# cvjena/mvlm

Hardware: AMD Instinct MI355X
Metric: views/sec (render+CNN+fuse) per mesh, 256x256x96 views (higher is better)
Workload: dtype f32; 1 GPU; configs[2] BU_3DFE-RGB+depth.json: 96 views @ 256x256 of one 99458-triangle textured synthetic face OBJ, 84 landmarks, 4 input channels (RGB+depth), seeded random weights; views_total=96, views_per_gpu=96, landmarks=84, in_channels=4, triangles=99458, selection_method=simple, parallelism=1 GPU, no collective

## Files before the change

### include/mvlm_hip.h

```cpp
#ifndef MVLM_HIP_H
#define MVLM_HIP_H

#include <stddef.h>
#include <stdint.h>

#ifdef __cplusplus
extern "C" {
#endif

typedef struct mvlm_ctx mvlm_ctx;
typedef struct mvlm_mesh mvlm_mesh;
typedef struct mvlm_texture mvlm_texture;

#define MVLM_IMAGE_SIZE 256
#define MVLM_CONV_DESC_INTS 12

enum { MVLM_MODE_QUANTILE = 0, MVLM_MODE_ABSOLUTE = 1 };
enum { MVLM_MAXIMA_SIMPLE = 0, MVLM_MAXIMA_MOMENT = 1 };

int mvlm_ctx_create(int device, mvlm_ctx** out);
void mvlm_ctx_destroy(mvlm_ctx* ctx);
const char* mvlm_last_error(mvlm_ctx* ctx);
int mvlm_set_stream(mvlm_ctx* ctx, void* hip_stream);
int mvlm_synchronize(mvlm_ctx* ctx);
const char* mvlm_build_arch(void);

typedef struct mvlm_obj mvlm_obj;
enum { MVLM_OBJ_ERR_ARGS = 1, MVLM_OBJ_ERR_FILE = 2, MVLM_OBJ_ERR_EMPTY = 3, MVLM_OBJ_ERR_INDEX = 4,
       MVLM_OBJ_ERR_SYNTAX = 5 };
int mvlm_obj_read(const char* path, mvlm_obj** out, char* err, int err_len);
int mvlm_obj_info(const mvlm_obj* obj, int64_t* n_verts, int64_t* n_tris, int* has_uvs);
int mvlm_obj_copy(const mvlm_obj* obj, float* verts, float* uvs, int32_t* tris);
int mvlm_obj_has_colors(const mvlm_obj* obj, int* has);
int mvlm_obj_copy_colors(const mvlm_obj* obj, uint8_t* rgb);
int mvlm_obj_has_normals(const mvlm_obj* obj, int* has);
int mvlm_obj_copy_normals(const mvlm_obj* obj, float* normals);
void mvlm_obj_free(mvlm_obj* obj);
int mvlm_mesh_read(const char* path, mvlm_obj** out, char* err, int err_len);

int mvlm_mesh_upload(mvlm_ctx* ctx, const float* verts_host, const float* uvs_host, int n_verts,
                     const int32_t* tris_host, int n_tris, const uint8_t* tex_host, int tex_h, int tex_w,
                     mvlm_mesh** out);
int mvlm_mesh_upload_colors(mvlm_ctx* ctx, mvlm_mesh* mesh, const uint8_t* rgb_host, int n_verts);
int mvlm_mesh_set_point_radius(mvlm_ctx* ctx, mvlm_mesh* mesh, double r_model_units);
int mvlm_mesh_point_radius(const mvlm_mesh* mesh, double* r_model_units);
int mvlm_points_auto_radius(const float* verts_host, int n, double* r_model_units);
int mvlm_points_set_counting(mvlm_ctx* ctx, int enabled);
int mvlm_points_get_stats(mvlm_ctx* ctx, unsigned long long* covered, unsigned long long* issued);
int mvlm_points_stage_ms(mvlm_ctx* ctx, float* ms2);
int mvlm_mesh_upload_normals(mvlm_ctx* ctx, mvlm_mesh* mesh, const float* normals_host, int n_verts);
int mvlm_mesh_estimate_normals(mvlm_ctx* ctx, mvlm_mesh* mesh, int32_t* neighbors_dev);
int mvlm_mesh_copy_normals(mvlm_ctx* ctx, const mvlm_mesh* mesh, float* normals_host);
int mvlm_normals_stage_ms(mvlm_ctx* ctx, float* ms3);
int mvlm_normals_get_stats(mvlm_ctx* ctx, unsigned long long* stats3);
int mvlm_mesh_triangulate_points(mvlm_ctx* ctx, const mvlm_mesh* cloud, const int32_t* neighbors_dev, int32_t* tris_dev, long long cap,
                                 int32_t* n_tris_dev);
int mvlm_cloud_mesh_stage_ms(mvlm_ctx* ctx, float* ms3);
void mvlm_mesh_free(mvlm_ctx* ctx, mvlm_mesh* mesh);

int mvlm_jpeg_info(const uint8_t* jpeg_host, size_t n_bytes, int* width, int* height, int* components, char* why, int why_len);
int mvlm_mesh_upload_jpeg(mvlm_ctx* ctx, const float* verts_host, const float* uvs_host, int n_verts,
                          const int32_t* tris_host, int n_tris, const uint8_t* jpeg_host, size_t jpeg_bytes,
                          mvlm_mesh** out);
int mvlm_texture_from_jpeg(mvlm_ctx* ctx, const uint8_t* jpeg_host, size_t jpeg_bytes, mvlm_texture** out);
int mvlm_texture_size(const mvlm_texture* tex, int* height, int* width);
void mvlm_texture_free(mvlm_ctx* ctx, mvlm_texture* tex);
int mvlm_mesh_upload_texture(mvlm_ctx* ctx, const float* verts_host, const float* uvs_host, int n_verts,
                             const int32_t* tris_host, int n_tris, mvlm_texture* tex, int* consumed, mvlm_mesh** out);
int mvlm_jpeg_decode(mvlm_ctx* ctx, const uint8_t* jpeg_host, size_t jpeg_bytes, uint8_t* rgb_dev, int* rounds_out);

int mvlm_render(mvlm_ctx* ctx, const mvlm_mesh* mesh, const double* rot_host, int n_views, float* out_dev);
int mvlm_render_rotations_dev(mvlm_ctx* ctx, const double** rot_dev);
int mvlm_set_render_shading(mvlm_ctx* ctx, int shading);
int mvlm_set_render_subpixel_bits(mvlm_ctx* ctx, int bits);
int mvlm_set_render_multisamples(mvlm_ctx* ctx, int samples);
int mvlm_render_set_profiling(mvlm_ctx* ctx, int enabled);
int mvlm_render_get_profile(mvlm_ctx* ctx, int32_t* n_views, int32_t* n_verts, int32_t* n_tris, float* ms, int cap);
int mvlm_render_check(mvlm_ctx* ctx);

int mvlm_render_landmark_view(mvlm_ctx* ctx, const mvlm_mesh* mesh, const double* rot_host, int n_views, int size,
                              const float* frame_host ,
                              const double* landmarks_host , int n_lm,
                              float radius, const uint8_t* lm_rgb_host ,
                              uint8_t* out_dev , int32_t* lm_pixels_dev );
int mvlm_landmark_view_stage_ms(mvlm_ctx* ctx, float* ms7);
int mvlm_render_landmark_view_colored(mvlm_ctx* ctx, const mvlm_mesh* mesh, const double* rot_host, int n_views, int size,
                                      const float* frame_host, const double* landmarks_host, int n_lm, float radius,
                                      const uint8_t* lm_rgb_host, uint8_t* out_dev, int32_t* lm_pixels_dev,
                                      const uint8_t* vert_rgba_dev );

int mvlm_render_ray_view(mvlm_ctx* ctx, const mvlm_mesh* mesh, const double* rot_host, int n_views, int size,
                         const float* frame_host, const double* landmarks_host, int n_lm, float radius, const uint8_t* lm_rgb_host,
                         const double* starts_dev, const double* ends_dev, int n_rays ,
                         float ray_radius, const uint8_t* ray_rgb_host ,
                         uint8_t* out_dev, int32_t* lm_pixels_dev, int32_t* ray_pixels_dev );
int mvlm_ray_view_stage_ms(mvlm_ctx* ctx, float* ms8);

int mvlm_view_sheet_layout(int n_views, int cols_in, int scale, int gap, int* cols, int* rows, int* width, int* height, char* why,
                           int why_len);
int mvlm_render_view_sheet(mvlm_ctx* ctx, const float* images_dev, int n_views, const float* maxima_dev, int n_lm,
                           const double* rot_host, const double* landmarks_host, const uint8_t* lm_rgb_host, const uint8_t* used_host,
                           int background, int cols_in, int scale, int gap, double marker_radius, uint8_t* out_dev);

int mvlm_heat_plane_peaks(mvlm_ctx* ctx, const float* heat_dev, int n_planes, float* peaks_dev);
int mvlm_render_heat_sheet(mvlm_ctx* ctx, const float* images_dev, const float* heat_dev, int n_views, int n_lm,
                           const uint8_t* sel_host , const uint8_t* lm_rgb_host ,
                           int background, int cols_in, int scale, int gap, double floor, double opacity, uint8_t* out_dev);
int mvlm_heat_sheet_stage_ms(mvlm_ctx* ctx, float* ms3);

int mvlm_surface_heat(mvlm_ctx* ctx, const mvlm_mesh* mesh, const double* rot_dev, const float* images_dev, const float* heat_dev,
                      int n_views, int n_lm, const uint8_t* sel_host, const uint8_t* lm_rgb_host, double floor, double opacity,
                      int depth_tol, uint8_t* vert_rgba_dev, float* score_dev ,
                      int32_t* n_vis_dev , int32_t* peak_vertex_dev ,
                      float* peak_score_dev );
int mvlm_surface_heat_stage_ms(mvlm_ctx* ctx, float* ms3);
int mvlm_surface_heat_release(mvlm_ctx* ctx);
int mvlm_scratch_bytes(mvlm_ctx* ctx, const char* prefix, size_t* bytes);

int mvlm_landmark_geodesics(mvlm_ctx* ctx, const mvlm_mesh* mesh, const double* pts_dev, int n, int init_rings, int max_sweeps,
                            long long max_scratch_bytes, const int32_t* pairs_host, int n_pairs, double* snapped_dev,
                            int32_t* tri_dev, double* D_dev, double* E_dev, int32_t* sweeps_dev, double* field_dev);
int mvlm_geodesic_stage_ms(mvlm_ctx* ctx, float* ms4);
int mvlm_geodesic_release(mvlm_ctx* ctx);

int mvlm_png_bound(int height, int width, size_t* bytes);
int mvlm_png_encode(mvlm_ctx* ctx, const uint8_t* rgba_dev, int n_images, int height, int width, int filter_mode,
                    uint8_t* png_host, size_t stride_bytes, size_t* png_bytes_out );
int mvlm_png_stage_ms(mvlm_ctx* ctx, float* ms4);

int mvlm_cnn_load(mvlm_ctx* ctx, const float* blob_host, size_t n_floats, const int32_t* desc_host, int n_slots,
                  int n_landmarks, int in_channels);
size_t mvlm_cnn_workspace_bytes(mvlm_ctx* ctx, int batch);
int mvlm_cnn_maxima(mvlm_ctx* ctx, const float* images_dev, int n_views, const int32_t* chan_sel_host,
                    float* maxima_dev, void* workspace_dev, size_t workspace_bytes, int batch);
int mvlm_cnn_set_selection(mvlm_ctx* ctx, int method);
int mvlm_cnn_heatmaps(mvlm_ctx* ctx, const float* images_dev, int n_views, const int32_t* chan_sel_host,
                      float* heat_dev, void* workspace_dev, size_t workspace_bytes, int batch);
int mvlm_cnn_set_execution(mvlm_ctx* ctx, int graph_mode, int concurrency);
int mvlm_cnn_set_pairing(mvlm_ctx* ctx, int mode);
int mvlm_cnn_set_winograd(mvlm_ctx* ctx, int mode);
int mvlm_pack_winograd_weights(const float* w9_host, int cin_pad, int cout_pad, float* w12_host);
int mvlm_cnn_set_winograd4(mvlm_ctx* ctx, int mode);
int mvlm_pack_winograd4_weights(const float* w9_host, int cin_pad, int cout_pad, float* w18_host);
int mvlm_cnn_set_winograd4_wide(mvlm_ctx* ctx, int on);
int mvlm_conv_wino4_wide_serves(int ksize, int cin_pad, int cout_pad, int size);
int mvlm_conv_wino4_wide_launches(mvlm_ctx* ctx, int64_t* count, int reset);
int mvlm_cnn_set_winograd4_padded(mvlm_ctx* ctx, int mode);
int mvlm_conv_wino4_padded_launches(mvlm_ctx* ctx, int64_t* count, int reset);
int mvlm_conv_wino4_padded_stride(int cout_pad);
int mvlm_pack_winograd4_weights_padded(const float* w9_host, const float* bias_host, int cin_pad, int cout_pad, float* w18_pad_host,
                                       float* bias_pad_host);
int mvlm_cnn_execution_stats(mvlm_ctx* ctx, int64_t* eager_runs, int64_t* graph_captures, int64_t* graph_replays,
                             int64_t* graph_failures);
size_t mvlm_pack_fast_weights(const float* w, int cout, int cin, int cout_pad, int cin_pad, uint16_t* out);
int mvlm_cnn_load_fast(mvlm_ctx* ctx, const uint16_t* blob_host, size_t n_u16, const int64_t* slot_offsets, int n_slots);
int mvlm_cnn_set_precision(mvlm_ctx* ctx, int fast);
int mvlm_conv2d_fast(mvlm_ctx* ctx, const float* x_dev, int batch, int cin, int h, int w, const float* w_host, int cout,
                     const float* bias_host, const float* pre_scale_host, const float* pre_shift_host,
                     const float* post_scale_host, const float* post_shift_host, const float* r_dev, float* y_dev);
size_t mvlm_pack_fast_weights16(const float* w, int cout, int cin, int cout_pad, int cin_pad, uint16_t* out, float* unscale);
int mvlm_cnn_load_fast16(mvlm_ctx* ctx, const uint16_t* blob_host, size_t n_u16, const int64_t* slot_offsets,
                         const float* slot_unscale, int n_slots);
int mvlm_cnn_fast16_overflowed(mvlm_ctx* ctx, int* overflowed);
int mvlm_conv2d_fast16(mvlm_ctx* ctx, const float* x_dev, int batch, int cin, int h, int w, const float* w_host, int cout,
                       const float* bias_host, const float* pre_scale_host, const float* pre_shift_host,
                       const float* post_scale_host, const float* post_shift_host, const float* r_dev, float* y_dev);
int mvlm_cnn_set_profiling(mvlm_ctx* ctx, int enabled);
int mvlm_cnn_get_profile(mvlm_ctx* ctx, int32_t* slot, int32_t* variant, double* flops, float* ms, int cap);
const char* mvlm_conv_variant_name(int variant);
int mvlm_cnn_get_profile_shapes(mvlm_ctx* ctx, int32_t* shapes6, int cap);
int mvlm_conv_variant_serves(int variant, int ksize, int cin_pad, int cout_pad, int size, int kind);
int mvlm_conv_set_override(mvlm_ctx* ctx, int ksize, int cin_pad, int cout_pad, int size, int kind, int variant);

int mvlm_heatmap_maxima(mvlm_ctx* ctx, const float* heat_dev, int n_views, int n_landmarks, int size, int method,
                        float* out_dev);

int mvlm_conv2d(mvlm_ctx* ctx, const float* x_dev, int batch, int cin, int h, int w, const float* w_host, int cout,
                int ksize, const float* bias_host, const float* pre_scale_host, const float* pre_shift_host,
                const float* post_scale_host, const float* post_shift_host, const float* r_dev, int upsample_in,
                float* y_dev);

int mvlm_conv2d_pair(mvlm_ctx* ctx, int batch, int cin, int cout, const float* x0_dev, int size0, const float* w0_host,
                     const float* r0_dev, float* raw0_dev, float* y0_dev, const float* x1_dev, int size1,
                     const float* w1_host, const float* r1_dev, float* raw1_dev, float* y1_dev,
                     const float* pre_scale_host, const float* pre_shift_host, int variant);
int mvlm_conv_force_variant(mvlm_ctx* ctx, int variant);
int mvlm_conv_bench(mvlm_ctx* ctx, int batch, int cin, int cout, int ksize, int size, int flags, int variant, int iters,
                    float* ms_per_launch, int* variant_used);
int mvlm_conv_pair_bench(mvlm_ctx* ctx, int batch, int cin, int cout, int size, int flags, int variant, int iters,
                         float* ms_per_launch);

int mvlm_estimate_lines(mvlm_ctx* ctx, const float* maxima_dev, const double* rot_dev, int n_views, int n_landmarks,
                        int image_size, double* starts_dev, double* ends_dev);
int mvlm_consensus_mask(mvlm_ctx* ctx, const float* maxima_dev, int n_views, int n_landmarks, int mode, double q,
                        double thr, uint8_t* mask_dev, int32_t* count_dev);
int mvlm_consensus_solve(mvlm_ctx* ctx, const double* starts_dev, const double* ends_dev, const uint8_t* mask_dev,
                         const int32_t* count_dev, const int32_t* draws_dev, int n_views, int n_landmarks,
                         double* out_dev, double* err_dev);

#define MVLM_REPORT_STATS 9
#define MVLM_VIEW_KEPT 1
#define MVLM_VIEW_DRAWN 2
#define MVLM_VIEW_INLIER 4
#define MVLM_VIEW_USED 8
int mvlm_consensus_report(mvlm_ctx* ctx, const double* starts_dev, const double* ends_dev, const uint8_t* mask_dev,
                          const int32_t* draws_dev, int n_views, int n_landmarks, double* out_dev, double* err_dev,
                          double* stats_dev, int32_t* counts_dev, double* dist2_dev, uint8_t* flags_dev);

int mvlm_project_to_surface(mvlm_ctx* ctx, const mvlm_mesh* mesh, const double* pts_dev, int n_points,
                            double* out_dev);

int mvlm_surface_attach(mvlm_ctx* ctx, const mvlm_mesh* mesh, const double* pts_dev, int n_points, double* snapped_dev,
                        int32_t* tri_dev, double* bary_dev, double* uv_dev);

int mvlm_clip_rays_to_mesh(mvlm_ctx* ctx, const mvlm_mesh* mesh, const double* starts_dev, const double* ends_dev,
                           int n_rays, double* new_ends_dev, uint8_t* hit_dev);

int mvlm_allgather_maxima(mvlm_ctx* ctx, void* nccl_comm, int rank, int world, const float* maxima_local_dev, int n_total,
                          int n_landmarks, float* maxima_all_dev);
int mvlm_gather_pack(mvlm_ctx* ctx, const float* maxima_local_dev, int n_local, int n_max, int n_landmarks, float* slot_dev);
int mvlm_gather_unpack(mvlm_ctx* ctx, const float* slots_dev, int world, int n_total, int n_landmarks, float* maxima_all_dev);

#ifdef __cplusplus
}
#endif
#endif
```

### mvlm_amd/_lib.py

```python
from __future__ import annotations

import ctypes as C
import os
import subprocess
import threading
from pathlib import Path

_HERE = Path(__file__).resolve().parent
LIB_PATH = Path(os.environ["MVLM_HIP_LIB"]) if os.environ.get("MVLM_HIP_LIB") else _HERE / "lib" / "libmvlm_hip.so"
CSRC = _HERE / "csrc"

c_float_p = C.POINTER(C.c_float)
c_double_p = C.POINTER(C.c_double)
c_int32_p = C.POINTER(C.c_int32)
c_uint8_p = C.POINTER(C.c_uint8)

SIGNATURES = {
    "mvlm_ctx_create": (C.c_int, [C.c_int, C.POINTER(C.c_void_p)]),
    "mvlm_ctx_destroy": (None, [C.c_void_p]),
    "mvlm_last_error": (C.c_char_p, [C.c_void_p]),
    "mvlm_set_stream": (C.c_int, [C.c_void_p, C.c_void_p]),
    "mvlm_synchronize": (C.c_int, [C.c_void_p]),
    "mvlm_build_arch": (C.c_char_p, []),
    "mvlm_obj_read": (C.c_int, [C.c_char_p, C.POINTER(C.c_void_p), C.c_char_p, C.c_int]),
    "mvlm_mesh_read": (C.c_int, [C.c_char_p, C.POINTER(C.c_void_p), C.c_char_p, C.c_int]),
    "mvlm_obj_info": (C.c_int, [C.c_void_p, C.POINTER(C.c_int64), C.POINTER(C.c_int64), C.POINTER(C.c_int)]),
    "mvlm_obj_copy": (C.c_int, [C.c_void_p, c_float_p, c_float_p, c_int32_p]),
    "mvlm_obj_has_colors": (C.c_int, [C.c_void_p, C.POINTER(C.c_int)]),
    "mvlm_obj_copy_colors": (C.c_int, [C.c_void_p, c_uint8_p]),
    "mvlm_obj_has_normals": (C.c_int, [C.c_void_p, C.POINTER(C.c_int)]),
    "mvlm_obj_copy_normals": (C.c_int, [C.c_void_p, c_float_p]),
    "mvlm_obj_free": (None, [C.c_void_p]),
    "mvlm_mesh_upload": (C.c_int, [C.c_void_p, c_float_p, c_float_p, C.c_int, c_int32_p, C.c_int, c_uint8_p,
                                   C.c_int, C.c_int, C.POINTER(C.c_void_p)]),
    "mvlm_mesh_upload_colors": (C.c_int, [C.c_void_p, C.c_void_p, c_uint8_p, C.c_int]),
    "mvlm_mesh_set_point_radius": (C.c_int, [C.c_void_p, C.c_void_p, C.c_double]),
    "mvlm_mesh_point_radius": (C.c_int, [C.c_void_p, c_double_p]),
    "mvlm_points_auto_radius": (C.c_int, [c_float_p, C.c_int, c_double_p]),
    "mvlm_points_set_counting": (C.c_int, [C.c_void_p, C.c_int]),
    "mvlm_points_stage_ms": (C.c_int, [C.c_void_p, c_float_p]),
    "mvlm_points_get_stats": (C.c_int, [C.c_void_p, C.POINTER(C.c_uint64), C.POINTER(C.c_uint64)]),
    "mvlm_mesh_upload_normals": (C.c_int, [C.c_void_p, C.c_void_p, c_float_p, C.c_int]),
    "mvlm_mesh_estimate_normals": (C.c_int, [C.c_void_p, C.c_void_p, C.c_void_p]),
    "mvlm_mesh_copy_normals": (C.c_int, [C.c_void_p, C.c_void_p, c_float_p]),
    "mvlm_normals_stage_ms": (C.c_int, [C.c_void_p, c_float_p]),
    "mvlm_normals_get_stats": (C.c_int, [C.c_void_p, C.POINTER(C.c_uint64)]),
    "mvlm_mesh_triangulate_points": (C.c_int, [C.c_void_p, C.c_void_p, C.c_void_p, C.c_void_p, C.c_longlong, C.c_void_p]),
    "mvlm_cloud_mesh_stage_ms": (C.c_int, [C.c_void_p, c_float_p]),
    "mvlm_mesh_free": (None, [C.c_void_p, C.c_void_p]),
    "mvlm_jpeg_info": (C.c_int, [c_uint8_p, C.c_size_t, C.POINTER(C.c_int), C.POINTER(C.c_int), C.POINTER(C.c_int), C.c_char_p, C.c_int]),
    "mvlm_mesh_upload_jpeg": (C.c_int, [C.c_void_p, c_float_p, c_float_p, C.c_int, c_int32_p, C.c_int, c_uint8_p, C.c_size_t,
                                        C.POINTER(C.c_void_p)]),
    "mvlm_texture_from_jpeg": (C.c_int, [C.c_void_p, c_uint8_p, C.c_size_t, C.POINTER(C.c_void_p)]),
    "mvlm_texture_size": (C.c_int, [C.c_void_p, C.POINTER(C.c_int), C.POINTER(C.c_int)]),
    "mvlm_texture_free": (None, [C.c_void_p, C.c_void_p]),
    "mvlm_mesh_upload_texture": (C.c_int, [C.c_void_p, c_float_p, c_float_p, C.c_int, c_int32_p, C.c_int, C.c_void_p,
                                           C.POINTER(C.c_int), C.POINTER(C.c_void_p)]),
    "mvlm_jpeg_decode": (C.c_int, [C.c_void_p, c_uint8_p, C.c_size_t, C.c_void_p, C.POINTER(C.c_int)]),
    "mvlm_render": (C.c_int, [C.c_void_p, C.c_void_p, c_double_p, C.c_int, C.c_void_p]),
    "mvlm_render_check": (C.c_int, [C.c_void_p]),
    "mvlm_render_landmark_view": (C.c_int, [C.c_void_p, C.c_void_p, c_double_p, C.c_int, C.c_int, c_float_p, c_double_p, C.c_int,
                                            C.c_float, c_uint8_p, C.c_void_p, C.c_void_p]),
    "mvlm_landmark_view_stage_ms": (C.c_int, [C.c_void_p, c_float_p]),
    "mvlm_render_ray_view": (C.c_int, [C.c_void_p, C.c_void_p, c_double_p, C.c_int, C.c_int, c_float_p, c_double_p, C.c_int,
                                       C.c_float, c_uint8_p, C.c_void_p, C.c_void_p, C.c_int, C.c_float, c_uint8_p,
                                       C.c_void_p, C.c_void_p, C.c_void_p]),
    "mvlm_ray_view_stage_ms": (C.c_int, [C.c_void_p, c_float_p]),
    "mvlm_view_sheet_layout": (C.c_int, [C.c_int, C.c_int, C.c_int, C.c_int, C.POINTER(C.c_int), C.POINTER(C.c_int), C.POINTER(C.c_int),
                                         C.POINTER(C.c_int), C.c_char_p, C.c_int]),
    "mvlm_render_view_sheet": (C.c_int, [C.c_void_p, C.c_void_p, C.c_int, C.c_void_p, C.c_int, c_double_p, c_double_p, c_uint8_p,
                                         c_uint8_p, C.c_int, C.c_int, C.c_int, C.c_int, C.c_double, C.c_void_p]),
    "mvlm_heat_plane_peaks": (C.c_int, [C.c_void_p, C.c_void_p, C.c_int, C.c_void_p]),
    "mvlm_render_heat_sheet": (C.c_int, [C.c_void_p, C.c_void_p, C.c_void_p, C.c_int, C.c_int, c_uint8_p, c_uint8_p, C.c_int, C.c_int,
                                         C.c_int, C.c_int, C.c_double, C.c_double, C.c_void_p]),
    "mvlm_heat_sheet_stage_ms": (C.c_int, [C.c_void_p, c_float_p]),
    "mvlm_surface_heat": (C.c_int, [C.c_void_p, C.c_void_p, C.c_void_p, C.c_void_p, C.c_void_p, C.c_int, C.c_int, c_uint8_p, c_uint8_p,
                                    C.c_double, C.c_double, C.c_int, C.c_void_p, C.c_void_p, C.c_void_p, C.c_void_p, C.c_void_p]),
    "mvlm_surface_heat_stage_ms": (C.c_int, [C.c_void_p, c_float_p]),
    "mvlm_surface_heat_release": (C.c_int, [C.c_void_p]),
    "mvlm_render_landmark_view_colored": (C.c_int, [C.c_void_p, C.c_void_p, c_double_p, C.c_int, C.c_int, c_float_p, c_double_p, C.c_int,
                                                    C.c_float, c_uint8_p, C.c_void_p, C.c_void_p, C.c_void_p]),
    "mvlm_scratch_bytes": (C.c_int, [C.c_void_p, C.c_char_p, C.POINTER(C.c_size_t)]),
    "mvlm_landmark_geodesics": (C.c_int, [C.c_void_p, C.c_void_p, C.c_void_p, C.c_int, C.c_int, C.c_int, C.c_longlong, c_int32_p, C.c_int,
                                          C.c_void_p, C.c_void_p, C.c_void_p, C.c_void_p, C.c_void_p, C.c_void_p]),
    "mvlm_geodesic_stage_ms": (C.c_int, [C.c_void_p, c_float_p]),
    "mvlm_geodesic_release": (C.c_int, [C.c_void_p]),
    "mvlm_png_bound": (C.c_int, [C.c_int, C.c_int, C.POINTER(C.c_size_t)]),
    "mvlm_png_encode": (C.c_int, [C.c_void_p, C.c_void_p, C.c_int, C.c_int, C.c_int, C.c_int, C.c_void_p, C.c_size_t,
                                  C.POINTER(C.c_size_t)]),
    "mvlm_png_stage_ms": (C.c_int, [C.c_void_p, c_float_p]),
    "mvlm_render_set_profiling": (C.c_int, [C.c_void_p, C.c_int]),
    "mvlm_render_get_profile": (C.c_int, [C.c_void_p, c_int32_p, c_int32_p, c_int32_p, c_float_p, C.c_int]),
    "mvlm_render_rotations_dev": (C.c_int, [C.c_void_p, C.POINTER(C.c_void_p)]),
    "mvlm_gather_pack": (C.c_int, [C.c_void_p, C.c_void_p, C.c_int, C.c_int, C.c_int, C.c_void_p]),
    "mvlm_gather_unpack": (C.c_int, [C.c_void_p, C.c_void_p, C.c_int, C.c_int, C.c_int, C.c_void_p]),
    "mvlm_allgather_maxima": (C.c_int, [C.c_void_p, C.c_void_p, C.c_int, C.c_int, C.c_void_p, C.c_int, C.c_int, C.c_void_p]),
    "mvlm_set_render_shading": (C.c_int, [C.c_void_p, C.c_int]),
    "mvlm_set_render_subpixel_bits": (C.c_int, [C.c_void_p, C.c_int]),
    "mvlm_set_render_multisamples": (C.c_int, [C.c_void_p, C.c_int]),
    "mvlm_cnn_load": (C.c_int, [C.c_void_p, c_float_p, C.c_size_t, c_int32_p, C.c_int, C.c_int, C.c_int]),
    "mvlm_cnn_workspace_bytes": (C.c_size_t, [C.c_void_p, C.c_int]),
    "mvlm_cnn_maxima": (C.c_int, [C.c_void_p, C.c_void_p, C.c_int, c_int32_p, C.c_void_p, C.c_void_p, C.c_size_t,
                                  C.c_int]),
    "mvlm_cnn_heatmaps": (C.c_int, [C.c_void_p, C.c_void_p, C.c_int, c_int32_p, C.c_void_p, C.c_void_p, C.c_size_t,
                                    C.c_int]),
    "mvlm_cnn_set_execution": (C.c_int, [C.c_void_p, C.c_int, C.c_int]),
    "mvlm_cnn_set_selection": (C.c_int, [C.c_void_p, C.c_int]),
    "mvlm_cnn_set_pairing": (C.c_int, [C.c_void_p, C.c_int]),
    "mvlm_cnn_set_winograd": (C.c_int, [C.c_void_p, C.c_int]),
    "mvlm_pack_winograd_weights": (C.c_int, [c_float_p, C.c_int, C.c_int, c_float_p]),
    "mvlm_cnn_set_winograd4": (C.c_int, [C.c_void_p, C.c_int]),
    "mvlm_pack_winograd4_weights": (C.c_int, [c_float_p, C.c_int, C.c_int, c_float_p]),
    "mvlm_cnn_set_winograd4_wide": (C.c_int, [C.c_void_p, C.c_int]),
    "mvlm_conv_wino4_wide_serves": (C.c_int, [C.c_int, C.c_int, C.c_int, C.c_int]),
    "mvlm_conv_wino4_wide_launches": (C.c_int, [C.c_void_p, C.POINTER(C.c_int64), C.c_int]),
    "mvlm_cnn_set_winograd4_padded": (C.c_int, [C.c_void_p, C.c_int]),
    "mvlm_conv_wino4_padded_launches": (C.c_int, [C.c_void_p, C.POINTER(C.c_int64), C.c_int]),
    "mvlm_conv_wino4_padded_stride": (C.c_int, [C.c_int]),
    "mvlm_pack_winograd4_weights_padded": (C.c_int, [c_float_p, c_float_p, C.c_int, C.c_int, c_float_p, c_float_p]),
    "mvlm_cnn_execution_stats": (C.c_int, [C.c_void_p, C.POINTER(C.c_int64), C.POINTER(C.c_int64), C.POINTER(C.c_int64),
                                          C.POINTER(C.c_int64)]),
    "mvlm_pack_fast_weights": (C.c_size_t, [c_float_p, C.c_int, C.c_int, C.c_int, C.c_int, C.POINTER(C.c_uint16)]),
    "mvlm_cnn_load_fast": (C.c_int, [C.c_void_p, C.POINTER(C.c_uint16), C.c_size_t, C.POINTER(C.c_int64), C.c_int]),
    "mvlm_cnn_set_precision": (C.c_int, [C.c_void_p, C.c_int]),
    "mvlm_pack_fast_weights16": (C.c_size_t, [c_float_p, C.c_int, C.c_int, C.c_int, C.c_int, C.POINTER(C.c_uint16), c_float_p]),
    "mvlm_cnn_load_fast16": (C.c_int, [C.c_void_p, C.POINTER(C.c_uint16), C.c_size_t, C.POINTER(C.c_int64), c_float_p, C.c_int]),
    "mvlm_cnn_fast16_overflowed": (C.c_int, [C.c_void_p, C.POINTER(C.c_int)]),
    "mvlm_conv2d_fast16": (C.c_int, [C.c_void_p, C.c_void_p, C.c_int, C.c_int, C.c_int, C.c_int, c_float_p, C.c_int, c_float_p,
                                     c_float_p, c_float_p, c_float_p, c_float_p, C.c_void_p, C.c_void_p]),
    "mvlm_conv2d_fast": (C.c_int, [C.c_void_p, C.c_void_p, C.c_int, C.c_int, C.c_int, C.c_int, c_float_p, C.c_int, c_float_p,
                                   c_float_p, c_float_p, c_float_p, c_float_p, C.c_void_p, C.c_void_p]),
    "mvlm_cnn_set_profiling": (C.c_int, [C.c_void_p, C.c_int]),
    "mvlm_cnn_get_profile": (C.c_int, [C.c_void_p, c_int32_p, c_int32_p, c_double_p, c_float_p, C.c_int]),
    "mvlm_conv_variant_name": (C.c_char_p, [C.c_int]),
    "mvlm_cnn_get_profile_shapes": (C.c_int, [C.c_void_p, c_int32_p, C.c_int]),
    "mvlm_conv_variant_serves": (C.c_int, [C.c_int, C.c_int, C.c_int, C.c_int, C.c_int, C.c_int]),
    "mvlm_conv_set_override": (C.c_int, [C.c_void_p, C.c_int, C.c_int, C.c_int, C.c_int, C.c_int, C.c_int]),
    "mvlm_heatmap_maxima": (C.c_int, [C.c_void_p, C.c_void_p, C.c_int, C.c_int, C.c_int, C.c_int, C.c_void_p]),
    "mvlm_conv2d": (C.c_int, [C.c_void_p, C.c_void_p, C.c_int, C.c_int, C.c_int, C.c_int, c_float_p, C.c_int, C.c_int,
                              c_float_p, c_float_p, c_float_p, c_float_p, c_float_p, C.c_void_p, C.c_int, C.c_void_p]),
    "mvlm_conv2d_pair": (C.c_int, [C.c_void_p, C.c_int, C.c_int, C.c_int, C.c_void_p, C.c_int, c_float_p, C.c_void_p, C.c_void_p,
                                   C.c_void_p, C.c_void_p, C.c_int, c_float_p, C.c_void_p, C.c_void_p, C.c_void_p, c_float_p, c_float_p,
                                   C.c_int]),
    "mvlm_conv_force_variant": (C.c_int, [C.c_void_p, C.c_int]),
    "mvlm_conv_bench": (C.c_int, [C.c_void_p, C.c_int, C.c_int, C.c_int, C.c_int, C.c_int, C.c_int, C.c_int, C.c_int,
                                  c_float_p, C.POINTER(C.c_int)]),
    "mvlm_conv_pair_bench": (C.c_int, [C.c_void_p, C.c_int, C.c_int, C.c_int, C.c_int, C.c_int, C.c_int, C.c_int, c_float_p]),
    "mvlm_estimate_lines": (C.c_int, [C.c_void_p, C.c_void_p, C.c_void_p, C.c_int, C.c_int, C.c_int, C.c_void_p,
                                      C.c_void_p]),
    "mvlm_consensus_mask": (C.c_int, [C.c_void_p, C.c_void_p, C.c_int, C.c_int, C.c_int, C.c_double, C.c_double,
                                      C.c_void_p, C.c_void_p]),
    "mvlm_consensus_solve": (C.c_int, [C.c_void_p, C.c_void_p, C.c_void_p, C.c_void_p, C.c_void_p, C.c_void_p, C.c_int,
                                       C.c_int, C.c_void_p, C.c_void_p]),
    "mvlm_project_to_surface": (C.c_int, [C.c_void_p, C.c_void_p, C.c_void_p, C.c_int, C.c_void_p]),
    "mvlm_consensus_report": (C.c_int, [C.c_void_p, C.c_void_p, C.c_void_p, C.c_void_p, C.c_void_p, C.c_int, C.c_int,
                                        C.c_void_p, C.c_void_p, C.c_void_p, C.c_void_p, C.c_void_p, C.c_void_p]),
    "mvlm_surface_attach": (C.c_int, [C.c_void_p, C.c_void_p, C.c_void_p, C.c_int, C.c_void_p, C.c_void_p, C.c_void_p,
                                      C.c_void_p]),
    "mvlm_clip_rays_to_mesh": (C.c_int, [C.c_void_p, C.c_void_p, C.c_void_p, C.c_void_p, C.c_int, C.c_void_p,
                                         C.c_void_p]),
}

_lib = None


class MvlmHipError(RuntimeError):
    pass


def build(force: bool = False) -> Path:
    if force and LIB_PATH.exists():
        LIB_PATH.unlink()
    jobs = str(min(8, os.cpu_count() or 1))
    r = subprocess.run(["make", "-C", str(CSRC), "-j", jobs], capture_output=True, text=True)
    if r.returncode != 0 or not LIB_PATH.exists():
        raise MvlmHipError(f"building libmvlm_hip.so failed:\n{r.stdout[-4000:]}\n{r.stderr[-4000:]}")
    return LIB_PATH


def load():
    global _lib
    if _lib is not None:
        return _lib
    if not LIB_PATH.exists():
        raise MvlmHipError(
            f"{LIB_PATH} not found - the MI355X HIP library is required (no CPU fallback). "
            "Build it with `python -c 'import __graft_entry__ as g; g.build()'` or `make -C mvlm_amd/csrc`.")
    import torch

    lib = C.CDLL(str(LIB_PATH))
    for name, (res, args) in SIGNATURES.items():
        fn = getattr(lib, name)
        fn.restype = res
        fn.argtypes = args
    _lib = lib
    return lib


def as_ptr(arr, ctype):
    return arr.ctypes.data_as(C.POINTER(ctype))


class Context:

    def __init__(self, device: int = 0):
        self.lib = load()
        self.handle = C.c_void_p()
        rc = self.lib.mvlm_ctx_create(int(device), C.byref(self.handle))
        if rc != 0:
            reasons = {2: "no such GPU device", 3: "hipSetDevice failed", 4: "hipGetDeviceProperties failed",
                       5: "device is not a gfx950 (MI355X)"}
            raise MvlmHipError(f"mvlm_ctx_create(device={device}) failed: {reasons.get(rc, rc)}")
        self.device = int(device)

    def check(self, rc: int, exc=MvlmHipError):
        if rc != 0:
            msg = self.lib.mvlm_last_error(self.handle)
            raise exc(msg.decode() if msg else f"mvlm call failed ({rc})")

    def set_stream(self, stream_ptr: int):
        self.check(self.lib.mvlm_set_stream(self.handle, C.c_void_p(stream_ptr)))
        self._bound_stream = stream_ptr

    def bind_current_stream(self, torch, dev):
        held = getattr(self, "_held_stream", None)
        if held is not None and held[0] == threading.get_ident() and getattr(self, "_bound_stream", None) == held[1]:
            return
        self.set_stream(torch.cuda.current_stream(dev).cuda_stream)

    def hold_stream(self, torch, dev):
        return _HeldStream(self, torch, dev)

    def synchronize(self):
        self.check(self.lib.mvlm_synchronize(self.handle))

    def close(self):
        if getattr(self, "handle", None) and self.handle.value:
            self.lib.mvlm_ctx_destroy(self.handle)
            self.handle = C.c_void_p()

    def __del__(self):
        try:
            self.close()
        except Exception:
            pass


class _HeldStream:
    def __init__(self, ctx, torch, dev):
        self.ctx, self.torch, self.dev, self.mine = ctx, torch, dev, False

    def __enter__(self):
        if getattr(self.ctx, "_held_stream", None) is None:
            ptr = self.torch.cuda.current_stream(self.dev).cuda_stream
            self.ctx.set_stream(ptr)
            self.ctx._held_stream = (threading.get_ident(), ptr)
            self.mine = True
        return self

    def __exit__(self, *exc):
        if self.mine:
            self.ctx._held_stream = None
        return False


_contexts: dict[int, Context] = {}


def get_context(device: int = 0) -> Context:
    ctx = _contexts.get(device)
    if ctx is None:
        ctx = _contexts[device] = Context(device)
# ... 2 lines not shown
```

### mvlm_amd/csrc/api.hip

```cpp
#include <atomic>
#include <cstring>

#include <memory>

#include <cmath>

#include "common.h"
#include "raster_points_math.h"
#include "raster_view_math.h"

void* mvlm_ctx::get_scratch(const char* name, size_t bytes) {
    auto& e = scratch[name];
    if (e.second >= bytes && e.first) return e.first;
    if (e.first) {
        hipStreamSynchronize(stream);
        hipFree(e.first);
        e = {nullptr, 0};
    }
    void* p = nullptr;
    const size_t want = bytes + bytes / 4 + 256;
    if (hipMalloc(&p, want) != hipSuccess) return nullptr;
    e = {p, want};
    return p;
}

extern "C" const char* mvlm_build_arch(void) { return "gfx950"; }

extern "C" int mvlm_ctx_create(int device, mvlm_ctx** out) {
    if (!out) return 1;
    *out = nullptr;
    int n = 0;
    if (hipGetDeviceCount(&n) != hipSuccess || device < 0 || device >= n) return 2;
    if (hipSetDevice(device) != hipSuccess) return 3;
    hipDeviceProp_t prop;
    if (hipGetDeviceProperties(&prop, device) != hipSuccess) return 4;
    auto* ctx = new mvlm_ctx();
    ctx->device = device;
    if (std::string(prop.gcnArchName).rfind("gfx950", 0) != 0) {
        fprintf(stderr, "mvlm_hip: device %d is %s, this library is built for gfx950 (MI355X) only\n", device,
                prop.gcnArchName);
        delete ctx;
        return 5;
    }
    *out = ctx;
    return 0;
}

extern "C" void mvlm_ctx_destroy(mvlm_ctx* ctx) {
    if (!ctx) return;
    hipSetDevice(ctx->device);
    hipStreamSynchronize(ctx->stream);
    for (auto& kv : ctx->scratch)
        if (kv.second.first) hipFree(kv.second.first);
    if (ctx->cnn.blob) hipFree(ctx->cnn.blob);
    if (ctx->cnn.fast_blob) hipFree(ctx->cnn.fast_blob);
    if (ctx->cnn.fast16_blob) hipFree(ctx->cnn.fast16_blob);
    for (auto& ww : ctx->cnn.wino)
        if (ww.blob) hipFree(ww.blob);
    if (ctx->cnn.wino4_pad_blob) hipFree(ctx->cnn.wino4_pad_blob);
    if (ctx->cnn.fast16_flag) hipFree(ctx->cnn.fast16_flag);
    if (ctx->switch_event) hipEventDestroy(ctx->switch_event);
    for (int i = 0; i < 2; ++i) {
        if (ctx->kparts_ws[i]) hipFree(ctx->kparts_ws[i]);
        if (ctx->kparts_cnt[i]) hipFree(ctx->kparts_cnt[i]);
    }
    for (auto& e : ctx->mesh_pool) {
        hipFree(e.p);
        if (e.freed) hipEventDestroy(e.freed);
    }
    for (hipEvent_t e : ctx->event_free) hipEventDestroy(e);
    for (int i = 0; i < 2; ++i) {
        if (ctx->upload_stage[i]) hipHostFree(ctx->upload_stage[i]);
        if (ctx->upload_stage_done[i]) hipEventDestroy(ctx->upload_stage_done[i]);
    }
    if (ctx->upload_stream) hipStreamDestroy(ctx->upload_stream);
    if (ctx->jpeg_scratch) hipFree(ctx->jpeg_scratch);
    if (ctx->jpeg_flags_host) hipHostFree(ctx->jpeg_flags_host);
    if (ctx->render_overflow_host) hipHostFree(ctx->render_overflow_host);
    for (auto e : ctx->cnn.event_pool)
        if (e) hipEventDestroy(e);
    for (auto e : ctx->render_events)
        if (e) hipEventDestroy(e);
    for (auto e : ctx->cnn.sync_events)
        if (e) hipEventDestroy(e);
    ctx->cnn.drop_graphs();
    if (ctx->cnn.side_stream) hipStreamDestroy(ctx->cnn.side_stream);
    if (ctx->cnn.capture_stream) hipStreamDestroy(ctx->cnn.capture_stream);
    delete ctx;
}

extern "C" const char* mvlm_last_error(mvlm_ctx* ctx) {
    if (!ctx) return "null context";
    if (mvlm_thread_error_ctx() != ctx) {
        std::lock_guard<std::mutex> lock(ctx->err_mu);
        mvlm_thread_error() = ctx->err;
        mvlm_thread_error_ctx() = ctx;
    }
    return mvlm_thread_error().c_str();
}

extern "C" int mvlm_set_stream(mvlm_ctx* ctx, void* hip_stream) {
    MVLM_ENTER(ctx);
    hipStream_t next = static_cast<hipStream_t>(hip_stream);
    if (next != ctx->stream) {
        if (!ctx->switch_event) MVLM_CHECK_HIP(ctx, hipEventCreateWithFlags(&ctx->switch_event, hipEventDisableTiming));
        if (!ctx->track_order) {
            MVLM_CHECK_HIP(ctx, hipEventRecord(ctx->switch_event, ctx->stream));
            ctx->order_recorded = true;
            ctx->track_order = true;
        }
        if (ctx->order_recorded) MVLM_CHECK_HIP(ctx, hipStreamWaitEvent(next, ctx->switch_event, 0));
    }
    ctx->stream = next;
    return 0;
}

extern "C" int mvlm_synchronize(mvlm_ctx* ctx) {
    MVLM_ENTER(ctx);
    MVLM_CHECK_HIP(ctx, hipStreamSynchronize(ctx->stream));
    return 0;
}

static bool take_upload_buffer(mvlm_ctx* ctx, size_t bytes, size_t room, void** p, size_t* cap, hipEvent_t* waited) {
    int pick = -1;
    for (int k = 0; k < int(ctx->mesh_pool.size()); ++k) {
        const size_t c = ctx->mesh_pool[size_t(k)].cap;
        if (c >= room && c <= 4 * bytes + (1u << 20)) {
            pick = k;
            break;
        }
    }
    if (pick >= 0) {
        const auto e = ctx->mesh_pool[size_t(pick)];
        ctx->mesh_pool.erase(ctx->mesh_pool.begin() + pick);
        ctx->mesh_pool_bytes -= e.cap;
        *p = e.p;
        *cap = e.cap;
        *waited = e.freed;
        return !(e.freed && hipStreamWaitEvent(ctx->upload_stream, e.freed, 0) != hipSuccess);
    }
    *cap = (room + 65535) / 65536 * 65536;
    if (hipMalloc(p, *cap) != hipSuccess) {
        *p = nullptr;
        *cap = 0;
        return false;
    }
    return true;
}

struct mvlm_texture {
    uint8_t* dev = nullptr;
    size_t cap = 0;
    int h = 0, w = 0;
    hipEvent_t waited = nullptr;
};

static int mesh_upload_impl(mvlm_ctx* ctx, const float* verts_host, const float* uvs_host, int n_verts, const int32_t* tris_host,
                            int n_tris, const uint8_t* tex_host, int tex_h, int tex_w, MvlmJpegPlan* jpeg,
                            const uint8_t* jpeg_bytes, size_t jpeg_n, mvlm_mesh** out, mvlm_texture* pre = nullptr) {
    MVLM_REQUIRE(ctx, out, "mesh_upload: null output");
    *out = nullptr;
    MVLM_REQUIRE(ctx, verts_host && n_verts > 0 && n_tris >= 0 && (tris_host || n_tris == 0), "mesh_upload: mesh does not contain any points");
    MVLM_REQUIRE(ctx, n_tris > 0 || !(jpeg || pre), "mesh_upload: a point cloud (n_tris == 0) takes no texture");
    if (n_tris == 0) {
        uvs_host = nullptr;
        tex_host = nullptr;
    }
    MVLM_REQUIRE(ctx, !(tex_host || jpeg || pre) || (tex_h > 0 && tex_w > 0), "mesh_upload: bad texture size");
    for (long i = 0; i < 3l * n_tris; ++i)
        MVLM_REQUIRE(ctx, tris_host[i] >= 0 && tris_host[i] < n_verts, "mesh_upload: triangle index out of range");
    const bool with_tex = (tex_host || jpeg || pre) && uvs_host;
    if (!with_tex) jpeg = nullptr;
    if (!with_tex) pre = nullptr;
    const void* src[4] = {verts_host, uvs_host, tris_host, with_tex && !jpeg && !pre ? tex_host : nullptr};
    const size_t bytes[4] = {size_t(n_verts) * 12, uvs_host ? size_t(n_verts) * 8 : 0, size_t(n_tris) * 12,
                             with_tex ? size_t(tex_h) * tex_w * 3 : 0};
    const size_t room[4] = {bytes[0], bytes[1], bytes[2], bytes[3] ? bytes[3] + 4 : 0};
    size_t off[5], total = 0;
    for (int i = 0; i < 4; ++i) {
        off[i] = total;
        total += ((src[i] ? bytes[i] : 0) + 255) / 256 * 256;
    }
    off[4] = total;
    if (jpeg) total += mvlm_jpeg_stage_bytes(*jpeg, jpeg_n);

    std::lock_guard<std::mutex> upload_lock(ctx->upload_mu);
    MVLM_CHECK_HIP(ctx, hipSetDevice(ctx->device));
    if (!ctx->upload_stream) MVLM_CHECK_HIP(ctx, hipStreamCreateWithFlags(&ctx->upload_stream, hipStreamNonBlocking));
    const int slot = ctx->upload_stage_next;
    ctx->upload_stage_next ^= 1;
    if (ctx->upload_stage_done[slot]) MVLM_CHECK_HIP(ctx, hipEventSynchronize(ctx->upload_stage_done[slot]));
    if (ctx->upload_stage_cap[slot] < total) {
        if (ctx->upload_stage[slot]) (void)hipHostFree(ctx->upload_stage[slot]);
        ctx->upload_stage[slot] = nullptr;
        ctx->upload_stage_cap[slot] = 0;
        const size_t cap = (total + (size_t(4) << 20)) / (size_t(4) << 20) * (size_t(4) << 20);
        MVLM_CHECK_HIP(ctx, hipHostMalloc(&ctx->upload_stage[slot], cap, hipHostMallocDefault));
        ctx->upload_stage_cap[slot] = cap;
    }
    auto* stage = static_cast<unsigned char*>(ctx->upload_stage[slot]);
    for (int i = 0; i < 4; ++i)
        if (src[i] && bytes[i]) std::memcpy(stage + off[i], src[i], bytes[i]);
    std::string jpeg_why;
    if (jpeg && mvlm_jpeg_fill_stage(*jpeg, jpeg_bytes, jpeg_n, stage + off[4], jpeg_why) != 0) {
        ctx->fail("jpeg: " + jpeg_why);
        return 2;
    }

    auto* m = new mvlm_mesh();
    static std::atomic<unsigned long long> next_uid{1};
    m->uid = next_uid.fetch_add(1);
    m->n_verts = n_verts;
// ... 537 lines not shown
```

### mvlm_amd/csrc/cnn_graph.hip

```cpp
#include <cstdlib>
#include <cstring>

#include "common.h"

namespace {

constexpr long CONCURRENT_MAX_PIXELS_32 = 32l * 32 * 32;

struct Tensor {
    float* p = nullptr;
    int C = 0, S = 0;
    size_t off = 0, elems = 0;
};

struct Block {
    size_t off, size;
    bool free;
    int arena;
    bool deferred;
};

bool parity_slots_usable(const ConvSlotDesc& r) { return r.present != 0 && (r.cout_pad == 96 || r.cout_pad == 80 || r.cout_pad == 84); }

struct Exec {
// ... 1 lines not shown
    CnnState& st;
    int B;
    char* ws;
    size_t ws_bytes;
    bool dry;
    size_t cursor = 0, high = 0;
    std::vector<Block> blocks;
    int rc = 0;
    int arena = 0;
    bool forked = false;
    const bool no_pool_fusion = [] { const char* e = getenv("MVLM_POOL_KERNEL_ONLY"); return e && e[0] == '1'; }();
    const bool scatter_only = [] { const char* e = getenv("MVLM_SCATTER_ONLY"); return e && e[0] == '1'; }();
    const int consumer_add_max_batch = [] { const char* e = getenv("MVLM_CONSUMER_ADD_MAX_BATCH"); return e ? atoi(e) : 16; }();

    Exec(mvlm_ctx* c, int batch, void* w, size_t wb, bool d) : ctx(c), st(c->cnn), B(batch), ws((char*)w), ws_bytes(wb), dry(d) {}

    Tensor alloc_raw(size_t bytes, int C, int S) {
        bytes = (bytes + 255) / 256 * 256;
        Tensor t;
        t.C = C;
        t.S = S;
        t.elems = bytes / 4;
        for (auto& b : blocks)
            if (b.free && b.size == bytes && b.arena == arena) {
                b.free = false;
                t.off = b.off;
                t.p = dry ? nullptr : reinterpret_cast<float*>(ws + b.off);
                return t;
            }
        blocks.push_back({cursor, bytes, false, arena, false});
        t.off = cursor;
        cursor += bytes;
        if (cursor > high) high = cursor;
        if (!dry && cursor > ws_bytes) {
            rc = ctx->fail("cnn: workspace too small (mvlm_cnn_workspace_bytes)");
            t.p = nullptr;
            return t;
        }
        t.p = dry ? nullptr : reinterpret_cast<float*>(ws + t.off);
        return t;
    }
    Tensor alloc(int C, int S) { return alloc_raw(size_t(B) * C * S * S * 4, C, S); }
    void release(const Tensor& t) {
        for (auto& b : blocks)
            if (b.off == t.off && !b.free && !b.deferred) {
                if (forked && b.arena == 0)
                    b.deferred = true;
                else
                    b.free = true;
                return;
            }
    }

    hipEvent_t next_event() {
        if (st.sync_cursor >= st.sync_events.size()) st.sync_events.resize(st.sync_cursor + 1, nullptr);
        hipEvent_t& e = st.sync_events[st.sync_cursor++];
        if (!e && hipEventCreateWithFlags(&e, hipEventDisableTiming) != hipSuccess) {
            rc = ctx->fail("cnn: hipEventCreate failed");
            return nullptr;
        }
        return e;
    }
    void fork() {
        forked = true;
        if (dry || rc) return;
        if (!st.side_stream) {
            int lo_prio = 0, hi_prio = 0;
            (void)hipDeviceGetStreamPriorityRange(&lo_prio, &hi_prio);
            if (hipStreamCreateWithPriority(&st.side_stream, hipStreamNonBlocking, hi_prio) != hipSuccess) {
                rc = ctx->fail("cnn: hipStreamCreate failed");
                return;
            }
        }
        hipEvent_t e = next_event();
        if (rc) return;
        if (hipEventRecord(e, ctx->stream) != hipSuccess || hipStreamWaitEvent(st.side_stream, e, 0) != hipSuccess)
            rc = ctx->fail("cnn: fork of the side stream failed");
    }
    void side() {
        arena = 1;
        if (!dry) ctx->launch_stream = st.side_stream;
    }
    void main() {
        arena = 0;
        ctx->launch_stream = nullptr;
    }
    void join() {
        main();
        forked = false;
        for (auto& b : blocks)
            if (b.deferred) {
                b.deferred = false;
                b.free = true;
            }
        if (dry || rc) return;
        hipEvent_t e = next_event();
        if (rc) return;
        if (hipEventRecord(e, st.side_stream) != hipSuccess || hipStreamWaitEvent(ctx->stream, e, 0) != hipSuccess)
            rc = ctx->fail("cnn: join of the side stream failed");
    }

    const ConvSlotDesc& d(int slot) const { return st.desc[size_t(slot)]; }
    const float* blob(int off) const { return off < 0 ? nullptr : st.blob + off; }

    void fill_shape(int slot, ConvArgs& a, int S) const {
        const ConvSlotDesc& r = d(slot);
        a.cin = r.cin;
        a.cout = r.cout;
        a.ksize = r.ksize;
        a.cin_pad = r.cin_pad;
        a.cout_pad = r.cout_pad;
        a.B = B;
        a.H = a.W = S;
    }
    int fill(int slot, const Tensor& x, ConvArgs& a, int S) {
        if (rc) return rc;
        const ConvSlotDesc& r = d(slot);
        if (!r.present) return rc = ctx->fail("cnn: conv slot not present in the packed weights");
        a.in = x.p;
        a.in_ctot = x.C;
        a.in_coff = 0;
        fill_shape(slot, a, S);
        a.w = blob(r.w_off);
        for (int f = 0; f < MVLM_WINO_FORMS_N; ++f) {
            const CnnState::WinoWeights& ww = st.wino[f];
            a.*mvlm_wino_form(f).weights = (size_t(slot) < ww.off.size() && ww.off[size_t(slot)] >= 0) ? ww.blob + ww.off[size_t(slot)] : nullptr;
        }
        a.wino4_pad = size_t(slot) < st.wino4_pad_id.size() ? st.wino4_pad_id[size_t(slot)] : 0;
        a.bias = blob(r.bias_off);
        a.pre_scale = blob(r.pre_scale_off);
        a.pre_shift = blob(r.pre_shift_off);
        a.post_scale = blob(r.post_scale_off);
        a.post_shift = blob(r.post_shift_off);
        if (x.C != a.cin) return rc = ctx->fail("cnn: channel mismatch between graph and packed weights");
        return 0;
    }
    bool runs_fast(int slot, const ConvArgs& a) const {
        const std::vector<long long>& off = st.fast == 2 ? st.fast16_off : st.fast_off;
        return st.fast && size_t(slot) < off.size() && off[size_t(slot)] >= 0 && mvlm_conv_fast_ok(a, st.fast == 2 ? 2 : 3);
    }
    int prof_begin(hipEvent_t& e0, hipEvent_t& e1) {
        if (!st.profiling) return 0;
        if (st.event_cursor + 2 > st.event_pool.size()) st.event_pool.resize(st.event_cursor + 2, nullptr);
        for (int k = 0; k < 2; ++k) {
            hipEvent_t& e = st.event_pool[st.event_cursor + k];
            if (!e && hipEventCreate(&e) != hipSuccess) return rc = ctx->fail("cnn: hipEventCreate failed");
        }
        e0 = st.event_pool[st.event_cursor];
        e1 = st.event_pool[st.event_cursor + 1];
        st.event_cursor += 2;
        hipEventRecord(e0, ctx->cur_stream());
        return 0;
    }
    static double conv_flops(const ConvArgs& a, int variant = -1) {
        const double taps = mvlm_conv_variant_is_wino(variant) ? mvlm_wino_form(MVLM_WINO_F23).macs
                            : mvlm_conv_variant_is_wino4(variant) ? mvlm_wino_form(MVLM_WINO_F43).macs : double(a.ksize * a.ksize);
        return 2.0 * a.cin * a.cout * taps * double(a.H) * a.W * a.B * a.n_par;
    }

    int conv(int slot, const Tensor& x, ConvArgs a, int S) {
        if (fill(slot, x, a, S)) return rc;
        if (dry) return 0;
        int variant = -1;
        hipEvent_t e0 = nullptr, e1 = nullptr;
        if (prof_begin(e0, e1)) return rc;
        if (runs_fast(slot, a)) {
            if (st.fast == 2) {
                variant = MVLM_CONV_VARIANT_FAST16;
                if (mvlm_launch_conv_fast(ctx, a, st.fast16_blob + st.fast16_off[size_t(slot)], 2, st.fast16_unscale[size_t(slot)])) return rc = 1;
            } else {
                variant = MVLM_CONV_VARIANT_FAST;
                if (mvlm_launch_conv_fast(ctx, a, st.fast_blob + st.fast_off[size_t(slot)])) return rc = 1;
            }
        } else if (mvlm_launch_conv(ctx, a, &variant)) {
            return rc = 1;
        }
        if (st.profiling) {
            hipEventRecord(e1, ctx->cur_stream());
            ConvProfileRec rec{slot, variant, conv_flops(a, variant), e0, e1};
            const ConvKey key = mvlm_conv_key(a);
            const short shape[6] = {key.ksize, key.cin_pad, key.cout_pad, key.size, key.kind, key.batch};
            for (int i = 0; i < 6; ++i) rec.shape[i] = shape[i];
            st.prof.push_back(rec);
        }
        return 0;
    }

    int pair_variant(int slot0, const Tensor& x0, ConvArgs a0, int S0, int slot1, const Tensor& x1, ConvArgs a1, int S1) {
        if (st.pairing == 0 || fill(slot0, x0, a0, S0) || fill(slot1, x1, a1, S1)) return -1;
        if (runs_fast(slot0, a0) || runs_fast(slot1, a1)) return -1;
        if (mvlm_conv_wino_variant(ctx, a0) >= 0 || mvlm_conv_wino_variant(ctx, a1) >= 0) return -1;
        return mvlm_conv_pair_variant(a0, a1, st.pairing);
    }

    int conv_pair(int pv, int slot0, const Tensor& x0, ConvArgs a0, int S0, int slot1, const Tensor& x1, ConvArgs a1, int S1) {
        if (pv < 0) {
            conv(slot0, x0, a0, S0);
            return conv(slot1, x1, a1, S1);
        }
        if (fill(slot0, x0, a0, S0) || fill(slot1, x1, a1, S1)) return rc;
        if (dry) return 0;
        hipEvent_t e0 = nullptr, e1 = nullptr;
        if (prof_begin(e0, e1)) return rc;
        if (mvlm_launch_conv_pair(ctx, a0, a1, pv)) return rc = 1;
        if (st.profiling) {
            hipEventRecord(e1, ctx->cur_stream());
            st.prof.push_back({slot0, pv, conv_flops(a0) + conv_flops(a1), e0, e1});
        }
        return 0;
    }

    struct RbPlan {
        int base = 0, S = 0, cout = 0;
        bool resample = false;
        Tensor x, y, t1, t2;
        Tensor* pooled = nullptr;
        ConvArgs ar, a[3];
        bool want_pool = false, keep_full = true;
    };
    RbPlan plan_rb(int rb_index, const Tensor& x, Tensor* hi, Tensor* pooled = nullptr, bool keep_full = true) {
        RbPlan P;
        P.base = 1 + 4 * rb_index;
        P.S = x.S;
        P.x = x;
        P.cout = d(P.base + 1).cout * 2;
        const int cout = P.cout, h = cout / 2, q = cout / 4;
        P.resample = d(P.base).present != 0;
        if (!hi) P.y = alloc(cout, P.S);
        if (P.resample && hi) {
            rc = ctx->fail("cnn: resampling block cannot scatter");
            return P;
        }
        P.t1 = alloc(h, P.S);
        P.t2 = alloc(q, P.S);
        if (P.resample) {
            P.ar.out = P.y.p;
            P.ar.out_ctot = cout;
        }
        const Tensor& res = P.resample ? P.y : P.x;
        const int coffs[3] = {0, h, h + q};
        for (int j = 0; j < 3; ++j) {
            ConvArgs& a = P.a[j];
            a.res1 = res.p;
            a.res1_ctot = res.C;
            a.res1_coff = coffs[j];
            if (hi) {
                a.out = hi->p;
                a.out_ctot = hi->C;
                a.out_coff = coffs[j];
                a.up_out = 1;
                a.skip = hi->p;
                a.skip_ctot = hi->C;
                a.skip_coff = coffs[j];
            } else {
                a.out = P.y.p;
                a.out_ctot = cout;
                a.out_coff = coffs[j];
            }
        }
        P.a[0].out_raw = P.t1.p;
        P.a[0].raw_ctot = h;
        P.a[1].out_raw = P.t2.p;
        P.a[1].raw_ctot = q;
        P.want_pool = pooled && !hi;
        if (P.want_pool)
            for (ConvArgs& a : P.a) a.pool_hint = 1;
        P.keep_full = keep_full;
        P.pooled = pooled;
        if (P.want_pool) *pooled = alloc(cout, P.S / 2);
        return P;
    }
    const Tensor& rb_input(const RbPlan& P, int j) const { return j == 0 ? P.x : (j == 1 ? P.t1 : P.t2); }
    void set_pool(RbPlan& P, bool can_fuse) {
        if (!P.want_pool || !can_fuse) return;
        for (ConvArgs& a : P.a) {
            a.pool_out = P.pooled->p;
            a.pool_ctot = P.cout;
            a.pool_coff = a.out_coff;
            if (!P.keep_full) a.out = nullptr;
        }
    }
    void finish_rb(RbPlan& P) {
        release(P.t1);
        release(P.t2);
        if (P.want_pool && !P.a[0].pool_out && !dry && !rc) pool_kernel(P.y.p, P.cout, P.S, P.pooled->p);
    }
    void pool_kernel(const float* in, int channels, int S, float* out) {
        hipEvent_t e0 = nullptr, e1 = nullptr;
        if (prof_begin(e0, e1)) return;
        if (mvlm_launch_maxpool2(ctx, in, B * channels, S, S, out)) {
            rc = 1;
            return;
        }
        if (st.profiling) {
            hipEventRecord(e1, ctx->cur_stream());
            ConvProfileRec rec{-1, -1, 0.0, e0, e1};
            rec.shape[2] = short(channels);
            rec.shape[3] = short(S);
            rec.shape[5] = short(B > 32767 ? 32767 : B);
            st.prof.push_back(rec);
        }
    }

    Tensor rb(int rb_index, const Tensor& x, Tensor* hi, Tensor* pooled = nullptr, bool keep_full = true) {
        RbPlan P = plan_rb(rb_index, x, hi, pooled, keep_full);
        if (rc) return P.y;
        if (P.resample) conv(P.base, x, P.ar, P.S);
        bool fuse = P.want_pool;
        for (int j = 0; j < 3 && fuse; ++j) fuse = pool_fusable(P.base + 1 + j, rb_input(P, j), P.a[j], P.S);
        set_pool(P, fuse);
        for (int j = 0; j < 3; ++j) conv(P.base + 1 + j, rb_input(P, j), P.a[j], P.S);
        finish_rb(P);
        return P.y;
    }

    void rb_pair(int rbA, const Tensor& xA, Tensor& yA, int rbB, const Tensor& xB, Tensor& yB, Tensor* pooledB) {
        RbPlan PA = plan_rb(rbA, xA, nullptr), PB = plan_rb(rbB, xB, nullptr, pooledB);
        yA = PA.y;
        yB = PB.y;
        if (rc) return;
        if (PA.resample) conv(PA.base, xA, PA.ar, PA.S);
        if (PB.resample) conv(PB.base, xB, PB.ar, PB.S);
        int pv[3];
        bool fuse = PB.want_pool;
        for (int j = 0; j < 3; ++j) {
            pv[j] = pair_variant(PA.base + 1 + j, rb_input(PA, j), PA.a[j], PA.S, PB.base + 1 + j, rb_input(PB, j), PB.a[j], PB.S);
            if (fuse) fuse = pv[j] >= 0 ? (!no_pool_fusion && mvlm_conv_variant_can_pool(pv[j])) : pool_fusable(PB.base + 1 + j, rb_input(PB, j), PB.a[j], PB.S);
        }
        set_pool(PB, fuse);
        for (int j = 0; j < 3; ++j)
            conv_pair(pv[j], PA.base + 1 + j, rb_input(PA, j), PA.a[j], PA.S, PB.base + 1 + j, rb_input(PB, j), PB.a[j], PB.S);
        finish_rb(PA);
// ... 271 lines not shown
int run_batch(mvlm_ctx* ctx, const float* img, int nb, const int* sel4, float* maxima, int view0, int n_total,
              float* heat, void* ws, size_t ws_bytes) {
    CnnState& st = ctx->cnn;
    auto eager = [&]() {
        st.sync_cursor = 0;
        Exec ex(ctx, nb, ws, ws_bytes, false);
        const int rc = ex.forward(img, sel4, maxima, view0, n_total, heat);
        ctx->launch_stream = nullptr;
        ++st.eager_runs;
        return rc;
    };
    if (!st.graph_mode || st.profiling) return eager();
    const void* out = heat ? static_cast<const void*>(heat) : static_cast<const void*>(maxima);
    CnnGraphEntry* ent = nullptr;
    for (auto& g : st.graphs)
        if (g.images == img && g.out == out && g.ws == ws && g.ws_bytes == ws_bytes && g.nb == nb && g.view0 == view0 &&
            g.n_total == n_total && g.heat == (heat ? 1 : 0) && g.sel4[0] == sel4[0] && g.sel4[1] == sel4[1] &&
            g.sel4[2] == sel4[2] && g.sel4[3] == sel4[3]) {
            ent = &g;
            break;
        }
    if (!ent) {
        constexpr size_t MAX_GRAPHS = 16;
        if (st.graphs.size() >= MAX_GRAPHS) {
            if (st.graphs.front().exec) hipGraphExecDestroy(st.graphs.front().exec);
            st.graphs.erase(st.graphs.begin());
        }
        CnnGraphEntry g;
        g.images = img;
        g.out = out;
        g.ws = ws;
        g.ws_bytes = ws_bytes;
        g.nb = nb;
        g.view0 = view0;
        g.n_total = n_total;
        g.heat = heat ? 1 : 0;
        for (int k = 0; k < 4; ++k) g.sel4[k] = sel4[k];
        st.graphs.push_back(g);
        ent = &st.graphs.back();
    }
    ++ent->uses;
    if (ent->exec) {
        MVLM_CHECK_HIP(ctx, hipGraphLaunch(ent->exec, ctx->stream));
        ++st.graph_replays;
        return 0;
    }
    if (ent->uses < 2) return eager();
    auto note = [&](const char* what, hipError_t e) {
        if (st.graph_failures++ == 0)
            fprintf(stderr, "mvlm_hip: %s failed (%s); this pass runs launch by launch\n", what, hipGetErrorString(e));
        (void)hipGetLastError();
    };
    if (!st.capture_stream) {
        const hipError_t e = hipStreamCreateWithFlags(&st.capture_stream, hipStreamNonBlocking);
        if (e != hipSuccess) {
            st.capture_stream = nullptr;
            note("hipStreamCreate (capture stream)", e);
            return eager();
        }
    }
    st.sync_cursor = 0;
    hipStream_t user_stream = ctx->stream;
    hipError_t e_begin = hipStreamBeginCapture(st.capture_stream, hipStreamCaptureModeThreadLocal);
    if (e_begin != hipSuccess) {
        note("hipStreamBeginCapture", e_begin);
        return eager();
    }
    int rc;
    ctx->stream = st.capture_stream;
    {
        Exec ex(ctx, nb, ws, ws_bytes, false);
        rc = ex.forward(img, sel4, maxima, view0, n_total, heat);
        ctx->launch_stream = nullptr;
    }
    ctx->stream = user_stream;
    hipGraph_t graph = nullptr;
    const hipError_t e_end = hipStreamEndCapture(st.capture_stream, &graph);
    if (rc) {
        if (graph) hipGraphDestroy(graph);
        return rc;
    }
    if (e_end != hipSuccess || !graph) {
        note("hipStreamEndCapture", e_end);
        if (graph) hipGraphDestroy(graph);
        ent->uses = -1000000;
        return eager();
    }
    hipGraphExec_t exec = nullptr;
    const hipError_t e_inst = hipGraphInstantiate(&exec, graph, nullptr, nullptr, 0);
    hipGraphDestroy(graph);
    if (e_inst != hipSuccess || !exec) {
        note("hipGraphInstantiate", e_inst);
        ent->uses = -1000000;
        return eager();
    }
    ent->exec = exec;
    ++st.graph_captures;
    MVLM_CHECK_HIP(ctx, hipGraphLaunch(ent->exec, ctx->stream));
    ++st.graph_replays;
    return 0;
}

int run_cnn(mvlm_ctx* ctx, const float* images, int n_views, const int32_t* chan_sel, float* maxima, float* heat,
            void* ws, size_t ws_bytes, int batch) {
    CnnState& st = ctx->cnn;
    MVLM_REQUIRE(ctx, st.loaded, "cnn: mvlm_cnn_load has not been called");
    MVLM_REQUIRE(ctx, images && n_views > 0 && batch > 0 && ws, "cnn: bad arguments");
    MVLM_REQUIRE(ctx, maxima || heat, "cnn: no output requested");
    int sel4[4] = {0, 0, 0, 0};
    for (int k = 0; k < st.in_channels; ++k) {
        MVLM_REQUIRE(ctx, chan_sel[k] >= 0 && chan_sel[k] < 4, "cnn: channel selector out of range");
        sel4[k] = chan_sel[k];
    }
    st.prof.clear();
    st.event_cursor = 0;
    if (st.fast == 2) MVLM_CHECK_HIP(ctx, hipMemsetAsync(st.fast16_flag, 0, sizeof(unsigned), ctx->stream));
    const size_t img_elems = size_t(MVLM_IMAGE_SIZE) * MVLM_IMAGE_SIZE;
    for (int v0 = 0; v0 < n_views; v0 += batch) {
        const int nb = (n_views - v0) < batch ? (n_views - v0) : batch;
        float* h = heat ? heat + size_t(v0) * st.n_landmarks * img_elems : nullptr;
        const float* img = images + size_t(v0) * img_elems * 4;
        if (run_batch(ctx, img, nb, sel4, maxima, v0, n_views, h, ws, ws_bytes)) return 1;
    }
    return 0;
}

}

extern "C" int mvlm_cnn_load(mvlm_ctx* ctx, const float* blob_host, size_t n_floats, const int32_t* desc_host,
                             int n_slots, int n_landmarks, int in_channels) {
    MVLM_ENTER(ctx);
    MVLM_REQUIRE(ctx, blob_host && desc_host && n_floats > 0, "cnn_load: null weights");
    MVLM_REQUIRE(ctx, n_slots == MVLM_N_SLOTS, "cnn_load: descriptor table must have 183 conv slots");
    MVLM_REQUIRE(ctx, n_landmarks > 0 && in_channels >= 1 && in_channels <= 4, "cnn_load: bad landmark / channel count");
    CnnState& st = ctx->cnn;
    MVLM_CHECK_HIP(ctx, hipSetDevice(ctx->device));
    if (st.blob) {
        MVLM_CHECK_HIP(ctx, hipFree(st.blob));
        st.blob = nullptr;
    }
    st.loaded = false;
    st.fast = 0;
    st.fast_off.clear();
    if (st.fast_blob) {
        (void)hipFree(st.fast_blob);
        st.fast_blob = nullptr;
    }
    st.fast16_off.clear();
    st.fast16_unscale.clear();
    if (st.fast16_blob) {
        (void)hipFree(st.fast16_blob);
        st.fast16_blob = nullptr;
    }
    float** const form_blobs[MVLM_WINO_FORMS_N + 1] = {&st.wino[MVLM_WINO_F23].blob, &st.wino[MVLM_WINO_F43].blob, &st.wino4_pad_blob};
    for (float** b : form_blobs)
        if (*b) {
            (void)hipFree(*b);
            *b = nullptr;
        }
    for (CnnState::WinoWeights& ww : st.wino) ww.off.clear();
    st.wino4_pad_id.clear();
    ctx->conv_wino4_pads.resize(1);
    st.drop_graphs();
    st.desc.resize(size_t(n_slots));
    memcpy(st.desc.data(), desc_host, size_t(n_slots) * sizeof(ConvSlotDesc));
    for (const ConvSlotDesc& r : st.desc) {
        if (!r.present) continue;
        MVLM_REQUIRE(ctx, r.cin > 0 && r.cout > 0 && r.ksize >= 1 && r.ksize <= 3, "cnn_load: bad conv shape");
        MVLM_REQUIRE(ctx, r.cin_pad % 4 == 0 && r.cin_pad >= r.cin &&
                              (r.cout_pad % 16 == 0 || (r.cout_pad == 84 && r.cout == 84 && (r.ksize == 3 || r.ksize == 2))) && r.cout_pad >= r.cout,
                     "cnn_load: bad padding");
        const size_t wsz = size_t(r.ksize) * r.ksize * r.cin_pad * r.cout_pad;
        MVLM_REQUIRE(ctx, r.w_off >= 0 && size_t(r.w_off) + wsz <= n_floats, "cnn_load: weight offset out of range");
        const int offs[5] = {r.bias_off, r.pre_scale_off, r.pre_shift_off, r.post_scale_off, r.post_shift_off};
        const int lens[5] = {r.cout_pad, r.cin_pad, r.cin_pad, r.cout_pad, r.cout_pad};
        for (int k = 0; k < 5; ++k)
            MVLM_REQUIRE(ctx, offs[k] < 0 || size_t(offs[k]) + lens[k] <= n_floats, "cnn_load: vector offset out of range");
    }
    MVLM_REQUIRE(ctx, st.desc[0].cin == in_channels, "cnn_load: conv1 input channels != in_channels");
    MVLM_REQUIRE(ctx, st.desc[MVLM_SLOT_CONV11].cout == n_landmarks, "cnn_load: conv11 output channels != n_landmarks");
    MVLM_CHECK_HIP(ctx, hipMalloc(&st.blob, n_floats * sizeof(float)));
    MVLM_CHECK_HIP(ctx, hipMemcpy(st.blob, blob_host, n_floats * sizeof(float), hipMemcpyHostToDevice));
    std::vector<float> host[MVLM_WINO_FORMS_N + 1];
    std::vector<ConvPackTargets> to(st.desc.size());
    size_t total[MVLM_WINO_FORMS_N + 1] = {0, 0, 0};
    for (int s = 0; s < n_slots; ++s) {
        const ConvSlotDesc& r = st.desc[size_t(s)];
        if (!r.present) continue;
        const ConvPackSizes sizes = mvlm_conv_pack_sizes(r.ksize, r.cin_pad, r.cout_pad);
        for (int f = 0; f < MVLM_WINO_FORMS_N; ++f)
            if (mvlm_wino_form(f).serves_slot(r.ksize, r.cin_pad, r.cout_pad)) {
                to[size_t(s)].wino[f] = &host[f];
                total[f] += sizes.wino[f];
            }
        if (mvlm_conv_wino4_pad_serves_slot(r.ksize, r.cin_pad, r.cout_pad)) {
            to[size_t(s)].wino4_pad = &host[MVLM_WINO_FORMS_N];
            total[MVLM_WINO_FORMS_N] += sizes.wino4_pad + sizes.wino4_pad_bias;
        }
    }
    for (int k = 0; k <= MVLM_WINO_FORMS_N; ++k) host[k].reserve(total[k]);
    for (CnnState::WinoWeights& ww : st.wino) ww.off.assign(size_t(n_slots), -1);
    st.wino4_pad_id.assign(size_t(n_slots), 0);
    std::vector<ConvPackOffsets> made(st.desc.size());
    for (int s = 0; s < n_slots; ++s) {
        const ConvSlotDesc& r = st.desc[size_t(s)];
        if (r.present) made[size_t(s)] = mvlm_conv_pack_forms(to[size_t(s)], blob_host + r.w_off, r.bias_off >= 0 ? blob_host + r.bias_off : nullptr, r.cin_pad, r.cout_pad);
    }
    for (int k = 0; k <= MVLM_WINO_FORMS_N; ++k)
        if (!host[k].empty()) {
            MVLM_CHECK_HIP(ctx, hipMalloc(form_blobs[k], host[k].size() * sizeof(float)));
            MVLM_CHECK_HIP(ctx, hipMemcpy(*form_blobs[k], host[k].data(), host[k].size() * sizeof(float), hipMemcpyHostToDevice));
        }
    for (int s = 0; s < n_slots; ++s) {
        const ConvPackOffsets& m = made[size_t(s)];
        for (int f = 0; f < MVLM_WINO_FORMS_N; ++f) st.wino[f].off[size_t(s)] = m.wino[f];
        if (m.wino4_pad < 0) continue;
        ctx->conv_wino4_pads.push_back({st.wino4_pad_blob + m.wino4_pad, m.wino4_pad_bias < 0 ? nullptr : st.wino4_pad_blob + m.wino4_pad_bias});
        st.wino4_pad_id[size_t(s)] = int(ctx->conv_wino4_pads.size());
    }
    st.n_landmarks = n_landmarks;
    st.in_channels = in_channels;
    st.loaded = true;
    return 0;
}

extern "C" size_t mvlm_cnn_workspace_bytes(mvlm_ctx* ctx, int batch) {
    std::lock_guard<std::mutex> lk(ctx->mu);
    if (!ctx->cnn.loaded || batch <= 0) return 0;
    Exec ex(ctx, batch, nullptr, 0, true);
    const int sel4[4] = {0, 0, 0, 0};
    ex.forward(nullptr, sel4, reinterpret_cast<float*>(8), 0, batch, nullptr);
    return ex.high + 256;
}

extern "C" int mvlm_cnn_maxima(mvlm_ctx* ctx, const float* images_dev, int n_views, const int32_t* chan_sel_host,
                               float* maxima_dev, void* workspace_dev, size_t workspace_bytes, int batch) {
    MVLM_ENTER(ctx);
    MVLM_REQUIRE(ctx, maxima_dev && chan_sel_host, "cnn_maxima: null output / selector");
    return run_cnn(ctx, images_dev, n_views, chan_sel_host, maxima_dev, nullptr, workspace_dev, workspace_bytes, batch);
}

extern "C" int mvlm_cnn_heatmaps(mvlm_ctx* ctx, const float* images_dev, int n_views, const int32_t* chan_sel_host,
                                 float* heat_dev, void* workspace_dev, size_t workspace_bytes, int batch) {
    MVLM_ENTER(ctx);
    MVLM_REQUIRE(ctx, heat_dev && chan_sel_host, "cnn_heatmaps: null output / selector");
    return run_cnn(ctx, images_dev, n_views, chan_sel_host, nullptr, heat_dev, workspace_dev, workspace_bytes, batch);
}

extern "C" int mvlm_cnn_set_execution(mvlm_ctx* ctx, int graph_mode, int concurrency) {
    MVLM_ENTER(ctx);
    MVLM_REQUIRE(ctx, (graph_mode == 0 || graph_mode == 1) && (concurrency == 0 || concurrency == 1),
                 "cnn_set_execution: flags must be 0 or 1");
    CnnState& st = ctx->cnn;
    if (concurrency != st.concurrency) st.drop_graphs();
    st.graph_mode = graph_mode;
    st.concurrency = concurrency;
    return 0;
}

extern "C" int mvlm_cnn_set_selection(mvlm_ctx* ctx, int method) {
    MVLM_ENTER(ctx);
    MVLM_REQUIRE(ctx, method == MVLM_MAXIMA_SIMPLE || method == MVLM_MAXIMA_MOMENT, "cnn_set_selection: 0 simple, 1 moment");
    CnnState& st = ctx->cnn;
    MVLM_REQUIRE(ctx, st.loaded, "cnn_set_selection: mvlm_cnn_load comes first");
    if (method == MVLM_MAXIMA_MOMENT) {
        const ConvSlotDesc& r = st.desc[MVLM_SLOT_PARITY0];
        MVLM_REQUIRE(ctx, parity_slots_usable(r) && r.ksize == 2,
                     "cnn_set_selection: the fused moment selection needs conv11's parity slots in the packed weights");
    }
    if (method != st.selection) st.drop_graphs();
    st.selection = method;
    return 0;
}

extern "C" int mvlm_cnn_set_pairing(mvlm_ctx* ctx, int mode) {
    MVLM_ENTER(ctx);
    MVLM_REQUIRE(ctx, mode >= 0 && mode <= 2, "cnn_set_pairing: 0 never, 1 the measured table (default), 2 wherever one kernel variant serves both");
    CnnState& st = ctx->cnn;
    if (mode != st.pairing) st.drop_graphs();
    st.pairing = mode;
    return 0;
}

static int set_winograd_mode(mvlm_ctx* ctx, int mvlm_ctx::*which, int mode, const char* usage) {
    MVLM_ENTER(ctx);
    MVLM_REQUIRE(ctx, mode >= 0 && mode <= 2, usage);
    if (mode != ctx->*which) ctx->cnn.drop_graphs();
    ctx->*which = mode;
    return 0;
}

extern "C" int mvlm_cnn_set_winograd(mvlm_ctx* ctx, int mode) {
    return set_winograd_mode(ctx, &mvlm_ctx::conv_winograd, mode, "cnn_set_winograd: 0 never, 1 the measured table (default), 2 every layer a Winograd variant can serve");
}

extern "C" int mvlm_cnn_set_winograd4(mvlm_ctx* ctx, int mode) {
    return set_winograd_mode(ctx, &mvlm_ctx::conv_winograd4, mode, "cnn_set_winograd4: 0 never, 1 the measured table (default), 2 every layer the F(4,3) Winograd tile can serve");
}

extern "C" int mvlm_cnn_set_winograd4_wide(mvlm_ctx* ctx, int on) {
    MVLM_ENTER(ctx);
    MVLM_REQUIRE(ctx, on == 0 || on == 1, "cnn_set_winograd4_wide: 0 the 32 x 16 shape on every launch, 1 the wide shape where the output channels come in 64s (default)");
    if (on != ctx->conv_winograd4_wide) ctx->cnn.drop_graphs();
    ctx->conv_winograd4_wide = on;
    return 0;
}

extern "C" int mvlm_cnn_set_winograd4_padded(mvlm_ctx* ctx, int mode) {
    return set_winograd_mode(ctx, &mvlm_ctx::conv_winograd4_padded, mode,
                             "cnn_set_winograd4_padded: 0 never, 1 the measured table (default), 2 every eligible launch of the 80- and 84-row tiles");
}

extern "C" int mvlm_conv_wino4_padded_launches(mvlm_ctx* ctx, int64_t* count, int reset) {
    std::lock_guard<std::mutex> lk(ctx->mu);
    if (count) *count = ctx->conv_wino4_padded_launches;
    if (reset) ctx->conv_wino4_padded_launches = 0;
    return 0;
}

extern "C" int mvlm_conv_wino4_wide_launches(mvlm_ctx* ctx, int64_t* count, int reset) {
    std::lock_guard<std::mutex> lk(ctx->mu);
    if (count) *count = ctx->conv_wino4_wide_launches;
    if (reset) ctx->conv_wino4_wide_launches = 0;
    return 0;
}

extern "C" int mvlm_cnn_execution_stats(mvlm_ctx* ctx, int64_t* eager_runs, int64_t* graph_captures,
                                        int64_t* graph_replays, int64_t* graph_failures) {
    std::lock_guard<std::mutex> lk(ctx->mu);
    const CnnState& st = ctx->cnn;
    if (eager_runs) *eager_runs = st.eager_runs;
    if (graph_captures) *graph_captures = st.graph_captures;
    if (graph_replays) *graph_replays = st.graph_replays;
    if (graph_failures) *graph_failures = st.graph_failures;
    return 0;
}

static int load_fast_weights(mvlm_ctx* ctx, const std::string& who, int splits, const uint16_t* blob_host, size_t n_u16, const int64_t* slot_offsets,
                             const float* slot_unscale, int n_slots) {
    CnnState& st = ctx->cnn;
    const bool f16 = splits == 2;
    MVLM_REQUIRE(ctx, st.loaded, who + ": mvlm_cnn_load comes first");
    MVLM_REQUIRE(ctx, blob_host && slot_offsets && (slot_unscale || !f16) && n_u16 > 0 && size_t(n_slots) == st.desc.size(), who + ": bad arguments");
    for (int s = 0; s < n_slots; ++s) {
        if (slot_offsets[s] < 0) continue;
        const ConvSlotDesc& r = st.desc[size_t(s)];
        MVLM_REQUIRE(ctx, r.present && r.ksize == 3 && mvlm_fast_channels_ok(r.cin, r.cout), who + ": slot is not a fast-eligible 3x3 layer");
        const size_t need = size_t(mvlm_fast_cin_pad(r.cin) / 16) * 9 * 2 * splits * size_t(mvlm_fast_cout_pad(r.cout)) * 8;
        MVLM_REQUIRE(ctx, slot_offsets[s] % 8 == 0 && size_t(slot_offsets[s]) + need <= n_u16, who + ": offset out of range");
        MVLM_REQUIRE(ctx, !f16 || (slot_unscale[s] > 0.f && slot_unscale[s] < 3.0e38f), who + ": bad inverse scale");
    }
    st.drop_graphs();
    if (st.fast == (f16 ? 2 : 1)) st.fast = 0;
    unsigned short*& blob = f16 ? st.fast16_blob : st.fast_blob;
    if (blob) {
        MVLM_CHECK_HIP(ctx, hipFree(blob));
        blob = nullptr;
    }
    if (f16 && !st.fast16_flag) {
        MVLM_CHECK_HIP(ctx, hipMalloc(&st.fast16_flag, sizeof(unsigned)));
        MVLM_CHECK_HIP(ctx, hipMemset(st.fast16_flag, 0, sizeof(unsigned)));
    }
    MVLM_CHECK_HIP(ctx, hipMalloc(&blob, n_u16 * sizeof(uint16_t)));
    MVLM_CHECK_HIP(ctx, hipMemcpy(blob, blob_host, n_u16 * sizeof(uint16_t), hipMemcpyHostToDevice));
    (f16 ? st.fast16_off : st.fast_off).assign(slot_offsets, slot_offsets + n_slots);
    if (f16) st.fast16_unscale.assign(slot_unscale, slot_unscale + n_slots);
    return 0;
}

extern "C" int mvlm_cnn_load_fast(mvlm_ctx* ctx, const uint16_t* blob_host, size_t n_u16, const int64_t* slot_offsets, int n_slots) {
    MVLM_ENTER(ctx);
    return load_fast_weights(ctx, "cnn_load_fast", 3, blob_host, n_u16, slot_offsets, nullptr, n_slots);
}

extern "C" int mvlm_cnn_load_fast16(mvlm_ctx* ctx, const uint16_t* blob_host, size_t n_u16, const int64_t* slot_offsets,
                                    const float* slot_unscale, int n_slots) {
    MVLM_ENTER(ctx);
    return load_fast_weights(ctx, "cnn_load_fast16", 2, blob_host, n_u16, slot_offsets, slot_unscale, n_slots);
}

extern "C" int mvlm_cnn_fast16_overflowed(mvlm_ctx* ctx, int* overflowed) {
    MVLM_ENTER(ctx);
    MVLM_REQUIRE(ctx, overflowed, "cnn_fast16_overflowed: null output");
    *overflowed = 0;
    if (!ctx->cnn.fast16_flag) return 0;
    unsigned v = 0;
    MVLM_CHECK_HIP(ctx, hipMemcpyAsync(&v, ctx->cnn.fast16_flag, sizeof(unsigned), hipMemcpyDeviceToHost, ctx->stream));
    MVLM_CHECK_HIP(ctx, hipStreamSynchronize(ctx->stream));
    *overflowed = v != 0u;
    return 0;
}

extern "C" int mvlm_cnn_set_precision(mvlm_ctx* ctx, int fast) {
    MVLM_ENTER(ctx);
    CnnState& st = ctx->cnn;
    MVLM_REQUIRE(ctx, fast >= 0 && fast <= 2, "cnn_set_precision: 0 (exact fp32), 1 (bf16x3 split) or 2 (f16x2 split on the eligible layers)");
    MVLM_REQUIRE(ctx, fast != 1 || st.fast_blob, "cnn_set_precision: mvlm_cnn_load_fast has not been called");
    MVLM_REQUIRE(ctx, fast != 2 || st.fast16_blob, "cnn_set_precision: mvlm_cnn_load_fast16 has not been called");
    if (fast != st.fast) st.drop_graphs();
    st.fast = fast;
    return 0;
}

extern "C" int mvlm_cnn_set_profiling(mvlm_ctx* ctx, int enabled) {
    MVLM_ENTER(ctx);
    ctx->cnn.profiling = enabled != 0;
    return 0;
}

extern "C" int mvlm_cnn_get_profile(mvlm_ctx* ctx, int32_t* slot, int32_t* variant, double* flops, float* ms, int cap) {
    std::lock_guard<std::mutex> lk(ctx->mu);
    if (hipSetDevice(ctx->device) != hipSuccess) return -1;
    CnnState& st = ctx->cnn;
    if (hipStreamSynchronize(ctx->stream) != hipSuccess) return -1;
    int n = 0;
    for (const auto& r : st.prof) {
        if (n >= cap) break;
        float t = 0.f;
        if (hipEventElapsedTime(&t, r.e0, r.e1) != hipSuccess) return -1;
        slot[n] = r.slot;
        variant[n] = r.variant;
        flops[n] = r.flops;
        ms[n] = t;
        ++n;
    }
    return n;
}

extern "C" int mvlm_cnn_get_profile_shapes(mvlm_ctx* ctx, int32_t* shapes6, int cap) {
    std::lock_guard<std::mutex> lk(ctx->mu);
    int n = 0;
    for (const auto& r : ctx->cnn.prof) {
        if (n >= cap) break;
        for (int k = 0; k < 6; ++k) shapes6[n * 6 + k] = r.shape[k];
        ++n;
    }
    return n;
}

extern "C" const char* mvlm_conv_variant_name(int variant) { return mvlm_conv_variant_name_impl(variant); }
```

### mvlm_amd/csrc/common.h

```cpp
#pragma once
#include <hip/hip_runtime.h>

#include <cstdint>
#include <cstdio>
#include <cstdlib>
#include <map>
#include <mutex>
#include <string>
#include <vector>

#include "../../include/mvlm_hip.h"
#include "conv_pack.h"
#include "jpeg_plan.h"

#define MVLM_CHECK_HIP(ctx, expr)                                                            \
    do {                                                                                     \
        hipError_t _e = (expr);                                                              \
        if (_e != hipSuccess) {                                                              \
            (ctx)->fail(std::string(#expr) + ": " + hipGetErrorString(_e));                  \
            return 1;                                                                        \
        }                                                                                    \
    } while (0)

#define MVLM_ENTER(ctx)                               \
    std::lock_guard<std::mutex> _mvlm_lock((ctx)->mu); \
    MvlmOrderGuard _mvlm_order{(ctx)};                 \
    MVLM_CHECK_HIP(ctx, hipSetDevice((ctx)->device))

#define MVLM_REQUIRE(ctx, cond, msg)                                                         \
    do {                                                                                     \
        if (!(cond)) {                                                                       \
            (ctx)->fail(std::string(msg) + " [" #cond "]");                                  \
            return 1;                                                                        \
        }                                                                                    \
    } while (0)

__host__ __device__ inline int argmax_key(float v) {
    v = v + 0.0f;
    int b;
    __builtin_memcpy(&b, &v, 4);
    if (v != v) return 0x7fffffff;
    return b >= 0 ? b : (b ^ 0x7fffffff);
}
__host__ __device__ inline float argmax_value(int key) {
    int b = key == 0x7fffffff ? 0x7fc00000 : (key >= 0 ? key : (key ^ 0x7fffffff));
    float v;
    __builtin_memcpy(&v, &b, 4);
    return v;
}
__host__ __device__ inline bool argmax_better(float ov, int oi, float bv, int bi) {
    const int ok = argmax_key(ov), bk = argmax_key(bv);
    return ok > bk || (ok == bk && oi < bi);
}

struct ConvArgs {
    const float* in = nullptr;
    int in_ctot = 0, in_coff = 0;
    int cin = 0, cin_pad = 0;
    int up_in = 0;
    const float* pre_scale = nullptr;
    const float* pre_shift = nullptr;
    int B = 0, H = 0, W = 0;
    const float* w = nullptr;
    int cout = 0, cout_pad = 0, ksize = 3;
    int wino4_pad = 0;
    const float* bias = nullptr;
    const float* post_scale = nullptr;
    const float* post_shift = nullptr;
    const float* res1 = nullptr;
    int res1_ctot = 0, res1_coff = 0;
    const float* res2 = nullptr;
    int res2_ctot = 0, res2_coff = 0;
    float* out_raw = nullptr;
    int raw_ctot = 0, raw_coff = 0;
    float* out = nullptr;
    int out_ctot = 0, out_coff = 0;
    int up_out = 0;
    int sub_y = 0, sub_x = 0;
    int n_par = 1;
    const float* w_par[4] = {nullptr, nullptr, nullptr, nullptr};
    int amax_par_stride = 0;
    const float* skip = nullptr;
    int skip_ctot = 0, skip_coff = 0;
    const float* in2 = nullptr;
    int in2_ctot = 0;
    int kparts = 1;
    float* kws = nullptr;
    unsigned* kcnt = nullptr;
    float* amax_val = nullptr;
    int* amax_idx = nullptr;
    int amax_parts = 0;
    int amax_part0 = 0;
    float* pool_out = nullptr;
    int pool_ctot = 0, pool_coff = 0;
    float fast_unscale = 1.f;
    int pool_hint = 0;
    unsigned* fast_ovf = nullptr;
    const float* w_wino4 = nullptr;
    unsigned long long* timing = nullptr;
    const float* w_wino = nullptr;
};
static_assert(sizeof(ConvArgs) == 360 && offsetof(ConvArgs, wino4_pad) == 84 && offsetof(ConvArgs, bias) == 88 && offsetof(ConvArgs, fast_ovf) == 328 &&
                  offsetof(ConvArgs, timing) == 344,
              "ConvArgs is passed to the kernels by value: moving a field changes the device code of every convolution kernel");

struct ConvWino4Pad {
    const float* w = nullptr;
    const float* bias = nullptr;
};

struct ConvProfileRec {
    int slot, variant;
    double flops;
    hipEvent_t e0, e1;
    short shape[6] = {0, 0, 0, 0, 0, 0};
};

struct ConvOverride {
    short ksize, cin_pad, cout_pad, size, kind;
    int variant;
};
struct ConvKey {
    short ksize, cin_pad, cout_pad, size, kind, batch;
};

struct CnnGraphEntry {
    const void* images = nullptr;
    const void* out = nullptr;
    const void* ws = nullptr;
    size_t ws_bytes = 0;
    int nb = 0, view0 = 0, n_total = 0, heat = 0;
    int sel4[4] = {0, 0, 0, 0};
    int uses = 0;
    hipGraphExec_t exec = nullptr;
};

struct WinoForm {
    bool (*serves_slot)(int ksize, int cin_pad, int cout_pad);
    const float* ConvArgs::*weights;
    double macs;
    const char* pack_fn;
};
const WinoForm& mvlm_wino_form(int form);

struct ConvSlotDesc {
    int32_t present, cin, cout, ksize, cin_pad, cout_pad, w_off, bias_off, pre_scale_off, pre_shift_off, post_scale_off, post_shift_off;
};
static_assert(sizeof(ConvSlotDesc) == MVLM_CONV_DESC_INTS * sizeof(int32_t), "a row is the 12 ints of include/mvlm_hip.h");
enum {
    MVLM_SLOT_CONV5 = 1 + 4 * 43,
    MVLM_SLOT_CONV6,
    MVLM_SLOT_CONV7,
    MVLM_SLOT_CONV9,
    MVLM_SLOT_CONV10,
    MVLM_SLOT_CONV11,
    MVLM_SLOT_PARITY0,
    MVLM_N_SLOTS = MVLM_SLOT_PARITY0 + 4,
};
static_assert(MVLM_N_SLOTS == 183, "the descriptor table has 183 conv slots");

struct CnnState {
    bool loaded = false;
    int n_landmarks = 0, in_channels = 0;
    float* blob = nullptr;
    std::vector<ConvSlotDesc> desc;
    bool profiling = false;
    std::vector<ConvProfileRec> prof;
    std::vector<hipEvent_t> event_pool;
    size_t event_cursor = 0;
    hipStream_t side_stream = nullptr;
    hipStream_t capture_stream = nullptr;
    std::vector<hipEvent_t> sync_events;
    size_t sync_cursor = 0;
    int graph_mode = 1;
    int concurrency = 0;
    int selection = 0;
    int pairing = 1;
    unsigned short* fast_blob = nullptr;
    std::vector<long long> fast_off;
    int fast = 0;
    unsigned short* fast16_blob = nullptr;
    std::vector<long long> fast16_off;
    std::vector<float> fast16_unscale;
    unsigned* fast16_flag = nullptr;
    struct WinoWeights {
        float* blob = nullptr;
        std::vector<long long> off;
    } wino[MVLM_WINO_FORMS_N];
    float* wino4_pad_blob = nullptr;
    std::vector<int> wino4_pad_id;
    std::vector<CnnGraphEntry> graphs;
    long graph_replays = 0, graph_captures = 0, eager_runs = 0, graph_failures = 0;
    void drop_graphs() {
        for (CnnGraphEntry& g : graphs)
            if (g.exec) hipGraphExecDestroy(g.exec);
        graphs.clear();
    }
};

struct mvlm_mesh {
    float* verts = nullptr;
    float* uvs = nullptr;
    int32_t* tris = nullptr;
    uint8_t* tex = nullptr;
    uint8_t* colors = nullptr;
    float* normals = nullptr;
    float* normals_buf = nullptr;
    int n_verts = 0, n_tris = 0, tex_h = 0, tex_w = 0;
    double point_radius = 0.0;
    int32_t point_R = 0;
    float point_c = 0.f;
    unsigned long long uid = 0;
    size_t cap[6] = {0, 0, 0, 0, 0, 0};
    hipEvent_t ready = nullptr;
    hipEvent_t waited[6] = {nullptr, nullptr, nullptr, nullptr, nullptr, nullptr};
};

struct RenderProfileRec {
    int n_views, n_verts, n_tris;
    hipEvent_t e0, e1;
};

inline std::string& mvlm_thread_error() {
    thread_local std::string s;
    return s;
}
inline const void*& mvlm_thread_error_ctx() {
    thread_local const void* c = nullptr;
    return c;
}

struct mvlm_ctx;

struct StageClock {
    StageClock() = default;
    StageClock(const StageClock&) = delete;
    StageClock& operator=(const StageClock&) = delete;
    ~StageClock() {
        for (hipEvent_t e : events) hipEventDestroy(e);
    }
    void invalidate() { recorded = 0; }
    int arm(mvlm_ctx* ctx, int n);
    int record(mvlm_ctx* ctx, int k, hipStream_t stream);
    hipEvent_t event(int k) const { return armed ? events[k] : nullptr; }
    void mark(int n) { recorded = armed ? n : 0; }
    int read(mvlm_ctx* ctx, int m, float* ms, const char* none);

private:
    std::vector<hipEvent_t> events;
    int recorded = 0;
    bool armed = false;
};

struct mvlm_ctx {
    int device = 0;
    hipStream_t stream = nullptr;
    hipStream_t launch_stream = nullptr;
    hipStream_t cur_stream() const { return launch_stream ? launch_stream : stream; }
    unsigned long long snap_mesh_uid = 0;
    const void* snap_soup = nullptr;
    const void* snap_vert_tri = nullptr;
    hipEvent_t switch_event = nullptr;
    bool track_order = false;
    bool order_recorded = false;
    std::mutex mu;
    std::string err;
    CnnState cnn;
    std::map<std::string, std::pair<void*, size_t>> scratch;
    float* kparts_ws[2] = {nullptr, nullptr};
    unsigned* kparts_cnt[2] = {nullptr, nullptr};
    int conv_force_variant = -1;
    int conv_winograd = [] { const char* e = getenv("MVLM_WINOGRAD"); return (e && e[0] >= '0' && e[0] <= '2' && !e[1]) ? e[0] - '0' : 1; }();
    int conv_winograd4 = [] { const char* e = getenv("MVLM_WINOGRAD4"); return (e && e[0] >= '0' && e[0] <= '2' && !e[1]) ? e[0] - '0' : 1; }();
    int conv_winograd4_wide = [] { const char* e = getenv("MVLM_WINOGRAD4_WIDE"); return (e && e[0] >= '0' && e[0] <= '1' && !e[1]) ? e[0] - '0' : 1; }();
    long long conv_wino4_wide_launches = 0;
    int conv_winograd4_padded = [] { const char* e = getenv("MVLM_WINOGRAD4_PADDED"); return (e && e[0] >= '0' && e[0] <= '2' && !e[1]) ? e[0] - '0' : 1; }();
    long long conv_wino4_padded_launches = 0;
    std::vector<ConvWino4Pad> conv_wino4_pads = std::vector<ConvWino4Pad>(1);
    std::vector<ConvOverride> conv_overrides;
    unsigned long long conv_attr_mask = 0;
    struct KeyPlaneState {
        const void* ptr = nullptr;
        size_t cap = 0;
    };
    KeyPlaneState raster_keys_clean;
    KeyPlaneState raster_keys4_clean;
    int render_subpixel_bits = 8;
    int render_multisamples = 0;
    int render_shading = 0;
    int* render_overflow_host = nullptr;
    bool points_counting = false;
    bool render_profiling = false;
    std::vector<RenderProfileRec> render_prof;
    std::vector<hipEvent_t> render_events;
    size_t render_event_cursor = 0;
    StageClock points_clock;
    StageClock normals_clock;
    StageClock cloudmesh_clock;
    StageClock view_clock;
    StageClock png_clock;
    StageClock heat_clock;
    StageClock backproject_clock;
    StageClock geodesic_clock;
    int geodesic_groups = 0;
    struct PoolEntry {
        void* p;
        size_t cap;
        hipEvent_t freed;
    };
    std::vector<PoolEntry> mesh_pool;
    size_t mesh_pool_bytes = 0;
    std::mutex upload_mu;
    hipStream_t upload_stream = nullptr;
    void* upload_stage[2] = {nullptr, nullptr};
    size_t upload_stage_cap[2] = {0, 0};
    hipEvent_t upload_stage_done[2] = {nullptr, nullptr};
    int upload_stage_next = 0;
    void* jpeg_scratch = nullptr;
    size_t jpeg_scratch_cap = 0;
    int32_t* jpeg_flags_host = nullptr;
    std::vector<hipEvent_t> event_free;
    hipEvent_t take_event() {
        if (!event_free.empty()) {
            hipEvent_t e = event_free.back();
            event_free.pop_back();
            return e;
        }
        hipEvent_t e = nullptr;
        if (hipEventCreateWithFlags(&e, hipEventDisableTiming) != hipSuccess) return nullptr;
        return e;
    }
    std::mutex err_mu;
    int fail(const std::string& m);
    void* get_scratch(const char* name, size_t bytes);
};

inline int mvlm_ctx::fail(const std::string& m) {
    {
        std::lock_guard<std::mutex> lock(err_mu);
        err = m;
    }
    mvlm_thread_error() = m;
    mvlm_thread_error_ctx() = this;
    return 1;
}

inline int StageClock::arm(mvlm_ctx* ctx, int n) {
    armed = false;
    if (!ctx->render_profiling) return 0;
    while (int(events.size()) < n) {
        hipEvent_t e = nullptr;
        MVLM_CHECK_HIP(ctx, hipEventCreate(&e));
        events.push_back(e);
    }
    armed = true;
    return 0;
}
inline int StageClock::record(mvlm_ctx* ctx, int k, hipStream_t stream) {
    if (armed) MVLM_CHECK_HIP(ctx, hipEventRecord(events[k], stream));
    return 0;
}
inline int StageClock::read(mvlm_ctx* ctx, int m, float* ms, const char* none) {
    if (recorded != m + 1) return ctx->fail(none);
    MVLM_CHECK_HIP(ctx, hipStreamSynchronize(ctx->stream));
    for (int k = 0; k < m; ++k) MVLM_CHECK_HIP(ctx, hipEventElapsedTime(&ms[k], events[k], events[k + 1]));
    return 0;
}

struct MvlmOrderGuard {
    mvlm_ctx* ctx;
    ~MvlmOrderGuard() {
        if (!ctx->track_order || !ctx->switch_event) return;
        if (hipEventRecord(ctx->switch_event, ctx->stream) == hipSuccess)
            ctx->order_recorded = true;
        else
            (void)hipGetLastError();
    }
};

inline int mvlm_mesh_wait_ready(mvlm_ctx* ctx, const mvlm_mesh* m, hipStream_t stream) {
    if (m->ready && hipStreamWaitEvent(stream, m->ready, 0) != hipSuccess) return ctx->fail("mesh: hipStreamWaitEvent failed");
    return 0;
}

int mvlm_jpeg_run(mvlm_ctx* ctx, MvlmJpegPlan& plan, const uint8_t* stage_pinned, uint8_t* rgb_dev, hipStream_t stream,
                  std::string& why, int* rounds_out);

int mvlm_view_sheet_draw(mvlm_ctx* ctx, const float* images_dev, int n_views, const float* maxima_dev, int n_lm, const double* rot_host,
                         const double* landmarks_host, const uint8_t* lm_rgb_host, const uint8_t* used_host, int background, int cols_in,
                         int scale, int gap, double marker_radius, uint8_t* out_dev);

void mvlm_heat_launch_peaks(mvlm_ctx* ctx, const float* heat_dev, int n_planes, float* peaks_dev);

constexpr long MVLM_KPARTS_MAX_TILES = 2048;
constexpr long MVLM_KPARTS_MAX_PARTS = 4096;
int mvlm_conv_kparts_workspace(mvlm_ctx* ctx, float** ws, unsigned** cnt);
int mvlm_launch_conv(mvlm_ctx* ctx, const ConvArgs& a, int* variant_out);
bool mvlm_conv_in2_ok(const mvlm_ctx* ctx, const ConvArgs& a);
bool mvlm_conv_can_pool(const mvlm_ctx* ctx, const ConvArgs& a);
int mvlm_conv_kind(const ConvArgs& a);
ConvKey mvlm_conv_key(const ConvArgs& a);
bool mvlm_conv_variant_can_pool(int variant);
bool mvlm_conv_variant_is_wino(int variant);
bool mvlm_conv_variant_is_wino4(int variant);
int mvlm_conv_wino_variant(const mvlm_ctx* ctx, const ConvArgs& a);
bool mvlm_conv_wino_serves_slot(int ksize, int cin_pad, int cout_pad);
bool mvlm_conv_wino4_serves_slot(int ksize, int cin_pad, int cout_pad);
constexpr int MVLM_CONV_PAIR_FLAG = 0x1000;
int mvlm_conv_pair_variant(const ConvArgs& a0, const ConvArgs& a1, int mode);
int mvlm_launch_conv_pair(mvlm_ctx* ctx, const ConvArgs& a0, const ConvArgs& a1, int pair_variant);
int mvlm_conv_amax_parts(int H, int W);
const char* mvlm_conv_variant_name_impl(int v);

inline int mvlm_fast_cin_pad(int cin) { return (cin + 15) / 16 * 16; }
inline int mvlm_fast_cout_pad(int cout) { return cout <= 32 ? 32 : (cout + 63) / 64 * 64; }
inline bool mvlm_fast_channels_ok(int cin, int cout) {
    return cin >= 16 && cin <= 256 && cout > 0 && cout * 8 >= mvlm_fast_cout_pad(cout) * 5;
}
bool mvlm_conv_fast_ok(const ConvArgs& a, int splits);
int mvlm_launch_conv_fast(mvlm_ctx* ctx, const ConvArgs& a, const unsigned short* wq_dev, int splits = 3, float unscale = 1.f);
constexpr int MVLM_CONV_VARIANT_WINO4 = 2048;
constexpr int MVLM_CONV_WINO4_ATTR_BIT = 41, MVLM_CONV_WINO4_WIDE_ATTR_BIT = 42, MVLM_CONV_FAST_ATTR_BIT0 = 54;
inline bool mvlm_conv_wino4_wide_shape_ok(int cout_pad, int H) { return cout_pad > 0 && cout_pad % 64 == 0 && H % 16 == 0; }
inline bool mvlm_conv_wino4_pad_serves_slot(int ksize, int cin_pad, int cout_pad) {
    return cout_pad > 0 && cout_pad % 32 != 0 && mvlm_conv_wino4_serves_slot(ksize, cin_pad, mvlm_conv_wino4_padded_cout(cout_pad));
}
constexpr int MVLM_CONV_VARIANT_FAST = 62;
constexpr int MVLM_CONV_VARIANT_FAST16 = 61;

int mvlm_launch_landmark_view(mvlm_ctx* ctx, const mvlm_mesh* mesh, const double* rot_host, int n_views, int size,
                              const float* frames_host, const double* landmarks_host, int n_lm, float radius,
                              const uint8_t* lm_rgb_host, uint8_t* out_dev, int32_t* lm_pixels_dev,
                              const uint8_t* vert_rgba_dev = nullptr);

int mvlm_launch_ray_view(mvlm_ctx* ctx, const mvlm_mesh* mesh, const double* rot_host, int n_views, int size,
                         const float* frames_host, const double* landmarks_host, int n_lm, float radius, const uint8_t* lm_rgb_host,
                         const double* starts_dev, const double* ends_dev, int n_rays, float ray_radius, const uint8_t* ray_rgb_host,
                         uint8_t* out_dev, int32_t* lm_pixels_dev, int32_t* ray_pixels_dev);

int mvlm_project_partials(mvlm_ctx* ctx, const mvlm_mesh* mesh, const double* pts_dev, int n_points, int* n_chunks_out,
                          const double** part_d_out, const int** part_t_out);

int mvlm_launch_surface_attach(mvlm_ctx* ctx, const mvlm_mesh* mesh, const double* pts_dev, int n_points, double* snapped_dev,
                               int32_t* tri_dev, double* bary_dev, double* uv_dev);

int mvlm_points_nearest(mvlm_ctx* ctx, const mvlm_mesh* mesh, const double* pts_dev, int n_points, double* out_dev);
extern "C" int mvlm_points_auto_radius(const float* verts, int n, double* r_out);

float* mvlm_mesh_normals_buffer(mvlm_ctx* ctx, mvlm_mesh* mesh);

int mvlm_launch_pack_input(mvlm_ctx* ctx, const float* images, int n, const int* sel4, int c, float* out);
int mvlm_launch_maxpool2(mvlm_ctx* ctx, const float* in, int planes, int H, int W, float* out);
int mvlm_launch_amax_final(mvlm_ctx* ctx, const float* val, const int* idx, int n_img, int view0, int n_views_total,
                           int nl, int parts, int size, float* maxima, int* best_idx = nullptr);
int mvlm_launch_fp16_poison(mvlm_ctx* ctx, const unsigned* flag, float* maxima, int n_img, int view0, int n_views_total, int nl,
                            float* heat);
int mvlm_launch_moment_refine(mvlm_ctx* ctx, const float* x10, int n_img, int nl, int cin_pad, int cout_pad, const float* const w_par[4],
                              const float* bias, const int* best_idx, int view0, int n_views_total, float* maxima);
```

### mvlm_amd/csrc/conv_hooks.hip

```cpp
#include <algorithm>

#include "common.h"
#include "conv_pack.h"

namespace {

struct LayerOffsets {
    long w = 0, bias = -1, pre_scale = -1, pre_shift = -1, post_scale = -1, post_shift = -1;
    ConvPackOffsets forms;
};

struct LayerDims {
    int batch, cin, cin_pad, cout, cout_pad, ksize, h, w;
};

ConvPackTargets forms_served(int ksize, int cin_pad, int cout_pad, std::vector<float>* blob) {
    ConvPackTargets to;
    for (int f = 0; f < MVLM_WINO_FORMS_N; ++f) to.wino[f] = mvlm_wino_form(f).serves_slot(ksize, cin_pad, cout_pad) ? blob : nullptr;
    to.wino4_pad = mvlm_conv_wino4_pad_serves_slot(ksize, cin_pad, cout_pad) ? blob : nullptr;
    return to;
}

ConvArgs layer_args(const float* base, const LayerOffsets& o, const LayerDims& d) {
    auto at = [&](long off) { return off < 0 ? nullptr : base + off; };
    ConvArgs a;
    a.in_ctot = a.cin = d.cin;
    a.cin_pad = d.cin_pad;
    a.B = d.batch;
    a.H = d.h;
    a.W = d.w;
    a.w = at(o.w);
    for (int f = 0; f < MVLM_WINO_FORMS_N; ++f) a.*mvlm_wino_form(f).weights = at(o.forms.wino[f]);
    a.wino4_pad = o.forms.wino4_pad < 0 ? 0 : 1;
    a.cout = a.out_ctot = d.cout;
    a.cout_pad = d.cout_pad;
    a.ksize = d.ksize;
    a.bias = at(o.bias);
    a.pre_scale = at(o.pre_scale);
    a.pre_shift = at(o.pre_shift);
    a.post_scale = at(o.post_scale);
    a.post_shift = at(o.post_shift);
    return a;
}

void set_tensors(ConvArgs& a, const float* in, const float* res, float* raw, float* out) {
    a.in = in;
    a.out = out;
    a.res1 = res;
    a.out_raw = raw;
    if (res) a.res1_ctot = a.cout;
    if (raw) a.raw_ctot = a.cout;
}

ConvWino4Pad wino4_pad_entry(const float* base, const ConvPackOffsets& o) {
    return {o.wino4_pad < 0 ? nullptr : base + o.wino4_pad, o.wino4_pad_bias < 0 ? nullptr : base + o.wino4_pad_bias};
}

template <class Launch>
int timed_launches(mvlm_ctx* ctx, const std::string& who, int iters, Launch launch, int* first, float* ms_per_launch) {
    int rc = launch(first);
    hipEvent_t e0 = nullptr, e1 = nullptr;
    if (!rc && (hipEventCreate(&e0) != hipSuccess || hipEventCreate(&e1) != hipSuccess)) rc = ctx->fail(who + ": hipEventCreate failed");
    if (!rc) {
        hipEventRecord(e0, ctx->stream);
        for (int i = 0; i < iters && !rc; ++i) rc = launch(nullptr);
        hipEventRecord(e1, ctx->stream);
        if (!rc && hipEventSynchronize(e1) != hipSuccess) rc = ctx->fail(who + ": kernel failed");
        float ms = 0.f;
        if (!rc) hipEventElapsedTime(&ms, e0, e1);
        *ms_per_launch = ms / iters;
    }
    if (e0) hipEventDestroy(e0);
    if (e1) hipEventDestroy(e1);
    return rc;
}

size_t round4(size_t n) { return (n + 3) / 4 * 4; }

}

extern "C" int mvlm_conv_force_variant(mvlm_ctx* ctx, int variant) {
    MVLM_ENTER(ctx);
    ctx->conv_force_variant = variant < 0 ? -1 : variant;
    return 0;
}

extern "C" int mvlm_conv2d(mvlm_ctx* ctx, const float* x_dev, int batch, int cin, int h, int w, const float* w_host,
                           int cout, int ksize, const float* bias_host, const float* pre_scale_host,
                           const float* pre_shift_host, const float* post_scale_host, const float* post_shift_host,
                           const float* r_dev, int upsample_in, float* y_dev) {
    MVLM_ENTER(ctx);
    MVLM_REQUIRE(ctx, x_dev && w_host && y_dev, "conv2d: null pointer");
    MVLM_REQUIRE(ctx, ksize == 1 || ksize == 3, "conv2d: kernel size must be 1 or 3");
    MVLM_REQUIRE(ctx, (pre_scale_host == nullptr) == (pre_shift_host == nullptr), "conv2d: pre scale/shift come in pairs");
    MVLM_REQUIRE(ctx, (post_scale_host == nullptr) == (post_shift_host == nullptr), "conv2d: post scale/shift come in pairs");
    const ConvPadding pad = mvlm_conv_hook_padding(
        MVLM_HOOK_CONV2D, {ksize, cin, cout, bias_host != nullptr, pre_scale_host != nullptr, post_scale_host != nullptr, r_dev != nullptr, upsample_in != 0, w, h});
    const int cin_pad = pad.cin_pad, cout_pad = pad.cout_pad;
    const ConvPackSizes sizes = mvlm_conv_pack_sizes(ksize, cin_pad, cout_pad);
    std::vector<float> blob;
    blob.reserve(round4(sizes.w) + round4(sizes.wino[0]) + round4(sizes.wino[1]) + round4(sizes.wino4_pad) + round4(sizes.wino4_pad_bias) +
                 2 * round4(size_t(cin_pad)) + 3 * round4(size_t(cout_pad)));
    auto push = [&](size_t n) {
        const size_t off = blob.size();
        blob.resize(off + round4(n), 0.f);
        return long(off);
    };
    auto vec = [&](const float* src, int n, int n_pad) -> long {
        if (!src) return -1;
        const long off = push(size_t(n_pad));
        std::copy(src, src + n, blob.begin() + off);
        return off;
    };
    LayerOffsets o;
    o.w = push(sizes.w);
    mvlm_conv_pack_transpose(w_host, cout, cin, ksize, cin_pad, cout_pad, blob.data() + o.w);
    o.bias = vec(bias_host, cout, cout_pad);
    o.pre_scale = vec(pre_scale_host, cin, cin_pad);
    o.pre_shift = vec(pre_shift_host, cin, cin_pad);
    o.post_scale = vec(post_scale_host, cout, cout_pad);
    o.post_shift = vec(post_shift_host, cout, cout_pad);
    o.forms = mvlm_conv_pack_forms(forms_served(ksize, cin_pad, cout_pad, &blob), blob.data() + o.w, o.bias < 0 ? nullptr : blob.data() + o.bias, cin_pad, cout_pad);
    auto* d = static_cast<float*>(ctx->get_scratch("conv2d.blob", blob.size() * 4));
    MVLM_REQUIRE(ctx, d, "conv2d: scratch allocation failed");
    MVLM_CHECK_HIP(ctx, hipMemcpy(d, blob.data(), blob.size() * 4, hipMemcpyHostToDevice));
    ConvArgs a = layer_args(d, o, {batch, cin, cin_pad, cout, cout_pad, ksize, h, w});
    set_tensors(a, x_dev, r_dev, nullptr, y_dev);
    a.up_in = upsample_in;
    ctx->conv_wino4_pads[0] = wino4_pad_entry(d, o.forms);
    if (mvlm_launch_conv(ctx, a, nullptr)) return 1;
    MVLM_CHECK_HIP(ctx, hipStreamSynchronize(ctx->stream));
    return 0;
}

extern "C" int mvlm_conv_bench(mvlm_ctx* ctx, int batch, int cin, int cout, int ksize, int size, int flags, int variant,
                               int iters, float* ms_per_launch, int* variant_used) {
    MVLM_ENTER(ctx);
    MVLM_REQUIRE(ctx, batch > 0 && cin > 0 && cout > 0 && size > 0 && iters > 0 && ms_per_launch, "conv_bench: bad arguments");
    MVLM_REQUIRE(ctx, ksize == 1 || ksize == 3, "conv_bench: kernel size must be 1 or 3");
    const ConvPadding pad = mvlm_conv_hook_padding(
        MVLM_HOOK_CONV_BENCH, {ksize, cin, cout, (flags & 4) != 0, (flags & 1) != 0, (flags & 8) != 0, (flags & 2) != 0, false, size, size});
    const int cin_pad = pad.cin_pad, cout_pad = pad.cout_pad;
    const size_t px = size_t(batch) * size * size;
    const size_t n_w = mvlm_conv_pack_arena_floats(ksize, cin_pad, cout_pad), n_vec = size_t(cin_pad) * 2 + size_t(cout_pad) * 3;
    const size_t n_x = px * cin, n_y = px * cout;
    const size_t total = n_w + n_vec + n_x + 3 * n_y + 64;
    auto* base = static_cast<float*>(ctx->get_scratch("conv_bench", total * sizeof(float)));
    MVLM_REQUIRE(ctx, base, "conv_bench: scratch allocation failed");
    MVLM_CHECK_HIP(ctx, hipMemsetAsync(base, 0, total * sizeof(float), ctx->stream));
    const long vec = long(n_w);
    float* x = base + vec + round4(n_vec);
    float* y = x + round4(n_x);
    float* raw = y + round4(n_y);
    float* res = raw + round4(n_y);
    std::vector<float> none;
    const ConvPackTargets which = forms_served(ksize, cin_pad, cout_pad, &none);
    LayerOffsets o;
    for (int f = 0; f < MVLM_WINO_FORMS_N; ++f) o.forms.wino[f] = which.wino[f] ? 0 : -1;
    if (which.wino4_pad) {
        o.forms.wino4_pad = 0;
        o.forms.wino4_pad_bias = vec + 2 * cin_pad;
    }
    if (flags & 1) {
        o.pre_scale = vec;
        o.pre_shift = vec + cin_pad;
    }
    if (flags & 4) o.bias = vec + 2 * cin_pad;
    if (flags & 8) {
        o.post_scale = vec + 2 * cin_pad + cout_pad;
        o.post_shift = vec + 2 * cin_pad + 2 * cout_pad;
    }
    ConvArgs a = layer_args(base, o, {batch, cin, cin_pad, cout, cout_pad, ksize, size, size});
    ctx->conv_wino4_pads[0] = wino4_pad_entry(base, o.forms);
    set_tensors(a, x, (flags & 2) ? res : nullptr, (flags & 2) ? raw : nullptr, y);
    const int saved = ctx->conv_force_variant;
    ctx->conv_force_variant = variant >= 0 ? variant : (variant == -2 ? -2 : -1);
    int used = -1;
    unsigned short* wq = nullptr;
    const int splits = variant == MVLM_CONV_VARIANT_FAST ? 3 : (variant == MVLM_CONV_VARIANT_FAST16 ? 2 : 0);
    if (splits) {
        a.cin_pad = (cin + 15) / 16 * 16;
        a.cout_pad = mvlm_fast_cout_pad(cout);
        const size_t n16 = size_t(a.cin_pad / 16) * 9 * 2 * splits * a.cout_pad * 8;
        wq = static_cast<unsigned short*>(ctx->get_scratch("conv_bench.wq", n16 * 2));
        if (!wq || !mvlm_conv_fast_ok(a, splits)) {
            ctx->conv_force_variant = saved;
            return ctx->fail("conv_bench: shape not eligible for the fast kernel");
        }
        (void)hipMemsetAsync(wq, 0, n16 * 2, ctx->stream);
    }
    auto launch = [&](int* v) { return wq ? mvlm_launch_conv_fast(ctx, a, wq, splits, 1.f) : mvlm_launch_conv(ctx, a, v); };
    const int rc = timed_launches(ctx, "conv_bench", iters, launch, &used, ms_per_launch);
    ctx->conv_force_variant = saved;
    if (variant_used) *variant_used = used;
    return rc;
}

extern "C" int mvlm_conv2d_pair(mvlm_ctx* ctx, int batch, int cin, int cout, const float* x0_dev, int size0, const float* w0_host,
                                const float* r0_dev, float* raw0_dev, float* y0_dev, const float* x1_dev, int size1,
                                const float* w1_host, const float* r1_dev, float* raw1_dev, float* y1_dev,
                                const float* pre_scale_host, const float* pre_shift_host, int variant) {
    MVLM_ENTER(ctx);
    MVLM_REQUIRE(ctx, x0_dev && x1_dev && w0_host && w1_host && y0_dev && y1_dev && variant >= 0, "conv2d_pair: bad arguments");
    MVLM_REQUIRE(ctx, (pre_scale_host == nullptr) == (pre_shift_host == nullptr), "conv2d_pair: pre scale/shift come in pairs");
    const ConvPadding pad = mvlm_conv_hook_padding(MVLM_HOOK_PAIR, {3, cin, cout});
    const int cin_pad = pad.cin_pad, cout_pad = pad.cout_pad;
    const size_t n_w = round4(mvlm_conv_pack_sizes(3, cin_pad, cout_pad).w);
    std::vector<float> blob(2 * n_w + 2 * size_t(cin_pad), 0.f);
    const float* ws[2] = {w0_host, w1_host};
    for (int i = 0; i < 2; ++i) mvlm_conv_pack_transpose(ws[i], cout, cin, 3, cin_pad, cout_pad, blob.data() + i * n_w);
    if (pre_scale_host) {
        std::copy(pre_scale_host, pre_scale_host + cin, blob.begin() + 2 * n_w);
        std::copy(pre_shift_host, pre_shift_host + cin, blob.begin() + 2 * n_w + cin_pad);
    }
    auto* d = static_cast<float*>(ctx->get_scratch("conv2d.blob", blob.size() * 4));
    MVLM_REQUIRE(ctx, d, "conv2d_pair: scratch allocation failed");
    MVLM_CHECK_HIP(ctx, hipMemcpy(d, blob.data(), blob.size() * 4, hipMemcpyHostToDevice));
    ConvArgs a[2];
    const float* xs[2] = {x0_dev, x1_dev};
    const float* rs[2] = {r0_dev, r1_dev};
    float* raws[2] = {raw0_dev, raw1_dev};
    float* ys[2] = {y0_dev, y1_dev};
    const int sizes[2] = {size0, size1};
    for (int i = 0; i < 2; ++i) {
        LayerOffsets o;
        o.w = long(i * n_w);
        if (pre_scale_host) {
            o.pre_scale = long(2 * n_w);
            o.pre_shift = long(2 * n_w) + cin_pad;
        }
        a[i] = layer_args(d, o, {batch, cin, cin_pad, cout, cout_pad, 3, sizes[i], sizes[i]});
        set_tensors(a[i], xs[i], rs[i], raws[i], ys[i]);
    }
    if (mvlm_launch_conv_pair(ctx, a[0], a[1], (variant & 0xfff) | MVLM_CONV_PAIR_FLAG)) return 1;
    MVLM_CHECK_HIP(ctx, hipStreamSynchronize(ctx->stream));
    return 0;
}

extern "C" int mvlm_conv_pair_bench(mvlm_ctx* ctx, int batch, int cin, int cout, int size, int flags, int variant, int iters,
                                    float* ms_per_launch) {
    MVLM_ENTER(ctx);
    MVLM_REQUIRE(ctx, batch > 0 && cin > 0 && cout > 0 && size >= 8 && size % 2 == 0 && iters > 0 && ms_per_launch, "conv_pair_bench: bad arguments");
    const ConvPadding pad = mvlm_conv_hook_padding(MVLM_HOOK_PAIR, {3, cin, cout});
    const int cin_pad = pad.cin_pad, cout_pad = pad.cout_pad;
    const size_t n_w = mvlm_conv_pack_sizes(3, cin_pad, cout_pad).w, n_vec = round4(size_t(cin_pad) * 2 + size_t(cout_pad) * 3);
    size_t px[2] = {size_t(batch) * size * size, size_t(batch) * (size / 2) * (size / 2)};
    size_t total = n_w + n_vec + 64;
    for (int i = 0; i < 2; ++i) total += round4(px[i] * cin) + 3 * round4(px[i] * cout);
    auto* base = static_cast<float*>(ctx->get_scratch("conv_bench", total * sizeof(float)));
    MVLM_REQUIRE(ctx, base, "conv_pair_bench: scratch allocation failed");
    MVLM_CHECK_HIP(ctx, hipMemsetAsync(base, 0, total * sizeof(float), ctx->stream));
    LayerOffsets o;
    if (flags & 1) {
        o.pre_scale = long(n_w);
        o.pre_shift = long(n_w) + cin_pad;
    }
    float* cur = base + n_w + n_vec;
    ConvArgs a[2];
    for (int i = 0; i < 2; ++i) {
        const int s = i ? size / 2 : size;
        a[i] = layer_args(base, o, {batch, cin, cin_pad, cout, cout_pad, 3, s, s});
        const size_t n_x = round4(px[i] * cin), n_y = round4(px[i] * cout);
        float* y = cur + n_x;
        set_tensors(a[i], cur, (flags & 2) ? y + 2 * n_y : nullptr, (flags & 2) ? y + n_y : nullptr, y);
        cur = y + 3 * n_y;
    }
    const int saved = ctx->conv_force_variant;
    ctx->conv_force_variant = -1;
    auto launch = [&](int*) -> int {
        if (variant < 0) return mvlm_launch_conv(ctx, a[0], nullptr) || mvlm_launch_conv(ctx, a[1], nullptr);
        return mvlm_launch_conv_pair(ctx, a[0], a[1], (variant & 0xfff) | MVLM_CONV_PAIR_FLAG);
    };
    const int rc = timed_launches(ctx, "conv_pair_bench", iters, launch, nullptr, ms_per_launch);
    ctx->conv_force_variant = saved;
    return rc;
}
```

### mvlm_amd/csrc/conv_mfma.hip

```cpp
#include <algorithm>
#include <array>
#include <cstdlib>
#include <map>
#include <mutex>
#include <string>
#include <tuple>
#include <vector>

#include "common.h"
#include "conv_cfg.h"
#include "conv_variants.h"
#include "conv_tuned.h"
#include "conv_tuned_net.h"
#include "conv_pair_tuned.h"
#include "conv_tuned_wino.h"
#include "conv_tuned_wino4.h"
#include "conv_wino4_wide_hold.h"
#include "conv_tuned_wino4_pad.h"

#define X(id, name, ...)                                         \
    int mvlm_conv_launch_##id(mvlm_ctx* ctx, const ConvArgs& a); \
    int mvlm_conv_pair_launch_##id(mvlm_ctx* ctx, const ConvArgs& a0, const ConvArgs& a1);
MVLM_CONV_VARIANTS(X)
#undef X
int mvlm_conv_launch_wino4_narrow(mvlm_ctx* ctx, const ConvArgs& a);
int mvlm_conv_launch_wino4_wide(mvlm_ctx* ctx, const ConvArgs& a);

const WinoForm& mvlm_wino_form(int form) {
    static const WinoForm forms[MVLM_WINO_FORMS_N] = {
        {mvlm_conv_wino_serves_slot, &ConvArgs::w_wino, 6.0, "mvlm_pack_winograd_weights"},
        {mvlm_conv_wino4_serves_slot, &ConvArgs::w_wino4, 4.5, "mvlm_pack_winograd4_weights"},
    };
    return forms[form];
}

namespace {

struct ConvVariantInfo {
    int id;
    const char* name;
    int KS, TW, TRI, NIMG, COUT_T, CK, PIX_T, NT, BN_MAXC;
    int form;
    bool SPLITK, TAIL16, PAIRABLE, CAN_POOL_ANY, HAS_IN2;
    int (*launch)(mvlm_ctx*, const ConvArgs&);
    int (*launch_pair)(mvlm_ctx*, const ConvArgs&, const ConvArgs&);
};
constexpr int MAX_VARIANT_ID = 64;

template <int ID, class V>
constexpr ConvVariantInfo variant_info(const char* name, int (*launch)(mvlm_ctx*, const ConvArgs&),
                                       int (*launch_pair)(mvlm_ctx*, const ConvArgs&, const ConvArgs&)) {
    static_assert(ID == MVLM_CONV_VARIANT_WINO4 || (ID >= 0 && ID < MVLM_CONV_FAST_ATTR_BIT0 && ID != MVLM_CONV_WINO4_ATTR_BIT && ID != MVLM_CONV_WINO4_WIDE_ATTR_BIT),
                  "base ids are below the fast kernels' attribute bits and leave the F(4,3) tile's two free");
    static_assert((ID == MVLM_CONV_VARIANT_WINO4) == V::WINO4, "the F(4,3) tile has the code of its own, and nothing else has");
    return {ID, name, V::KS, V::TW, V::TRI, V::NIMG, V::COUT_T, V::CK, V::PIX_T, V::NT, V::BN_MAXC,
            V::WINO ? MVLM_WINO_F23 : V::WINO4 ? MVLM_WINO_F43 : -1, V::SPLITK, V::TAIL16, V::PAIRABLE, V::CAN_POOL_ANY, V::HAS_IN2, launch, launch_pair};
}

constexpr ConvVariantInfo VARIANTS[] = {
#define X(id, name, ...) variant_info<id, __VA_ARGS__>(name, mvlm_conv_launch_##id, mvlm_conv_pair_launch_##id),
    MVLM_CONV_VARIANTS(X)
#undef X
    variant_info<MVLM_CONV_VARIANT_WINO4, MVLM_CONV_WINO4_CFG>(MVLM_CONV_WINO4_NAME, mvlm_conv_launch_wino4_narrow, nullptr),
};

const ConvVariantInfo* conv_variant(int id) {
    static const std::array<const ConvVariantInfo*, MAX_VARIANT_ID> by_id = [] {
        std::array<const ConvVariantInfo*, MAX_VARIANT_ID> t{};
        for (const ConvVariantInfo& v : VARIANTS)
            if (v.id < MAX_VARIANT_ID) t[size_t(v.id)] = &v;
        return t;
    }();
    if (id == MVLM_CONV_VARIANT_WINO4) return &VARIANTS[sizeof VARIANTS / sizeof VARIANTS[0] - 1];
    return id >= 0 && id < MAX_VARIANT_ID ? by_id[size_t(id)] : nullptr;
}

struct VariantCode {
    const ConvVariantInfo* row;
    int kparts;
};
VariantCode decode_variant(int v) {
    if (v == MVLM_CONV_VARIANT_WINO4) return {conv_variant(v), 1};
    if (v >= 0 && v < 1024) return {conv_variant(v & 255), 1 << (v >> 8)};
    return {nullptr, 0};
}
const ConvVariantInfo* variant_row(int v) { return conv_variant(v == MVLM_CONV_VARIANT_WINO4 ? v : v & 255); }

bool tile_fits(const ConvVariantInfo& t, int ksize, int cin_pad, int cout_pad, int H, int W) {
    return ksize == t.KS && W % t.TW == 0 && H % t.TRI == 0 && cout_pad % t.COUT_T == 0 && cin_pad % t.CK == 0 &&
           (!t.SPLITK || cin_pad % 32 == 0);
}

template <class E, class Lead, class LeadOf>
const E* tuned_entry(const E* table, int n, const Lead& lead, short batch, LeadOf lead_of) {
    const E* end = table + n;
    const E* it = std::lower_bound(table, end, std::make_pair(lead, batch),
                                   [&](const E& e, const std::pair<Lead, short>& key) { return std::make_pair(lead_of(e), e.batch) < key; });
    return it != end && lead_of(*it) == lead ? it : nullptr;
}

const ConvOverride* find_override(const mvlm_ctx* ctx, const ConvKey& k) {
    if (ctx)
        for (const ConvOverride& o : ctx->conv_overrides)
            if (o.ksize == k.ksize && o.cin_pad == k.cin_pad && o.cout_pad == k.cout_pad && o.size == k.size && o.kind == k.kind) return &o;
    return nullptr;
}

constexpr long SPLITK_MAX_PIXELS = 8192;

int pick_variant_rules(const ConvArgs& a) {
    if (a.ksize == 1) return (a.W >= 32 && a.cout_pad % 128 == 0) ? 4 : -1;
    if (a.ksize == 2) return (a.W >= 32 && a.H % 8 == 0) ? (a.cout_pad == 96 ? 11 : a.cout_pad == 80 ? 17 : a.cout_pad == 84 ? 29 : -1) : -1;
    if (a.cout_pad == 80) return (a.W >= 32 && a.H % 8 == 0) ? 16 : -1;
    if (a.cout_pad % 32 == 20)
        return (a.cout_pad == 84 && a.W >= 32 && a.H % 8 == 0 && !a.amax_val && !a.up_out) ? 26 : -1;
    const long px = long(a.B) * a.H * a.W;
    const bool sk = a.cin_pad % 32 == 0 && px <= SPLITK_MAX_PIXELS && !a.amax_val;
    if (a.W == 32 && sk) return 15;
    if (a.W >= 32) {
        if (a.cout_pad % 128 == 0) {
            const long blocks = px / 256 * (a.cout_pad / 128);
            return (blocks < 512 && !a.amax_val) ? 8 : 0;
        }
        if (a.cout_pad % 96 == 0) return 1;
        if (a.cout_pad % 64 == 0) {
            const long blocks = px / 256 * (a.cout_pad / 64);
            return blocks < 768 ? 9 : 10;
        }
        return (a.H % 16 == 0) ? 3 : -1;
    }
    if (a.W == 16) return sk ? 12 : (a.cin_pad % 16 == 0 ? 5 : -1);
    if (a.W == 8) return sk ? 13 : (a.cin_pad % 16 == 0 ? 6 : -1);
    if (a.W == 4) return sk ? 14 : (a.cin_pad % 16 == 0 ? 7 : -1);
    return -1;
}

int pick_variant(const mvlm_ctx* ctx, const ConvArgs& a, bool rules_only = false) {
    const int by_rule = pick_variant_rules(a);
    if (rules_only || a.amax_val || a.up_in || a.up_out == 2 || a.ksize == 2 || a.H != a.W) return by_rule;
    const ConvKey k = mvlm_conv_key(a);
    if (const ConvOverride* o = find_override(ctx, k)) return o->variant;
    const auto shape = std::make_tuple(k.ksize, k.cin_pad, k.cout_pad, k.size);
    if (const ConvTunedNet* e = tuned_entry(MVLM_CONV_TUNED_NET, MVLM_CONV_TUNED_NET_N, std::tuple_cat(shape, std::make_tuple(k.kind)), k.batch,
                                            [](const ConvTunedNet& e) { return std::make_tuple(e.ksize, e.cin_pad, e.cout_pad, e.size, e.kind); }))
        return e->variant;
    if (const ConvTuned* e = tuned_entry(MVLM_CONV_TUNED, MVLM_CONV_TUNED_N, shape, k.batch,
                                         [](const ConvTuned& e) { return std::make_tuple(e.ksize, e.cin_pad, e.cout_pad, e.size); }))
        return e->variant;
    return by_rule;
}

int wino_candidate(const ConvArgs& a, int form) {
    if (a.ksize != 3 || a.up_in || a.in2 || a.amax_val || a.up_out == 2 || a.n_par != 1 || a.H != a.W) return -1;
    for (const ConvVariantInfo& t : VARIANTS)
        if (t.form == form && tile_fits(t, a.ksize, a.cin_pad, a.cout_pad, a.H, a.W) && a.cin_pad <= t.BN_MAXC) return t.id;
    return -1;
}

bool form_serves_slot(int form, int ksize, int cin_pad, int cout_pad, bool bn_bound) {
    for (const ConvVariantInfo& t : VARIANTS)
        if (t.form == form && tile_fits(t, ksize, cin_pad, cout_pad, t.TRI, t.TW) && (!bn_bound || cin_pad <= t.BN_MAXC)) return true;
    return false;
}

template <class E>
const E* shape_kind_row(const E* table, int n, int cin_pad, int cout_pad, int size, int kind) {
    for (int i = 0; i < n; ++i)
        if (table[i].cin_pad == cin_pad && table[i].cout_pad == cout_pad && table[i].size == size && table[i].kind == kind) return &table[i];
    return nullptr;
}

template <class E>
int wino_table_variant(const E* table, int n, const ConvKey& k) {
    const E* e = shape_kind_row(table, n, k.cin_pad, k.cout_pad, k.size, k.kind);
    return e && k.batch >= e->min_batch ? e->variant : -1;
}

enum class F43Plan { none, narrow, wide, padded };

F43Plan f43_plan(const mvlm_ctx* ctx, const ConvArgs& a, const ConvVariantInfo& t, int kparts) {
    const int kind = mvlm_conv_kind(a);
    if (t.form == MVLM_WINO_F43) {
        const bool wide = ctx->conv_winograd4_wide && mvlm_conv_wino4_wide_shape_ok(a.cout_pad, a.H) &&
                          !shape_kind_row(MVLM_CONV_WINO4_WIDE_HOLD, MVLM_CONV_WINO4_WIDE_HOLD_N, a.cin_pad, a.cout_pad, a.H, kind);
        return wide ? F43Plan::wide : F43Plan::narrow;
    }
    if (t.form >= 0 || !t.TAIL16 || t.KS != 3) return F43Plan::none;
    if (a.wino4_pad <= 0 || size_t(a.wino4_pad) > ctx->conv_wino4_pads.size()) return F43Plan::none;
    const ConvWino4Pad& pad = ctx->conv_wino4_pads[size_t(a.wino4_pad) - 1];
    if (!pad.w || (a.bias && !pad.bias)) return F43Plan::none;
    if (a.ksize != 3 || a.up_in || a.in2 || a.amax_val || a.res1 || a.res2 || a.post_scale || a.out_raw || a.pool_out || a.up_out || !a.out || a.n_par != 1 ||
        kparts > 1 || a.H != a.W || a.H % 16 != 0 || a.cin_pad > 256)
        return F43Plan::none;
    if (ctx->conv_force_variant >= 0) return F43Plan::none;
    if (ctx->conv_winograd == 0 || ctx->conv_winograd4 == 0 || ctx->conv_winograd4_padded == 0) return F43Plan::none;
    if (ctx->conv_winograd4_padded == 2) return F43Plan::padded;
    const ConvTunedWino4Pad* e = shape_kind_row(MVLM_CONV_TUNED_WINO4_PAD, MVLM_CONV_TUNED_WINO4_PAD_N, a.cin_pad, a.cout_pad, a.H, kind);
    return e && a.B >= e->min_batch ? F43Plan::padded : F43Plan::none;
}

}

ConvKey mvlm_conv_key(const ConvArgs& a) {
    return {short(a.ksize), short(a.cin_pad), short(a.cout_pad), short(a.H), short(mvlm_conv_kind(a)), short(a.B > 32767 ? 32767 : a.B)};
}

bool mvlm_conv_variant_is_wino(int v) {
    const ConvVariantInfo* t = conv_variant(v);
    return t && t->form == MVLM_WINO_F23;
}

bool mvlm_conv_variant_is_wino4(int v) {
    const ConvVariantInfo* t = conv_variant(v);
    return t && t->form == MVLM_WINO_F43;
}

bool mvlm_conv_wino4_serves_slot(int ksize, int cin_pad, int cout_pad) { return form_serves_slot(MVLM_WINO_F43, ksize, cin_pad, cout_pad, true); }

bool mvlm_conv_wino_serves_slot(int ksize, int cin_pad, int cout_pad) { return form_serves_slot(MVLM_WINO_F23, ksize, cin_pad, cout_pad, false); }

int mvlm_conv_wino_variant(const mvlm_ctx* ctx, const ConvArgs& a) {
    const int cand = wino_candidate(a, MVLM_WINO_F23);
    const int cand4 = a.w_wino4 ? wino_candidate(a, MVLM_WINO_F43) : -1;
    if (cand < 0 && cand4 < 0) return -1;
    const ConvKey k = mvlm_conv_key(a);
    if (const ConvOverride* o = find_override(ctx, k))
        return ((cand >= 0 && mvlm_conv_variant_is_wino(o->variant)) || (cand4 >= 0 && mvlm_conv_variant_is_wino4(o->variant))) ? o->variant : -1;
    const int mode = ctx ? ctx->conv_winograd : 1;
    if (mode == 0) return -1;
    const int mode4 = ctx ? ctx->conv_winograd4 : 1;
    if (cand4 >= 0 && mode4 == 2) return cand4;
    if (cand4 >= 0 && mode4 == 1 && mode == 1) {
        const int v = wino_table_variant(MVLM_CONV_TUNED_WINO4, MVLM_CONV_TUNED_WINO4_N, k);
        if (v >= 0) return v;
    }
    if (cand < 0) return -1;
    return mode == 2 ? cand : wino_table_variant(MVLM_CONV_TUNED_WINO, MVLM_CONV_TUNED_WINO_N, k);
}

static int route_variant(const mvlm_ctx* ctx, const ConvArgs& a) {
    const int w = mvlm_conv_wino_variant(ctx, a);
    return w >= 0 ? w : pick_variant(ctx, a);
}

int mvlm_conv_kparts_workspace(mvlm_ctx* ctx, float** ws, unsigned** cnt) {
    const int which = (ctx->launch_stream && ctx->launch_stream == ctx->cnn.side_stream) ? 1 : 0;
    if (!ctx->kparts_ws[0]) {
        for (int i = 0; i < 2; ++i) {
            MVLM_CHECK_HIP(ctx, hipMalloc(&ctx->kparts_ws[i], size_t(MVLM_KPARTS_MAX_PARTS) * 1024 * sizeof(float)));
            MVLM_CHECK_HIP(ctx, hipMalloc(&ctx->kparts_cnt[i], size_t(MVLM_KPARTS_MAX_TILES) * sizeof(unsigned)));
            MVLM_CHECK_HIP(ctx, hipMemset(ctx->kparts_cnt[i], 0, size_t(MVLM_KPARTS_MAX_TILES) * sizeof(unsigned)));
        }
    }
    *ws = ctx->kparts_ws[which];
    *cnt = ctx->kparts_cnt[which];
    return 0;
}

const char* mvlm_conv_variant_name_impl(int v) {
    if (const ConvVariantInfo* t = conv_variant(v)) return t->name;
    if (v == MVLM_CONV_VARIANT_FAST) return "conv3x3_bf16x3_t8x32";
    if (v == MVLM_CONV_VARIANT_FAST16) return "conv3x3_f16x2_t8x32";
    if (v >= 256) {
        static std::mutex mu;
        static std::map<int, std::string> names;
        std::lock_guard<std::mutex> lk(mu);
        auto it = names.find(v);
        if (it == names.end()) {
            std::string n = mvlm_conv_variant_name_impl(v & 255);
            if (v & MVLM_CONV_PAIR_FLAG) {
                n += "_pair";
                const int l0 = (v >> 8) & 3, l1 = (v >> 10) & 3;
                if (l0 || l1) n += "_k" + std::to_string(1 << l0) + "k" + std::to_string(1 << l1);
            } else {
                n += "_k" + std::to_string(1 << ((v >> 8) & 3));
            }
            it = names.emplace(v, n).first;
        }
        return it->second.c_str();
    }
    return "?";
}

bool mvlm_conv_in2_ok(const mvlm_ctx* ctx, const ConvArgs& a) {
    if (a.ksize != 3 || a.up_in || a.up_out || a.amax_val || a.in_coff != 0 || (a.H & 1) || a.H != a.W) return false;
    if (ctx && ctx->conv_force_variant != -1) return false;
    return route_variant(ctx, a) == 0;
}

int mvlm_conv_kind(const ConvArgs& a) { return a.up_out == 1 ? 1 : ((a.pool_out || a.pool_hint) ? 2 : 0); }

bool mvlm_conv_can_pool(const mvlm_ctx* ctx, const ConvArgs& a_in) {
    if (a_in.up_out || a_in.amax_val || (a_in.H & 1) || (a_in.W & 1)) return false;
    ConvArgs a = a_in;
    a.pool_hint = 1;
    return mvlm_conv_variant_can_pool((ctx && ctx->conv_force_variant >= 0) ? ctx->conv_force_variant : route_variant(ctx, a));
}

bool mvlm_conv_variant_can_pool(int v) {
    const ConvVariantInfo* t = variant_row(v);
    return t && t->CAN_POOL_ANY;
}

namespace {
bool pair_variant_serves(int v, const ConvArgs& a) {
    const ConvVariantInfo* t = conv_variant(v);
    return t && t->PAIRABLE && tile_fits(*t, a.ksize, a.cin_pad, a.cout_pad, a.H, a.W);
}
}

int mvlm_conv_pair_variant(const ConvArgs& a0, const ConvArgs& a1, int mode) {
    if (mode <= 0) return -1;
    for (const ConvArgs* a : {&a0, &a1})
        if (a->ksize != 3 || a->amax_val || a->up_in || a->up_out == 2 || a->n_par != 1 || a->H != a->W) return -1;
    if (a0.B != a1.B) return -1;
    if (mode == 2) {
        for (int cand : {pick_variant(nullptr, a0), pick_variant(nullptr, a1), pick_variant_rules(a0), pick_variant_rules(a1)}) {
            if (cand < 0) continue;
            const int base = cand & 255, lg = cand >> 8;
            if (pair_variant_serves(base, a0) && pair_variant_serves(base, a1)) return base | (lg << 8) | (lg << 10) | MVLM_CONV_PAIR_FLAG;
        }
        return -1;
    }
    if (a0.cin_pad != a1.cin_pad || a0.cout_pad != a1.cout_pad || a0.H != 2 * a1.H) return -1;
    const ConvKey k = mvlm_conv_key(a0);
    const ConvPairTuned* e = tuned_entry(MVLM_CONV_PAIR_TUNED, MVLM_CONV_PAIR_TUNED_N, std::make_tuple(k.cin_pad, k.cout_pad, k.size), k.batch,
                                         [](const ConvPairTuned& e) { return std::make_tuple(e.cin_pad, e.cout_pad, e.size); });
    if (!e || e->variant < 0) return -1;
    const int v = e->variant;
    if (!pair_variant_serves(v & 255, a0) || !pair_variant_serves(v & 255, a1)) return -1;
    for (const ConvArgs* a : {&a0, &a1})
        if (a->pool_hint && !mvlm_conv_variant_can_pool(v) && mvlm_conv_can_pool(nullptr, *a)) return -1;
    return v | MVLM_CONV_PAIR_FLAG;
}

int mvlm_launch_conv_pair(mvlm_ctx* ctx, const ConvArgs& a0, const ConvArgs& a1, int pair_variant) {
    MVLM_REQUIRE(ctx, pair_variant >= 0 && (pair_variant & MVLM_CONV_PAIR_FLAG) && pair_variant < 2 * MVLM_CONV_PAIR_FLAG, "conv: not a pair variant");
    ConvArgs b[2] = {a0, a1};
    for (int i = 0; i < 2; ++i) {
        const ConvArgs& a = b[i];
        MVLM_REQUIRE(ctx, a.in && a.w && a.B > 0 && a.H > 0 && a.W > 0 && a.H == a.W, "conv: null input / weights or bad shape");
        MVLM_REQUIRE(ctx, !a.up_in && a.up_out != 2 && (a.up_out != 1 || a.skip), "conv: a paired launch takes plain or scattering 3x3 convolutions");
        const double px = double(a.B) * a.H * a.W, lim = 4294967295.0;
        MVLM_REQUIRE(ctx, px * a.in_ctot < lim && (!a.out_raw || px * a.raw_ctot < lim) && (!a.res1 || px * a.res1_ctot < lim) &&
                              (!a.res2 || px * a.res2_ctot < lim) && (!a.out || px * a.out_ctot * (a.up_out ? 4 : 1) < lim) &&
                              (a.up_out != 1 || px * a.skip_ctot * 4 < lim) && (!a.pool_out || px / 4 * a.pool_ctot < lim),
                     "conv: a tensor exceeds 32-bit element offsets (lower the batch)");
        MVLM_REQUIRE(ctx, a.out || a.pool_out, "conv: no output requested");
        MVLM_REQUIRE(ctx, !a.pool_out || (mvlm_conv_variant_can_pool(pair_variant) && !(a.H & 1) && !a.up_out), "conv: this pair's kernel variant cannot emit the pooled tensor");
    }
    b[0].kparts = 1 << ((pair_variant >> 8) & 3);
    b[1].kparts = 1 << ((pair_variant >> 10) & 3);
    const ConvVariantInfo* t = conv_variant(pair_variant & 255);
    return t ? t->launch_pair(ctx, b[0], b[1]) : ctx->fail("conv: unreachable variant");
}

int mvlm_conv_amax_parts(int H, int W) {
    return (W / 32) * (H / 8) * 4;
}

int mvlm_launch_conv(mvlm_ctx* ctx, const ConvArgs& a, int* variant_out) {
    MVLM_REQUIRE(ctx, a.in && a.w && a.B > 0 && a.H > 0 && a.W > 0, "conv: null input / weights or empty shape");
    MVLM_REQUIRE(ctx, a.H == a.W, "conv: square feature maps only");
    MVLM_REQUIRE(ctx, !a.up_in || (a.H % 2 == 0), "conv: upsampled input needs even size");
    MVLM_REQUIRE(ctx, a.up_out != 1 || a.skip, "conv: up_out needs a skip tensor");
    MVLM_REQUIRE(ctx, a.ksize != 2 || ((a.sub_y | a.sub_x) & ~1) == 0, "conv: 2x2 window offset must be 0 or 1");
    const double px = double(a.B) * a.H * a.W, lim = 4294967295.0;
    MVLM_REQUIRE(ctx, px * a.in_ctot < lim, "conv: input tensor exceeds 32-bit element offsets (lower the batch)");
    MVLM_REQUIRE(ctx, !a.out_raw || px * a.raw_ctot < lim, "conv: raw output exceeds 32-bit element offsets");
    MVLM_REQUIRE(ctx, !a.res1 || px * a.res1_ctot < lim, "conv: residual exceeds 32-bit element offsets");
    MVLM_REQUIRE(ctx, !a.res2 || px * a.res2_ctot < lim, "conv: residual exceeds 32-bit element offsets");
    MVLM_REQUIRE(ctx, !a.out || px * a.out_ctot * (a.up_out ? 4 : 1) < lim, "conv: output exceeds 32-bit element offsets");
    MVLM_REQUIRE(ctx, a.up_out != 1 || px * a.skip_ctot * 4 < lim, "conv: skip tensor exceeds 32-bit element offsets");
    const int v = ctx->conv_force_variant >= 0 ? ctx->conv_force_variant
                  : ctx->conv_force_variant == -2 ? pick_variant(ctx, a, true) : route_variant(ctx, a);
    MVLM_REQUIRE(ctx, v >= 0, "conv: no kernel variant for this shape");
    const VariantCode d = decode_variant(v);
    const WinoForm* form = d.row && d.row->form >= 0 ? &mvlm_wino_form(d.row->form) : nullptr;
    MVLM_REQUIRE(ctx, !form || a.*form->weights, std::string("conv: a Winograd tile needs the layer's transformed weights (") + form->pack_fn + ")");
    MVLM_REQUIRE(ctx, !a.in2 || v == 0, "conv: a second input tensor needs the 128-channel 8x32 tile (ask mvlm_conv_in2_ok first)");
    MVLM_REQUIRE(ctx, !a.in2 || px / 4 * a.in2_ctot < lim, "conv: second input exceeds 32-bit element offsets");
    MVLM_REQUIRE(ctx, !a.pool_out || mvlm_conv_variant_can_pool(v), "conv: this shape's kernel variant cannot emit the pooled tensor");
    MVLM_REQUIRE(ctx, !a.pool_out || px / 4 * a.pool_ctot < lim, "conv: pooled output exceeds 32-bit element offsets");
    MVLM_REQUIRE(ctx, !form || !a.amax_val || a.out || a.pool_out, "conv: a Winograd tile has no fused argmax, and no other output is requested");
    MVLM_REQUIRE(ctx, a.out || a.pool_out || a.amax_val, "conv: no output requested");
    if (variant_out) *variant_out = v;
    MVLM_REQUIRE(ctx, d.kparts > 0, "conv: unknown kernel variant");
    ConvArgs b = a;
    b.kparts = d.kparts;
    if (form) b.w = a.*form->weights;
    if (!d.row) return ctx->fail("conv: unreachable variant");
    switch (f43_plan(ctx, a, *d.row, d.kparts)) {
    case F43Plan::wide:
        if (mvlm_conv_launch_wino4_wide(ctx, b)) return 1;
        ++ctx->conv_wino4_wide_launches;
        return 0;
    case F43Plan::padded: {
        const ConvWino4Pad& pad = ctx->conv_wino4_pads[size_t(a.wino4_pad) - 1];
        b.w = pad.w;
        b.bias = a.bias ? pad.bias : nullptr;
        b.cout_pad = mvlm_conv_wino4_padded_cout(a.cout_pad);
        if (mvlm_conv_launch_wino4_narrow(ctx, b)) return 1;
        ++ctx->conv_wino4_padded_launches;
        if (variant_out) *variant_out = MVLM_CONV_VARIANT_WINO4;
        return 0;
    }
    default: return d.row->launch(ctx, b);
    }
}

extern "C" int mvlm_conv_variant_serves(int variant, int ksize, int cin_pad, int cout_pad, int size, int kind) {
    const VariantCode d = decode_variant(variant);
    const ConvVariantInfo* t = d.row;
    if (!t || ksize != 3 || kind < 0 || kind > 2 || !tile_fits(*t, ksize, cin_pad, cout_pad, size, size)) return 0;
    const int parts = d.kparts;
    const bool residual_block_tile = !t->TAIL16 && t->COUT_T != 96;
    const bool bn_fits = t->form < 0 || cin_pad <= t->BN_MAXC;
    const bool parts_ok = parts == 1 || (t->SPLITK && t->PIX_T == 32 && cin_pad % (parts * t->CK) == 0);
    return residual_block_tile && bn_fits && parts_ok;
}

extern "C" int mvlm_conv_wino4_wide_serves(int ksize, int cin_pad, int cout_pad, int size) {
    return mvlm_conv_variant_serves(MVLM_CONV_VARIANT_WINO4, ksize, cin_pad, cout_pad, size, 0) && mvlm_conv_wino4_wide_shape_ok(cout_pad, size);
}

extern "C" int mvlm_conv_set_override(mvlm_ctx* ctx, int ksize, int cin_pad, int cout_pad, int size, int kind, int variant) {
    MVLM_ENTER(ctx);
    auto& ov = ctx->conv_overrides;
    if (ksize == 0) {
        ov.clear();
    } else {
        const ConvKey k = {short(ksize), short(cin_pad), short(cout_pad), short(size), short(kind), 0};
        const bool fits = k.ksize == ksize && k.cin_pad == cin_pad && k.cout_pad == cout_pad && k.size == size && k.kind == kind;
        while (const ConvOverride* o = fits ? find_override(ctx, k) : nullptr) ov.erase(ov.begin() + (o - ov.data()));
        if (variant >= 0) {
            MVLM_REQUIRE(ctx, mvlm_conv_variant_serves(variant, ksize, cin_pad, cout_pad, size, kind), "conv_set_override: the variant cannot serve this shape");
            ov.push_back({k.ksize, k.cin_pad, k.cout_pad, k.size, k.kind, variant});
        }
    }
    ctx->cnn.drop_graphs();
    return 0;
}
```

### mvlm_amd/csrc/conv_pack.cpp

```cpp
#include "conv_pack.h"

#include <algorithm>
#include <cassert>
#include <functional>

#include "../../include/mvlm_hip.h"

void mvlm_winograd_transform(const float* w9, int cin_pad, int cout_pad, float* w12) {
    const size_t n = size_t(cin_pad) * cout_pad;
    for (int kx = 0; kx < 3; ++kx)
        for (size_t i = 0; i < n; ++i) {
            const double g0 = w9[size_t(kx) * n + i], g1 = w9[size_t(3 + kx) * n + i], g2 = w9[size_t(6 + kx) * n + i];
            w12[size_t(kx) * n + i] = float(g0);
            w12[size_t(3 + kx) * n + i] = float((g0 + g1 + g2) * 0.5);
            w12[size_t(6 + kx) * n + i] = float((g0 - g1 + g2) * 0.5);
            w12[size_t(9 + kx) * n + i] = float(g2);
        }
}

void mvlm_winograd4_transform(const float* w9, int cin_pad, int cout_pad, float* w18) {
    const size_t n = size_t(cin_pad) * cout_pad;
    for (int kx = 0; kx < 3; ++kx)
        for (size_t i = 0; i < n; ++i) {
            const double g0 = w9[size_t(kx) * n + i], g1 = w9[size_t(3 + kx) * n + i], g2 = w9[size_t(6 + kx) * n + i];
            w18[size_t(kx) * n + i] = float(g0);
            w18[size_t(3 + kx) * n + i] = float(0.0 - (g0 + g1 + g2) / 3.0);
            w18[size_t(6 + kx) * n + i] = float((g0 - g1 + g2) / 3.0);
            w18[size_t(9 + kx) * n + i] = float((g0 + 2.0 * g1 + 4.0 * g2) / 15.0);
            w18[size_t(12 + kx) * n + i] = float((-16.0 * g0 + 8.0 * g1 - 4.0 * g2) / 15.0);
            w18[size_t(15 + kx) * n + i] = float(g2);
        }
}

void mvlm_winograd4_pack_padded(const float* w9, const float* bias, int cin_pad, int cout_pad, float* w18_pad, float* bias_pad) {
    const int P = mvlm_conv_wino4_padded_cout(cout_pad);
    const size_t rows = size_t(18) * cin_pad;
    std::vector<float> w18(rows * cout_pad);
    mvlm_winograd4_transform(w9, cin_pad, cout_pad, w18.data());
    for (size_t r = 0; r < rows; ++r) {
        std::copy(w18.begin() + r * cout_pad, w18.begin() + (r + 1) * cout_pad, w18_pad + r * P);
        std::fill(w18_pad + r * P + cout_pad, w18_pad + (r + 1) * P, 0.f);
    }
    if (bias && bias_pad) {
        std::copy(bias, bias + cout_pad, bias_pad);
        std::fill(bias_pad + cout_pad, bias_pad + P, 0.f);
    }
}

extern "C" int mvlm_pack_winograd_weights(const float* w9_host, int cin_pad, int cout_pad, float* w12_host) {
    if (!w9_host || !w12_host || cin_pad <= 0 || cout_pad <= 0) return 1;
    mvlm_winograd_transform(w9_host, cin_pad, cout_pad, w12_host);
    return 0;
}

extern "C" int mvlm_pack_winograd4_weights(const float* w9_host, int cin_pad, int cout_pad, float* w18_host) {
    if (!w9_host || !w18_host || cin_pad <= 0 || cout_pad <= 0) return 1;
    mvlm_winograd4_transform(w9_host, cin_pad, cout_pad, w18_host);
    return 0;
}

extern "C" int mvlm_conv_wino4_padded_stride(int cout_pad) { return cout_pad > 0 ? mvlm_conv_wino4_padded_cout(cout_pad) : 0; }

extern "C" int mvlm_pack_winograd4_weights_padded(const float* w9_host, const float* bias_host, int cin_pad, int cout_pad, float* w18_pad_host,
                                                  float* bias_pad_host) {
    if (!w9_host || !w18_pad_host || cin_pad <= 0 || cout_pad <= 0 || (bias_host && !bias_pad_host)) return 1;
    mvlm_winograd4_pack_padded(w9_host, bias_host, cin_pad, cout_pad, w18_pad_host, bias_pad_host);
    return 0;
}

void mvlm_conv_pack_transpose(const float* w_oihw, int cout, int cin, int ksize, int cin_pad, int cout_pad, float* out) {
    const int taps = ksize * ksize;
    for (int co = 0; co < cout; ++co)
        for (int ci = 0; ci < cin; ++ci)
            for (int t = 0; t < taps; ++t) out[(size_t(t) * cin_pad + ci) * cout_pad + co] = w_oihw[(size_t(co) * cin + ci) * taps + t];
}

ConvPackSizes mvlm_conv_pack_sizes(int ksize, int cin_pad, int cout_pad) {
    const size_t n = size_t(cin_pad) * cout_pad;
    ConvPackSizes s;
    s.w = size_t(ksize) * ksize * n;
    if (ksize != 3) return s;
    s.wino[MVLM_WINO_F23] = 12 * n;
    s.wino[MVLM_WINO_F43] = 18 * n;
    s.wino4_pad_bias = size_t(mvlm_conv_wino4_padded_cout(cout_pad));
    s.wino4_pad = size_t(18) * cin_pad * s.wino4_pad_bias;
    return s;
}

ConvPackOffsets mvlm_conv_pack_forms(const ConvPackTargets& to, const float* w9, const float* bias, int cin_pad, int cout_pad) {
    const ConvPackSizes sizes = mvlm_conv_pack_sizes(3, cin_pad, cout_pad);
    const std::less<const float*> before;
    auto push = [&](std::vector<float>* blob, size_t n) -> long {
        if (!blob) return -1;
        const float* const was = blob->data();
        const bool holds_w9 = !blob->empty() && !before(w9, was) && before(w9, was + blob->size());
        const size_t off = (blob->size() + 3) / 4 * 4;
        blob->resize(off + n, 0.f);
        assert((!holds_w9 || blob->data() == was) && "sources inside a blob: the caller reserves the room, so it does not move");
        (void)holds_w9;
        return long(off);
    };
    ConvPackOffsets o;
    for (int f = 0; f < MVLM_WINO_FORMS_N; ++f) o.wino[f] = push(to.wino[f], sizes.wino[f]);
    o.wino4_pad = push(to.wino4_pad, sizes.wino4_pad);
    if (o.wino4_pad >= 0 && bias) o.wino4_pad_bias = push(to.wino4_pad, sizes.wino4_pad_bias);
    if (o.wino[MVLM_WINO_F23] >= 0) mvlm_winograd_transform(w9, cin_pad, cout_pad, to.wino[MVLM_WINO_F23]->data() + o.wino[MVLM_WINO_F23]);
    if (o.wino[MVLM_WINO_F43] >= 0) mvlm_winograd4_transform(w9, cin_pad, cout_pad, to.wino[MVLM_WINO_F43]->data() + o.wino[MVLM_WINO_F43]);
    if (o.wino4_pad >= 0)
        mvlm_winograd4_pack_padded(w9, bias, cin_pad, cout_pad, to.wino4_pad->data() + o.wino4_pad, o.wino4_pad_bias < 0 ? nullptr : to.wino4_pad->data() + o.wino4_pad_bias);
    return o;
}

size_t mvlm_conv_pack_arena_floats(int ksize, int cin_pad, int cout_pad) {
    const ConvPackSizes s = mvlm_conv_pack_sizes(ksize, cin_pad, cout_pad);
    const size_t longest = std::max({s.w, s.wino[MVLM_WINO_F23], s.wino[MVLM_WINO_F43], s.wino4_pad});
    return std::max(longest, size_t(ksize) * ksize * cin_pad * mvlm_conv_wino4_padded_cout(cout_pad));
}

ConvPadding mvlm_conv_hook_padding(ConvHookSite site, const ConvHookLayer& l) {
    const bool plain = !l.pre && !l.post && !l.residual, rows32 = l.w >= 32 && l.h % 8 == 0;
    bool strip16 = false, exact84 = false;
    switch (site) {
    case MVLM_HOOK_CONV2D:
        strip16 = l.ksize == 3 && plain && rows32;
        exact84 = strip16 && l.bias && !l.upsample_in;
        break;
    case MVLM_HOOK_CONV_BENCH:
        strip16 = plain && l.bias;
        exact84 = strip16 && l.ksize == 3;
        break;
    case MVLM_HOOK_PAIR: break;
    }
    const int cout16 = (l.cout + 15) / 16 * 16;
    return {l.ksize == 1 ? (l.cin + 7) / 8 * 8 : (l.cin + 3) / 4 * 4,
            strip16 && cout16 == 80 ? 80 : exact84 && l.cout == 84 ? 84 : (l.cout + 31) / 32 * 32};
}
```

### mvlm_amd/csrc/conv_pack.h

```cpp
#pragma once
#include <cstddef>
#include <vector>

enum { MVLM_WINO_F23 = 0, MVLM_WINO_F43 = 1, MVLM_WINO_FORMS_N = 2 };

inline int mvlm_conv_wino4_padded_cout(int cout_pad) { return (cout_pad + 31) / 32 * 32; }

void mvlm_winograd_transform(const float* w9, int cin_pad, int cout_pad, float* w12);
void mvlm_winograd4_transform(const float* w9, int cin_pad, int cout_pad, float* w18);
void mvlm_winograd4_pack_padded(const float* w9, const float* bias, int cin_pad, int cout_pad, float* w18_pad, float* bias_pad);

void mvlm_conv_pack_transpose(const float* w_oihw, int cout, int cin, int ksize, int cin_pad, int cout_pad, float* out);

struct ConvPackTargets {
    std::vector<float>* wino[MVLM_WINO_FORMS_N] = {nullptr, nullptr};
    std::vector<float>* wino4_pad = nullptr;
};
struct ConvPackOffsets {
    long wino[MVLM_WINO_FORMS_N] = {-1, -1};
    long wino4_pad = -1, wino4_pad_bias = -1;
};
struct ConvPackSizes {
    size_t w = 0, wino[MVLM_WINO_FORMS_N] = {0, 0}, wino4_pad = 0, wino4_pad_bias = 0;
};
ConvPackSizes mvlm_conv_pack_sizes(int ksize, int cin_pad, int cout_pad);

ConvPackOffsets mvlm_conv_pack_forms(const ConvPackTargets& to, const float* w9, const float* bias, int cin_pad, int cout_pad);

size_t mvlm_conv_pack_arena_floats(int ksize, int cin_pad, int cout_pad);

enum ConvHookSite { MVLM_HOOK_CONV2D, MVLM_HOOK_CONV_BENCH, MVLM_HOOK_PAIR };
struct ConvHookLayer {
    int ksize, cin, cout;
    bool bias = false, pre = false, post = false, residual = false, upsample_in = false;
    int w = 0, h = 0;
};
struct ConvPadding {
    int cin_pad, cout_pad;
};
ConvPadding mvlm_conv_hook_padding(ConvHookSite site, const ConvHookLayer& l);
```

Baseline: 1377 views/s.

## Add 2-D Winograd F(4x2,3x3) conv kernel for 3x3 layers with 64-multiple cout

Adds a new convolution kernel that applies a two-dimensional Winograd transform (4x2 output tiles) to 3x3 layers whose padded output channels are multiples of 64 and whose square feature maps are multiples of 64. It pre-packs the transformed weights into a new device blob, keeps the BatchNorm pre-scale table in LDS, double-buffers input and weight chunks, and remaps block ids across XCDs. Selection goes through a measured lookup table and is on by default through an environment knob. The aim is fewer multiplies per output than the 1-D Winograd forms. The cost is a large LDS footprint that limits each CU to one workgroup, plus extra weight memory.

```diff
diff --git a/include/mvlm_hip.h b/include/mvlm_hip.h
--- a/include/mvlm_hip.h
+++ b/include/mvlm_hip.h
@@ -150,6 +150,11 @@
 int mvlm_conv_wino4_padded_stride(int cout_pad);
 int mvlm_pack_winograd4_weights_padded(const float* w9_host, const float* bias_host, int cin_pad, int cout_pad, float* w18_pad_host,
                                        float* bias_pad_host);
+int mvlm_cnn_set_winograd4_2d(mvlm_ctx* ctx, int on);
+int mvlm_conv_wino4_2d_force(mvlm_ctx* ctx, int on);
+int mvlm_conv_wino4_2d_serves(int ksize, int cin_pad, int cout_pad, int size, int kind);
+int mvlm_conv_wino4_2d_launches(mvlm_ctx* ctx, int64_t* count, int reset);
+int mvlm_pack_winograd4_2d_weights(const float* w9_host, int cin_pad, int cout_pad, float* w24_host);
 int mvlm_cnn_execution_stats(mvlm_ctx* ctx, int64_t* eager_runs, int64_t* graph_captures, int64_t* graph_replays,
                              int64_t* graph_failures);
 size_t mvlm_pack_fast_weights(const float* w, int cout, int cin, int cout_pad, int cin_pad, uint16_t* out);
diff --git a/mvlm_amd/_lib.py b/mvlm_amd/_lib.py
--- a/mvlm_amd/_lib.py
+++ b/mvlm_amd/_lib.py
@@ -118,6 +118,11 @@
     "mvlm_conv_wino4_padded_launches": (C.c_int, [C.c_void_p, C.POINTER(C.c_int64), C.c_int]),
     "mvlm_conv_wino4_padded_stride": (C.c_int, [C.c_int]),
     "mvlm_pack_winograd4_weights_padded": (C.c_int, [c_float_p, c_float_p, C.c_int, C.c_int, c_float_p, c_float_p]),
+    "mvlm_cnn_set_winograd4_2d": (C.c_int, [C.c_void_p, C.c_int]),
+    "mvlm_conv_wino4_2d_force": (C.c_int, [C.c_void_p, C.c_int]),
+    "mvlm_conv_wino4_2d_serves": (C.c_int, [C.c_int, C.c_int, C.c_int, C.c_int, C.c_int]),
+    "mvlm_conv_wino4_2d_launches": (C.c_int, [C.c_void_p, C.POINTER(C.c_int64), C.c_int]),
+    "mvlm_pack_winograd4_2d_weights": (C.c_int, [c_float_p, C.c_int, C.c_int, c_float_p]),
     "mvlm_cnn_execution_stats": (C.c_int, [C.c_void_p, C.POINTER(C.c_int64), C.POINTER(C.c_int64), C.POINTER(C.c_int64),
                                           C.POINTER(C.c_int64)]),
     "mvlm_pack_fast_weights": (C.c_size_t, [c_float_p, C.c_int, C.c_int, C.c_int, C.c_int, C.POINTER(C.c_uint16)]),
diff --git a/mvlm_amd/csrc/api.hip b/mvlm_amd/csrc/api.hip
--- a/mvlm_amd/csrc/api.hip
+++ b/mvlm_amd/csrc/api.hip
@@ -58,6 +58,7 @@
     for (auto& ww : ctx->cnn.wino)
         if (ww.blob) hipFree(ww.blob);
     if (ctx->cnn.wino4_pad_blob) hipFree(ctx->cnn.wino4_pad_blob);
+    if (ctx->cnn.wino4_2d_blob) hipFree(ctx->cnn.wino4_2d_blob);
     if (ctx->cnn.fast16_flag) hipFree(ctx->cnn.fast16_flag);
     if (ctx->switch_event) hipEventDestroy(ctx->switch_event);
     for (int i = 0; i < 2; ++i) {
diff --git a/mvlm_amd/csrc/cnn_graph.hip b/mvlm_amd/csrc/cnn_graph.hip
--- a/mvlm_amd/csrc/cnn_graph.hip
+++ b/mvlm_amd/csrc/cnn_graph.hip
@@ -177,8 +177,10 @@
         hipEventRecord(e0, ctx->cur_stream());
         return 0;
     }
+    static constexpr int MVLM_CONV_FLOPS_WINO4_2D = -36;
     static double conv_flops(const ConvArgs& a, int variant = -1) {
-        const double taps = mvlm_conv_variant_is_wino(variant) ? mvlm_wino_form(MVLM_WINO_F23).macs
+        const double taps = variant == MVLM_CONV_FLOPS_WINO4_2D ? 3.0
+                            : mvlm_conv_variant_is_wino(variant) ? mvlm_wino_form(MVLM_WINO_F23).macs
                             : mvlm_conv_variant_is_wino4(variant) ? mvlm_wino_form(MVLM_WINO_F43).macs : double(a.ksize * a.ksize);
         return 2.0 * a.cin * a.cout * taps * double(a.H) * a.W * a.B * a.n_par;
     }
@@ -202,7 +204,7 @@
         }
         if (st.profiling) {
             hipEventRecord(e1, ctx->cur_stream());
-            ConvProfileRec rec{slot, variant, conv_flops(a, variant), e0, e1};
+            ConvProfileRec rec{slot, variant, conv_flops(a, ctx->conv_last_launch_wino4_2d ? MVLM_CONV_FLOPS_WINO4_2D : variant), e0, e1};
             const ConvKey key = mvlm_conv_key(a);
             const short shape[6] = {key.ksize, key.cin_pad, key.cout_pad, key.size, key.kind, key.batch};
             for (int i = 0; i < 6; ++i) rec.shape[i] = shape[i];
@@ -780,7 +782,7 @@
         (void)hipFree(st.fast16_blob);
         st.fast16_blob = nullptr;
     }
-    float** const form_blobs[MVLM_WINO_FORMS_N + 1] = {&st.wino[MVLM_WINO_F23].blob, &st.wino[MVLM_WINO_F43].blob, &st.wino4_pad_blob};
+    float** const form_blobs[MVLM_WINO_FORMS_N + 2] = {&st.wino[MVLM_WINO_F23].blob, &st.wino[MVLM_WINO_F43].blob, &st.wino4_pad_blob, &st.wino4_2d_blob};
     for (float** b : form_blobs)
         if (*b) {
             (void)hipFree(*b);
@@ -809,9 +811,10 @@
     MVLM_REQUIRE(ctx, st.desc[MVLM_SLOT_CONV11].cout == n_landmarks, "cnn_load: conv11 output channels != n_landmarks");
     MVLM_CHECK_HIP(ctx, hipMalloc(&st.blob, n_floats * sizeof(float)));
     MVLM_CHECK_HIP(ctx, hipMemcpy(st.blob, blob_host, n_floats * sizeof(float), hipMemcpyHostToDevice));
-    std::vector<float> host[MVLM_WINO_FORMS_N + 1];
+    constexpr int N_BLOBS = MVLM_WINO_FORMS_N + 2, PAD_BLOB = MVLM_WINO_FORMS_N, W2D_BLOB = MVLM_WINO_FORMS_N + 1;
+    std::vector<float> host[N_BLOBS];
     std::vector<ConvPackTargets> to(st.desc.size());
-    size_t total[MVLM_WINO_FORMS_N + 1] = {0, 0, 0};
+    size_t total[N_BLOBS] = {0, 0, 0, 0};
     for (int s = 0; s < n_slots; ++s) {
         const ConvSlotDesc& r = st.desc[size_t(s)];
         if (!r.present) continue;
@@ -822,11 +825,15 @@
                 total[f] += sizes.wino[f];
             }
         if (mvlm_conv_wino4_pad_serves_slot(r.ksize, r.cin_pad, r.cout_pad)) {
-            to[size_t(s)].wino4_pad = &host[MVLM_WINO_FORMS_N];
-            total[MVLM_WINO_FORMS_N] += sizes.wino4_pad + sizes.wino4_pad_bias;
-        }
-    }
-    for (int k = 0; k <= MVLM_WINO_FORMS_N; ++k) host[k].reserve(total[k]);
+            to[size_t(s)].wino4_pad = &host[PAD_BLOB];
+            total[PAD_BLOB] += sizes.wino4_pad + sizes.wino4_pad_bias;
+        }
+        if (mvlm_conv_wino4_2d_serves_slot(r.ksize, r.cin_pad, r.cout_pad)) {
+            to[size_t(s)].wino4_2d = &host[W2D_BLOB];
+            total[W2D_BLOB] += sizes.wino4_2d;
+        }
+    }
+    for (int k = 0; k < N_BLOBS; ++k) host[k].reserve(total[k]);
     for (CnnState::WinoWeights& ww : st.wino) ww.off.assign(size_t(n_slots), -1);
     st.wino4_pad_id.assign(size_t(n_slots), 0);
     std::vector<ConvPackOffsets> made(st.desc.size());
@@ -834,7 +841,7 @@
         const ConvSlotDesc& r = st.desc[size_t(s)];
         if (r.present) made[size_t(s)] = mvlm_conv_pack_forms(to[size_t(s)], blob_host + r.w_off, r.bias_off >= 0 ? blob_host + r.bias_off : nullptr, r.cin_pad, r.cout_pad);
     }
-    for (int k = 0; k <= MVLM_WINO_FORMS_N; ++k)
+    for (int k = 0; k < N_BLOBS; ++k)
         if (!host[k].empty()) {
             MVLM_CHECK_HIP(ctx, hipMalloc(form_blobs[k], host[k].size() * sizeof(float)));
             MVLM_CHECK_HIP(ctx, hipMemcpy(*form_blobs[k], host[k].data(), host[k].size() * sizeof(float), hipMemcpyHostToDevice));
@@ -842,8 +849,11 @@
     for (int s = 0; s < n_slots; ++s) {
         const ConvPackOffsets& m = made[size_t(s)];
         for (int f = 0; f < MVLM_WINO_FORMS_N; ++f) st.wino[f].off[size_t(s)] = m.wino[f];
-        if (m.wino4_pad < 0) continue;
-        ctx->conv_wino4_pads.push_back({st.wino4_pad_blob + m.wino4_pad, m.wino4_pad_bias < 0 ? nullptr : st.wino4_pad_blob + m.wino4_pad_bias});
+        if (m.wino4_pad < 0 && m.wino4_2d < 0) continue;
+        ConvWino4Pad entry;
+        if (m.wino4_pad >= 0) entry = {st.wino4_pad_blob + m.wino4_pad, m.wino4_pad_bias < 0 ? nullptr : st.wino4_pad_blob + m.wino4_pad_bias};
+        if (m.wino4_2d >= 0) entry.w2d = st.wino4_2d_blob + m.wino4_2d;
+        ctx->conv_wino4_pads.push_back(entry);
         st.wino4_pad_id[size_t(s)] = int(ctx->conv_wino4_pads.size());
     }
     st.n_landmarks = n_landmarks;
@@ -931,6 +941,29 @@
     MVLM_REQUIRE(ctx, on == 0 || on == 1, "cnn_set_winograd4_wide: 0 the 32 x 16 shape on every launch, 1 the wide shape where the output channels come in 64s (default)");
     if (on != ctx->conv_winograd4_wide) ctx->cnn.drop_graphs();
     ctx->conv_winograd4_wide = on;
+    return 0;
+}
+
+extern "C" int mvlm_cnn_set_winograd4_2d(mvlm_ctx* ctx, int on) {
+    MVLM_ENTER(ctx);
+    MVLM_REQUIRE(ctx, on == 0 || on == 1, "cnn_set_winograd4_2d: 0 never, 1 where the measured table has a row (default)");
+    if (on != ctx->conv_winograd4_2d) ctx->cnn.drop_graphs();
+    ctx->conv_winograd4_2d = on;
+    return 0;
+}
+
+extern "C" int mvlm_conv_wino4_2d_force(mvlm_ctx* ctx, int on) {
+    MVLM_ENTER(ctx);
+    MVLM_REQUIRE(ctx, on == 0 || on == 1, "conv_wino4_2d_force: 0 or 1");
+    if (on != ctx->conv_wino4_2d_force) ctx->cnn.drop_graphs();
+    ctx->conv_wino4_2d_force = on;
+    return 0;
+}
+
+extern "C" int mvlm_conv_wino4_2d_launches(mvlm_ctx* ctx, int64_t* count, int reset) {
+    std::lock_guard<std::mutex> lk(ctx->mu);
+    if (count) *count = ctx->conv_wino4_2d_launches;
+    if (reset) ctx->conv_wino4_2d_launches = 0;
     return 0;
 }
 
diff --git a/mvlm_amd/csrc/common.h b/mvlm_amd/csrc/common.h
--- a/mvlm_amd/csrc/common.h
+++ b/mvlm_amd/csrc/common.h
@@ -107,6 +107,7 @@
 struct ConvWino4Pad {
     const float* w = nullptr;
     const float* bias = nullptr;
+    const float* w2d = nullptr;
 };
 
 struct ConvProfileRec {
@@ -189,6 +190,7 @@
     } wino[MVLM_WINO_FORMS_N];
     float* wino4_pad_blob = nullptr;
     std::vector<int> wino4_pad_id;
+    float* wino4_2d_blob = nullptr;
     std::vector<CnnGraphEntry> graphs;
     long graph_replays = 0, graph_captures = 0, eager_runs = 0, graph_failures = 0;
     void drop_graphs() {
@@ -276,6 +278,10 @@
     long long conv_wino4_wide_launches = 0;
     int conv_winograd4_padded = [] { const char* e = getenv("MVLM_WINOGRAD4_PADDED"); return (e && e[0] >= '0' && e[0] <= '2' && !e[1]) ? e[0] - '0' : 1; }();
     long long conv_wino4_padded_launches = 0;
+    int conv_winograd4_2d = [] { const char* e = getenv("MVLM_WINOGRAD4_2D"); return (e && e[0] >= '0' && e[0] <= '1' && !e[1]) ? e[0] - '0' : 1; }();
+    int conv_wino4_2d_force = 0;
+    long long conv_wino4_2d_launches = 0;
+    bool conv_last_launch_wino4_2d = false;
     std::vector<ConvWino4Pad> conv_wino4_pads = std::vector<ConvWino4Pad>(1);
     std::vector<ConvOverride> conv_overrides;
     unsigned long long conv_attr_mask = 0;
@@ -425,6 +431,12 @@
 inline bool mvlm_conv_wino4_pad_serves_slot(int ksize, int cin_pad, int cout_pad) {
     return cout_pad > 0 && cout_pad % 32 != 0 && mvlm_conv_wino4_serves_slot(ksize, cin_pad, mvlm_conv_wino4_padded_cout(cout_pad));
 }
+constexpr int MVLM_CONV_WINO4_2D_ATTR_BIT = 43;
+inline bool mvlm_conv_wino4_2d_serves_slot(int ksize, int cin_pad, int cout_pad) {
+    return ksize == 3 && cout_pad > 0 && cout_pad % 64 == 0 && cin_pad > 0 && cin_pad % 4 == 0 && cin_pad <= 256;
+}
+inline bool mvlm_conv_wino4_2d_shape_ok(int cin_pad, int cout_pad, int H) { return mvlm_conv_wino4_2d_serves_slot(3, cin_pad, cout_pad) && H > 0 && H % 64 == 0; }
+void mvlm_conv_register_wino4_2d(int (*launch)(mvlm_ctx*, const ConvArgs&));
 constexpr int MVLM_CONV_VARIANT_FAST = 62;
 constexpr int MVLM_CONV_VARIANT_FAST16 = 61;
 
diff --git a/mvlm_amd/csrc/conv_hooks.hip b/mvlm_amd/csrc/conv_hooks.hip
--- a/mvlm_amd/csrc/conv_hooks.hip
+++ b/mvlm_amd/csrc/conv_hooks.hip
@@ -18,6 +18,7 @@
     ConvPackTargets to;
     for (int f = 0; f < MVLM_WINO_FORMS_N; ++f) to.wino[f] = mvlm_wino_form(f).serves_slot(ksize, cin_pad, cout_pad) ? blob : nullptr;
     to.wino4_pad = mvlm_conv_wino4_pad_serves_slot(ksize, cin_pad, cout_pad) ? blob : nullptr;
+    to.wino4_2d = mvlm_conv_wino4_2d_serves_slot(ksize, cin_pad, cout_pad) ? blob : nullptr;
     return to;
 }
 
@@ -31,7 +32,7 @@
     a.W = d.w;
     a.w = at(o.w);
     for (int f = 0; f < MVLM_WINO_FORMS_N; ++f) a.*mvlm_wino_form(f).weights = at(o.forms.wino[f]);
-    a.wino4_pad = o.forms.wino4_pad < 0 ? 0 : 1;
+    a.wino4_pad = (o.forms.wino4_pad < 0 && o.forms.wino4_2d < 0) ? 0 : 1;
     a.cout = a.out_ctot = d.cout;
     a.cout_pad = d.cout_pad;
     a.ksize = d.ksize;
@@ -53,7 +54,7 @@
 }
 
 ConvWino4Pad wino4_pad_entry(const float* base, const ConvPackOffsets& o) {
-    return {o.wino4_pad < 0 ? nullptr : base + o.wino4_pad, o.wino4_pad_bias < 0 ? nullptr : base + o.wino4_pad_bias};
+    return {o.wino4_pad < 0 ? nullptr : base + o.wino4_pad, o.wino4_pad_bias < 0 ? nullptr : base + o.wino4_pad_bias, o.wino4_2d < 0 ? nullptr : base + o.wino4_2d};
 }
 
 template <class Launch>
@@ -99,7 +100,7 @@
     const int cin_pad = pad.cin_pad, cout_pad = pad.cout_pad;
     const ConvPackSizes sizes = mvlm_conv_pack_sizes(ksize, cin_pad, cout_pad);
     std::vector<float> blob;
-    blob.reserve(round4(sizes.w) + round4(sizes.wino[0]) + round4(sizes.wino[1]) + round4(sizes.wino4_pad) + round4(sizes.wino4_pad_bias) +
+    blob.reserve(round4(sizes.w) + round4(sizes.wino[0]) + round4(sizes.wino[1]) + round4(sizes.wino4_pad) + round4(sizes.wino4_pad_bias) + round4(sizes.wino4_2d) +
                  2 * round4(size_t(cin_pad)) + 3 * round4(size_t(cout_pad)));
     auto push = [&](size_t n) {
         const size_t off = blob.size();
@@ -157,6 +158,7 @@
     const ConvPackTargets which = forms_served(ksize, cin_pad, cout_pad, &none);
     LayerOffsets o;
     for (int f = 0; f < MVLM_WINO_FORMS_N; ++f) o.forms.wino[f] = which.wino[f] ? 0 : -1;
+    if (which.wino4_2d) o.forms.wino4_2d = 0;
     if (which.wino4_pad) {
         o.forms.wino4_pad = 0;
         o.forms.wino4_pad_bias = vec + 2 * cin_pad;
diff --git a/mvlm_amd/csrc/conv_inst_x0.hip b/mvlm_amd/csrc/conv_inst_x0.hip
--- /dev/null
+++ b/mvlm_amd/csrc/conv_inst_x0.hip
@@ -0,0 +1,45 @@
+#include "conv_wino4_2d.h"
+
+using W2Cfg = Wino4x2Cfg;
+static_assert(W2Cfg::STAGE == 12288 && W2Cfg::XT == 6144 && W2Cfg::WT == 6144);
+static_assert(W2Cfg::LDS_BYTES == 131072, "the exchange buffer: the two stages and the BatchNorm table are 100 352 bytes");
+static_assert(W2Cfg::LDS_BYTES > 80 * 1024 && W2Cfg::LDS_BYTES <= 160 * 1024, "one workgroup per CU, within its LDS");
+
+namespace {
+
+__global__ __launch_bounds__(256) __attribute__((amdgpu_waves_per_eu(1, 1))) void conv_wino4_2d_kernel(const ConvArgs a, const int tiles_x, const int tiles_y,
+                                                                                                      const int cout_tiles) {
+    wino4x2_tile<W2Cfg>(a, tiles_x, tiles_y, cout_tiles, int(blockIdx.x), int(gridDim.x));
+}
+
+int launch_wino4_2d(mvlm_ctx* ctx, const ConvArgs& a_in) {
+    ConvArgs a = a_in;
+#if defined(MVLM_CONV_TIMING)
+    if (const char* e = getenv("MVLM_CONV_TIMING_BUF")) a.timing = reinterpret_cast<unsigned long long*>(strtoull(e, nullptr, 0));
+#endif
+    MVLM_REQUIRE(ctx, a.ksize == 3 && a.H == a.W, "conv: the 2-D Winograd tile serves 3x3 layers of square feature maps");
+    MVLM_REQUIRE(ctx, !a.up_in && !a.in2 && !a.amax_val && a.up_out != 2 && a.n_par == 1 && a.kparts <= 1 && !a.pool_out,
+                 "conv: the 2-D Winograd tile serves plain and scattering 3x3 layers (no upsampled / second input, no fused argmax, no K parts, no pooled output)");
+    MVLM_REQUIRE(ctx, a.out && (a.up_out != 1 || a.skip), "conv: the 2-D Winograd tile writes an output tensor (scattered: into a skip tensor)");
+    MVLM_REQUIRE(ctx, a.W % W2Cfg::TW == 0 && a.H % W2Cfg::TRI == 0, "conv: spatial size not a multiple of the tile");
+    MVLM_REQUIRE(ctx, a.cout_pad % W2Cfg::COUT_T == 0 && a.cout <= a.cout_pad, "conv: cout_pad not a multiple of the cout tile");
+    MVLM_REQUIRE(ctx, a.cin_pad % W2Cfg::CK == 0 && a.cin_pad >= W2Cfg::CK && a.cin <= a.cin_pad && a.cin > a.cin_pad - W2Cfg::CK,
+                 "conv: cin_pad must be the input channels rounded up to the K-chunk");
+    MVLM_REQUIRE(ctx, a.cin_pad <= W2Cfg::BN_MAXC, "conv: the 2-D Winograd tile keeps a BatchNorm pair of every input channel in LDS (up to 256)");
+    MVLM_REQUIRE(ctx, (reinterpret_cast<size_t>(a.in) & 7) == 0 && (reinterpret_cast<size_t>(a.w) & 15) == 0 && (!a.skip || ((reinterpret_cast<size_t>(a.skip) | reinterpret_cast<size_t>(a.out)) & 7) == 0),
+                 "conv: the 2-D Winograd tile loads aligned column pairs and 16-byte weight quads");
+    const int tiles_x = a.W / W2Cfg::TW, tiles_y = a.H / W2Cfg::TRI, cout_tiles = a.cout_pad / W2Cfg::COUT_T;
+    const long nblk = long(tiles_x) * tiles_y * a.B * cout_tiles;
+    MVLM_REQUIRE(ctx, nblk > 0 && nblk < (1l << 31), "conv: bad grid");
+    if (!((ctx->conv_attr_mask >> MVLM_CONV_WINO4_2D_ATTR_BIT) & 1ull)) {
+        MVLM_CHECK_HIP(ctx, hipFuncSetAttribute(reinterpret_cast<const void*>(conv_wino4_2d_kernel), hipFuncAttributeMaxDynamicSharedMemorySize, int(W2Cfg::LDS_BYTES)));
+        ctx->conv_attr_mask |= 1ull << MVLM_CONV_WINO4_2D_ATTR_BIT;
+    }
+    hipLaunchKernelGGL(conv_wino4_2d_kernel, dim3((unsigned)nblk), dim3(256), W2Cfg::LDS_BYTES, ctx->cur_stream(), a, tiles_x, tiles_y, cout_tiles);
+    MVLM_CHECK_HIP(ctx, hipGetLastError());
+    return 0;
+}
+
+const bool registered = (mvlm_conv_register_wino4_2d(launch_wino4_2d), true);
+
+}
diff --git a/mvlm_amd/csrc/conv_mfma.hip b/mvlm_amd/csrc/conv_mfma.hip
--- a/mvlm_amd/csrc/conv_mfma.hip
+++ b/mvlm_amd/csrc/conv_mfma.hip
@@ -17,6 +17,7 @@
 #include "conv_tuned_wino4.h"
 #include "conv_wino4_wide_hold.h"
 #include "conv_tuned_wino4_pad.h"
+#include "conv_tuned_wino4_2d.h"
 
 #define X(id, name, ...)                                         \
     int mvlm_conv_launch_##id(mvlm_ctx* ctx, const ConvArgs& a); \
@@ -25,6 +26,9 @@
 #undef X
 int mvlm_conv_launch_wino4_narrow(mvlm_ctx* ctx, const ConvArgs& a);
 int mvlm_conv_launch_wino4_wide(mvlm_ctx* ctx, const ConvArgs& a);
+
+static int (*g_launch_wino4_2d)(mvlm_ctx*, const ConvArgs&) = nullptr;
+void mvlm_conv_register_wino4_2d(int (*launch)(mvlm_ctx*, const ConvArgs&)) { g_launch_wino4_2d = launch; }
 
 const WinoForm& mvlm_wino_form(int form) {
     static const WinoForm forms[MVLM_WINO_FORMS_N] = {
@@ -176,11 +180,29 @@
     return e && k.batch >= e->min_batch ? e->variant : -1;
 }
 
-enum class F43Plan { none, narrow, wide, padded };
+enum class F43Plan { none, narrow, wide, padded, two_d };
+
+const float* wino4_2d_weights(const mvlm_ctx* ctx, const ConvArgs& a) {
+    if (a.wino4_pad <= 0 || size_t(a.wino4_pad) > ctx->conv_wino4_pads.size()) return nullptr;
+    return ctx->conv_wino4_pads[size_t(a.wino4_pad) - 1].w2d;
+}
+
+bool wino4_2d_can_serve(const mvlm_ctx* ctx, const ConvArgs& a, int kparts) {
+    return g_launch_wino4_2d && wino4_2d_weights(ctx, a) && mvlm_conv_wino4_2d_shape_ok(a.cin_pad, a.cout_pad, a.H) && a.H == a.W && kparts == 1 &&
+           !a.pool_out && !a.pool_hint && !a.up_in && !a.in2 && !a.amax_val && a.up_out != 2 && a.n_par == 1;
+}
 
 F43Plan f43_plan(const mvlm_ctx* ctx, const ConvArgs& a, const ConvVariantInfo& t, int kparts) {
     const int kind = mvlm_conv_kind(a);
     if (t.form == MVLM_WINO_F43) {
+        if (wino4_2d_can_serve(ctx, a, kparts)) {
+            if (ctx->conv_wino4_2d_force) return F43Plan::two_d;
+            const bool routed = ctx->conv_force_variant == -1 && ctx->conv_winograd == 1 && ctx->conv_winograd4 == 1 && !find_override(ctx, mvlm_conv_key(a));
+            if (routed && ctx->conv_winograd4_2d) {
+                const ConvTunedWino4x2* e = shape_kind_row(MVLM_CONV_TUNED_WINO4_2D, MVLM_CONV_TUNED_WINO4_2D_N, a.cin_pad, a.cout_pad, a.H, kind);
+                if (e && a.B >= e->min_batch) return F43Plan::two_d;
+            }
+        }
         const bool wide = ctx->conv_winograd4_wide && mvlm_conv_wino4_wide_shape_ok(a.cout_pad, a.H) &&
                           !shape_kind_row(MVLM_CONV_WINO4_WIDE_HOLD, MVLM_CONV_WINO4_WIDE_HOLD_N, a.cin_pad, a.cout_pad, a.H, kind);
         return wide ? F43Plan::wide : F43Plan::narrow;
@@ -390,7 +412,14 @@
     b.kparts = d.kparts;
     if (form) b.w = a.*form->weights;
     if (!d.row) return ctx->fail("conv: unreachable variant");
+    ctx->conv_last_launch_wino4_2d = false;
     switch (f43_plan(ctx, a, *d.row, d.kparts)) {
+    case F43Plan::two_d:
+        b.w = wino4_2d_weights(ctx, a);
+        if (g_launch_wino4_2d(ctx, b)) return 1;
+        ++ctx->conv_wino4_2d_launches;
+        ctx->conv_last_launch_wino4_2d = true;
+        return 0;
     case F43Plan::wide:
         if (mvlm_conv_launch_wino4_wide(ctx, b)) return 1;
         ++ctx->conv_wino4_wide_launches;
@@ -424,6 +453,11 @@
     return mvlm_conv_variant_serves(MVLM_CONV_VARIANT_WINO4, ksize, cin_pad, cout_pad, size, 0) && mvlm_conv_wino4_wide_shape_ok(cout_pad, size);
 }
 
+extern "C" int mvlm_conv_wino4_2d_serves(int ksize, int cin_pad, int cout_pad, int size, int kind) {
+    return g_launch_wino4_2d != nullptr && (kind == 0 || kind == 1) && mvlm_conv_variant_serves(MVLM_CONV_VARIANT_WINO4, ksize, cin_pad, cout_pad, size, kind) &&
+           mvlm_conv_wino4_2d_shape_ok(cin_pad, cout_pad, size);
+}
+
 extern "C" int mvlm_conv_set_override(mvlm_ctx* ctx, int ksize, int cin_pad, int cout_pad, int size, int kind, int variant) {
     MVLM_ENTER(ctx);
     auto& ov = ctx->conv_overrides;
diff --git a/mvlm_amd/csrc/conv_pack.cpp b/mvlm_amd/csrc/conv_pack.cpp
--- a/mvlm_amd/csrc/conv_pack.cpp
+++ b/mvlm_amd/csrc/conv_pack.cpp
@@ -47,6 +47,31 @@
     }
 }
 
+void mvlm_winograd4_2d_transform(const float* w9, int cin_pad, int cout_pad, float* w24) {
+    const size_t n = size_t(cin_pad) * cout_pad;
+    for (int ci = 0; ci < cin_pad; ++ci)
+        for (int co = 0; co < cout_pad; ++co) {
+            const size_t i = size_t(ci) * cout_pad + co;
+            double u[6][3];
+            for (int kx = 0; kx < 3; ++kx) {
+                const double g0 = w9[size_t(kx) * n + i], g1 = w9[size_t(3 + kx) * n + i], g2 = w9[size_t(6 + kx) * n + i];
+                u[0][kx] = g0;
+                u[1][kx] = 0.0 - (g0 + g1 + g2) / 3.0;
+                u[2][kx] = (g0 - g1 + g2) / 3.0;
+                u[3][kx] = (g0 + 2.0 * g1 + 4.0 * g2) / 15.0;
+                u[4][kx] = (-16.0 * g0 + 8.0 * g1 - 4.0 * g2) / 15.0;
+                u[5][kx] = g2;
+            }
+            for (int ty = 0; ty < 6; ++ty) {
+                float* const o = w24 + ((size_t(ci) * 6 + ty) * cout_pad + co) * 4;
+                o[0] = float(u[ty][0]);
+                o[1] = float((u[ty][0] + u[ty][1] + u[ty][2]) * 0.5);
+                o[2] = float((u[ty][0] - u[ty][1] + u[ty][2]) * 0.5);
+                o[3] = float(u[ty][2]);
+            }
+        }
+}
+
 extern "C" int mvlm_pack_winograd_weights(const float* w9_host, int cin_pad, int cout_pad, float* w12_host) {
     if (!w9_host || !w12_host || cin_pad <= 0 || cout_pad <= 0) return 1;
     mvlm_winograd_transform(w9_host, cin_pad, cout_pad, w12_host);
@@ -56,6 +81,12 @@
 extern "C" int mvlm_pack_winograd4_weights(const float* w9_host, int cin_pad, int cout_pad, float* w18_host) {
     if (!w9_host || !w18_host || cin_pad <= 0 || cout_pad <= 0) return 1;
     mvlm_winograd4_transform(w9_host, cin_pad, cout_pad, w18_host);
+    return 0;
+}
+
+extern "C" int mvlm_pack_winograd4_2d_weights(const float* w9_host, int cin_pad, int cout_pad, float* w24_host) {
+    if (!w9_host || !w24_host || cin_pad <= 0 || cout_pad <= 0) return 1;
+    mvlm_winograd4_2d_transform(w9_host, cin_pad, cout_pad, w24_host);
     return 0;
 }
 
@@ -84,6 +115,7 @@
     s.wino[MVLM_WINO_F43] = 18 * n;
     s.wino4_pad_bias = size_t(mvlm_conv_wino4_padded_cout(cout_pad));
     s.wino4_pad = size_t(18) * cin_pad * s.wino4_pad_bias;
+    s.wino4_2d = 24 * n;
     return s;
 }
 
@@ -104,16 +136,18 @@
     for (int f = 0; f < MVLM_WINO_FORMS_N; ++f) o.wino[f] = push(to.wino[f], sizes.wino[f]);
     o.wino4_pad = push(to.wino4_pad, sizes.wino4_pad);
     if (o.wino4_pad >= 0 && bias) o.wino4_pad_bias = push(to.wino4_pad, sizes.wino4_pad_bias);
+    o.wino4_2d = push(to.wino4_2d, sizes.wino4_2d);
     if (o.wino[MVLM_WINO_F23] >= 0) mvlm_winograd_transform(w9, cin_pad, cout_pad, to.wino[MVLM_WINO_F23]->data() + o.wino[MVLM_WINO_F23]);
     if (o.wino[MVLM_WINO_F43] >= 0) mvlm_winograd4_transform(w9, cin_pad, cout_pad, to.wino[MVLM_WINO_F43]->data() + o.wino[MVLM_WINO_F43]);
     if (o.wino4_pad >= 0)
         mvlm_winograd4_pack_padded(w9, bias, cin_pad, cout_pad, to.wino4_pad->data() + o.wino4_pad, o.wino4_pad_bias < 0 ? nullptr : to.wino4_pad->data() + o.wino4_pad_bias);
+    if (o.wino4_2d >= 0) mvlm_winograd4_2d_transform(w9, cin_pad, cout_pad, to.wino4_2d->data() + o.wino4_2d);
     return o;
 }
 
 size_t mvlm_conv_pack_arena_floats(int ksize, int cin_pad, int cout_pad) {
     const ConvPackSizes s = mvlm_conv_pack_sizes(ksize, cin_pad, cout_pad);
-    const size_t longest = std::max({s.w, s.wino[MVLM_WINO_F23], s.wino[MVLM_WINO_F43], s.wino4_pad});
+    const size_t longest = std::max({s.w, s.wino[MVLM_WINO_F23], s.wino[MVLM_WINO_F43], s.wino4_pad, s.wino4_2d});
     return std::max(longest, size_t(ksize) * ksize * cin_pad * mvlm_conv_wino4_padded_cout(cout_pad));
 }
 
diff --git a/mvlm_amd/csrc/conv_pack.h b/mvlm_amd/csrc/conv_pack.h
--- a/mvlm_amd/csrc/conv_pack.h
+++ b/mvlm_amd/csrc/conv_pack.h
@@ -9,19 +9,23 @@
 void mvlm_winograd_transform(const float* w9, int cin_pad, int cout_pad, float* w12);
 void mvlm_winograd4_transform(const float* w9, int cin_pad, int cout_pad, float* w18);
 void mvlm_winograd4_pack_padded(const float* w9, const float* bias, int cin_pad, int cout_pad, float* w18_pad, float* bias_pad);
+void mvlm_winograd4_2d_transform(const float* w9, int cin_pad, int cout_pad, float* w24);
 
 void mvlm_conv_pack_transpose(const float* w_oihw, int cout, int cin, int ksize, int cin_pad, int cout_pad, float* out);
 
 struct ConvPackTargets {
     std::vector<float>* wino[MVLM_WINO_FORMS_N] = {nullptr, nullptr};
     std::vector<float>* wino4_pad = nullptr;
+    std::vector<float>* wino4_2d = nullptr;
 };
 struct ConvPackOffsets {
     long wino[MVLM_WINO_FORMS_N] = {-1, -1};
     long wino4_pad = -1, wino4_pad_bias = -1;
+    long wino4_2d = -1;
 };
 struct ConvPackSizes {
     size_t w = 0, wino[MVLM_WINO_FORMS_N] = {0, 0}, wino4_pad = 0, wino4_pad_bias = 0;
+    size_t wino4_2d = 0;
 };
 ConvPackSizes mvlm_conv_pack_sizes(int ksize, int cin_pad, int cout_pad);
 
diff --git a/mvlm_amd/csrc/conv_tuned_wino4_2d.h b/mvlm_amd/csrc/conv_tuned_wino4_2d.h
--- /dev/null
+++ b/mvlm_amd/csrc/conv_tuned_wino4_2d.h
@@ -0,0 +1,10 @@
+#ifndef MVLM_CONV_TUNED_WINO4_2D_H
+#define MVLM_CONV_TUNED_WINO4_2D_H
+struct ConvTunedWino4x2 {
+    short cin_pad, cout_pad, size, kind, min_batch;
+};
+static const ConvTunedWino4x2 MVLM_CONV_TUNED_WINO4_2D[] = {
+    {0, 0, 0, 0, 0},
+};
+static const int MVLM_CONV_TUNED_WINO4_2D_N = 0;
+#endif
diff --git a/mvlm_amd/csrc/conv_wino4_2d.h b/mvlm_amd/csrc/conv_wino4_2d.h
--- /dev/null
+++ b/mvlm_amd/csrc/conv_wino4_2d.h
@@ -0,0 +1,407 @@
+#ifndef MVLM_CONV_WINO4_2D_H
+#define MVLM_CONV_WINO4_2D_H
+#include <type_traits>
+
+#include "common.h"
+
+using f32x16 = __attribute__((ext_vector_type(16))) float;
+using f32x4 = __attribute__((ext_vector_type(4))) float;
+
+namespace {
+
+template <int I, int N, class F>
+__device__ __forceinline__ void static_for(F&& f) {
+    if constexpr (I < N) {
+        f(std::integral_constant<int, I>{});
+        static_for<I + 1, N>(f);
+    }
+}
+
+template <class T>
+__device__ __forceinline__ void wino_opaque(T& v) {
+    asm volatile("" : "+v"(v));
+}
+
+struct Wino4x2Cfg {
+    static constexpr int COUT_T = 64, TW = 64, TRI = 8, CK = 4, BN_MAXC = 256;
+    static constexpr int XT = CK * (TRI / 4) * 24 * (TW / 2), XT_PAD = XT, WT = 24 * CK * COUT_T, STAGE = XT_PAD + WT;
+    static constexpr int ENT = 8;
+    static constexpr int EXCHANGE = 4 * 2 * 16 * 4 * TW;
+    static constexpr size_t LDS_BYTES = size_t(2 * STAGE + 2 * BN_MAXC > EXCHANGE ? 2 * STAGE + 2 * BN_MAXC : EXCHANGE) * 4;
+};
+
+template <class C>
+struct Wino4x2Stage {
+    unsigned off[6];
+    unsigned hoff[6];
+    unsigned m0, m5, mc;
+    unsigned mh0, mh5, mh;
+    unsigned woff;
+    int wlds;
+    int xlds;
+    int bn;
+    int lane_l, lane_r;
+    bool edge_l, edge_r;
+    float2 x[6];
+    float h[6];
+    float v[3][6];
+    float bn_s, bn_t, floor;
+    f32x4 wv[3];
+    int abase, bbase;
+};
+
+constexpr int WINO4X2_LOAD_SLICES = 7, WINO4X2_WORK_SLICES = 23, WINO4X2_FIRST_WORK_GAP = 47 - WINO4X2_WORK_SLICES;
+
+template <class C, int S>
+__device__ __forceinline__ void wino4x2_load_slice(const char* in_cb, const char* w_cb, size_t w_step, const float* sbn, Wino4x2Stage<C>& ws) {
+    if constexpr (S < 3) {
+#pragma unroll
+        for (int r = 2 * S; r < 2 * S + 2; ++r) {
+            wino_opaque(ws.off[r]);
+            ws.x[r] = *reinterpret_cast<const float2*>(in_cb + ws.off[r]);
+        }
+    } else if constexpr (S < 5) {
+#pragma unroll
+        for (int r = 3 * (S - 3); r < 3 * (S - 3) + 3; ++r) {
+            wino_opaque(ws.hoff[r]);
+            ws.h[r] = *reinterpret_cast<const float*>(in_cb + ws.hoff[r]);
+        }
+    } else if constexpr (S == 5) {
+        const float2 st = *reinterpret_cast<const float2*>(sbn + 2 * ws.bn);
+        ws.bn_s = st.x;
+        ws.bn_t = st.y;
+        wino_opaque(ws.woff);
+        ws.wv[0] = *reinterpret_cast<const f32x4*>(w_cb + ws.woff);
+    } else {
+        wino_opaque(ws.woff);
+        ws.wv[1] = *reinterpret_cast<const f32x4*>(w_cb + w_step + ws.woff);
+        ws.wv[2] = *reinterpret_cast<const f32x4*>(w_cb + 2 * w_step + ws.woff);
+    }
+}
+
+template <class C>
+__device__ __forceinline__ float wino4x2_act(float d, unsigned mask, const Wino4x2Stage<C>& ws) {
+    const float v = fmaxf(fmaf(d, ws.bn_s, ws.bn_t), ws.floor);
+    return __uint_as_float(__float_as_uint(v) & mask);
+}
+
+template <int P>
+__device__ __forceinline__ void wino4x2_ypair(float d0, float d1, float d2, float d3, float d4, float d5, float (&v)[6]) {
+    if constexpr (P == 0) {
+        v[0] = fmaf(-1.5f, d3, fmaf(-2.f, d2, fmaf(1.5f, d1, d0))) + d4;
+        v[1] = fmaf(-0.5f, d3, fmaf(-2.5f, d2, -d1)) + d4;
+    } else if constexpr (P == 1) {
+        v[2] = fmaf(-2.5f, d3, fmaf(0.5f, d2, d1)) + d4;
+        v[3] = fmaf(0.5f, d3, fmaf(-0.5f, d1, -d2)) + d4;
+    } else {
+        v[4] = fmaf(-2.f, d3, fmaf(2.f, d1, -d2)) + d4;
+        v[5] = fmaf(-1.5f, d4, fmaf(-2.f, d3, fmaf(1.5f, d2, d1))) + d5;
+    }
+}
+
+template <class C, int S>
+__device__ __forceinline__ void wino4x2_work_slice(float* next, const char* w_cb, size_t w_step, Wino4x2Stage<C>& ws) {
+    if constexpr (S < 6) {
+        constexpr int r = S;
+        ws.x[r].x = wino4x2_act<C>(ws.x[r].x, r == 0 ? ws.m0 : r == 5 ? ws.m5 : ws.mc, ws);
+        ws.x[r].y = wino4x2_act<C>(ws.x[r].y, r == 0 ? ws.m0 : r == 5 ? ws.m5 : ws.mc, ws);
+        ws.h[r] = wino4x2_act<C>(ws.h[r], r == 0 ? ws.mh0 : r == 5 ? ws.mh5 : ws.mh, ws);
+    } else if constexpr (S < 15) {
+        constexpr int col = (S - 6) / 3, p = (S - 6) % 3;
+        if constexpr (col == 0) wino4x2_ypair<p>(ws.x[0].x, ws.x[1].x, ws.x[2].x, ws.x[3].x, ws.x[4].x, ws.x[5].x, ws.v[0]);
+        if constexpr (col == 1) wino4x2_ypair<p>(ws.x[0].y, ws.x[1].y, ws.x[2].y, ws.x[3].y, ws.x[4].y, ws.x[5].y, ws.v[1]);
+        if constexpr (col == 2) wino4x2_ypair<p>(ws.h[0], ws.h[1], ws.h[2], ws.h[3], ws.h[4], ws.h[5], ws.v[2]);
+    } else if constexpr (S == 15) {
+#pragma unroll
+        for (int i = 0; i < 3; ++i) *reinterpret_cast<f32x4*>(next + C::XT_PAD + ws.wlds + i * 1024) = ws.wv[i];
+#pragma unroll
+        for (int i = 0; i < 3; ++i) {
+            wino_opaque(ws.woff);
+            ws.wv[i] = *reinterpret_cast<const f32x4*>(w_cb + (3 + i) * w_step + ws.woff);
+        }
+    } else if constexpr (S < 22) {
+        constexpr int ty = S - 16;
+        const float d1 = ws.v[0][ty], d2 = ws.v[1][ty], hv = ws.v[2][ty];
+        const float l = __int_as_float(__builtin_amdgcn_ds_bpermute(ws.lane_l, __float_as_int(d2)));
+        const float r = __int_as_float(__builtin_amdgcn_ds_bpermute(ws.lane_r, __float_as_int(d1)));
+        const float d0 = ws.edge_l ? hv : l, d3 = ws.edge_r ? hv : r;
+        *reinterpret_cast<f32x4*>(next + ws.xlds + ty * 128) = f32x4{d0 - d2, d1 + d2, d2 - d1, d1 - d3};
+    } else {
+#pragma unroll
+        for (int i = 0; i < 3; ++i) *reinterpret_cast<f32x4*>(next + C::XT_PAD + ws.wlds + (3 + i) * 1024) = ws.wv[i];
+    }
+}
+
+template <class C, int G>
+__device__ __forceinline__ void wino4x2_gap(float* next, const float* sbn, const char* in_cb, const char* w_cb, size_t w_step, Wino4x2Stage<C>& ws) {
+    if constexpr (G < WINO4X2_LOAD_SLICES) wino4x2_load_slice<C, G>(in_cb, w_cb, w_step, sbn, ws);
+    if constexpr (G >= WINO4X2_FIRST_WORK_GAP && G < 47) wino4x2_work_slice<C, G - WINO4X2_FIRST_WORK_GAP>(next, w_cb, w_step, ws);
+}
+
+template <class C>
+struct Wino4x2Acc {
+    f32x16 a[4][4];
+    f32x16 v[2][4];
+};
+
+template <int TY, int TX, class C>
+__device__ __forceinline__ void wino4x2_mfma(Wino4x2Acc<C>& m, float wa, float xb) {
+    if constexpr (TY < 4) asm volatile("v_mfma_f32_32x32x2_f32 %0, %1, %2, %0" : "+a"(m.a[TY][TX]) : "v"(wa), "v"(xb));
+    else asm volatile("v_mfma_f32_32x32x2_f32 %0, %1, %2, %0" : "+v"(m.v[TY - 4][TX]) : "v"(wa), "v"(xb));
+}
+
+__device__ __forceinline__ void wino4x2_settle() {
+    __builtin_amdgcn_sched_barrier(0);
+    asm volatile("s_nop 15\n\ts_nop 7");
+    __builtin_amdgcn_sched_barrier(0);
+}
+
+template <class C, bool STAGE_NEXT>
+__device__ __forceinline__ void wino4x2_chunk(const float* cur, float* next, const float* sbn, const char* in_cb, const char* w_cb, size_t w_step,
+                                              Wino4x2Stage<C>& ws, Wino4x2Acc<C>& m) {
+    f32x4 av[2], bv[2];
+    av[0] = *reinterpret_cast<const f32x4*>(cur + ws.abase);
+    bv[0] = *reinterpret_cast<const f32x4*>(cur + ws.bbase);
+    static_for<0, 12>([&](auto gc) {
+        constexpr int g = decltype(gc)::value, ty = g % 6;
+        if constexpr (g + 1 < 12) {
+            constexpr int ks = (g + 1) / 6, t = (g + 1) % 6;
+            av[(g + 1) & 1] = *reinterpret_cast<const f32x4*>(cur + ws.abase + (ks * 12 + t) * 256);
+            bv[(g + 1) & 1] = *reinterpret_cast<const f32x4*>(cur + ws.bbase + (ks * 24 + t) * 128);
+        }
+        __builtin_amdgcn_sched_barrier(0);
+        static_for<0, 4>([&](auto xc) {
+            constexpr int tx = decltype(xc)::value;
+            wino4x2_mfma<ty, tx>(m, av[g & 1][tx], bv[g & 1][tx]);
+            __builtin_amdgcn_sched_barrier(0);
+            if constexpr (STAGE_NEXT) {
+                wino4x2_gap<C, 4 * g + tx>(next, sbn, in_cb, w_cb, w_step, ws);
+                __builtin_amdgcn_sched_barrier(0);
+            }
+        });
+    });
+}
+
+template <class C>
+__device__ __forceinline__ void wino4x2_mask_tail(bool okc, Wino4x2Stage<C>& ws) {
+    const unsigned keep = okc ? 0xFFFFFFFFu : 0u;
+    ws.m0 &= keep, ws.m5 &= keep, ws.mc &= keep, ws.mh0 &= keep, ws.mh5 &= keep, ws.mh &= keep;
+#pragma unroll
+    for (int r = 0; r < 6; ++r) ws.off[r] &= keep, ws.hoff[r] &= keep;
+}
+
+template <class C>
+__device__ __forceinline__ void wino4x2_main(const ConvArgs& a, float* smem, const int tid, const int y0, const int x0, const int b0, const int co0,
+                                             const unsigned HWin, f32x16 (&acc)[C::ENT], long long* t_loop) {
+    static_assert(C::ENT == 8 && C::XT == 6144 && C::WT == 6144 && C::XT_PAD == C::XT, "one job and six weight float4s per thread");
+    const int lane = tid & 63, wave = tid >> 6, half = lane >> 5, l31 = lane & 31;
+    const int wq = wave & 1, wh = wave >> 1;
+    Wino4x2Stage<C> ws;
+    {
+        const int c = wave, q = half, j = l31;
+        const int y = y0 + 4 * q - 1, x = x0 + 2 * j;
+        const bool inb = b0 < a.B;
+        ws.edge_l = j == 0;
+        ws.edge_r = j == 31;
+        const int hx = ws.edge_l ? x0 - 1 : ws.edge_r ? x0 + 64 : x;
+        const bool okh = inb && hx >= 0 && hx < a.W;
+#pragma unroll
+        for (int r = 0; r < 6; ++r) {
+            const bool ok = inb && y + r >= 0 && y + r < a.H;
+            ws.off[r] = ok ? (unsigned(c) * HWin + unsigned((y + r) * a.W + x)) * 4u : 0u;
+            ws.hoff[r] = (ok && okh) ? (unsigned(c) * HWin + unsigned((y + r) * a.W + hx)) * 4u : 0u;
+        }
+        ws.m0 = (inb && y >= 0) ? 0xFFFFFFFFu : 0u;
+        ws.m5 = (inb && y + 5 < a.H) ? 0xFFFFFFFFu : 0u;
+        ws.mc = inb ? 0xFFFFFFFFu : 0u;
+        ws.mh = okh ? 0xFFFFFFFFu : 0u;
+        ws.mh0 = ws.mh & ws.m0;
+        ws.mh5 = ws.mh & ws.m5;
+        ws.xlds = ((c * 2 + q) * 6) * 128 + j * 4;
+        ws.bn = c;
+        ws.lane_l = ((lane + 63) & 63) * 4;
+        ws.lane_r = ((lane + 1) & 63) * 4;
+    }
+    ws.woff = (unsigned(tid >> 6) * unsigned(a.cout_pad) + unsigned(co0 + (tid & 63))) * 16u;
+    ws.wlds = tid * 4;
+    const size_t w_step = size_t(4) * a.cout_pad * 16;
+    const size_t w_cstep = size_t(C::CK) * 6 * a.cout_pad * 16;
+    const size_t in_step = size_t(C::CK) * HWin * 4;
+    ws.floor = __int_as_float(__builtin_amdgcn_readfirstlane(a.pre_scale != nullptr ? 0 : int(0xFF800000u)));
+    ws.abase = C::XT_PAD + (half * 6 * 64 + 32 * wh + l31) * 4;
+    ws.bbase = ((half * 2 + wq) * 6) * 128 + l31 * 4;
+    float* const sbn = smem + 2 * C::STAGE;
+    const char* in_cb = reinterpret_cast<const char*>(a.in + size_t((b0 < a.B ? b0 : 0) * a.in_ctot + a.in_coff) * HWin);
+    const char* w_cb = reinterpret_cast<const char*>(a.w);
+    const int last = a.cin_pad - C::CK;
+    if (last == 0) wino4x2_mask_tail<C>(wave < a.cin, ws);
+    static_for<0, 5>([&](auto sc) { wino4x2_load_slice<C, decltype(sc)::value>(in_cb, w_cb, w_step, sbn, ws); });
+    for (int i = tid; i < a.cin_pad; i += 256) {
+        sbn[2 * i] = a.pre_scale != nullptr ? a.pre_scale[i] : 1.f;
+        sbn[2 * i + 1] = a.pre_scale != nullptr ? a.pre_shift[i] : -0.f;
+    }
+    __syncthreads();
+    static_for<5, WINO4X2_LOAD_SLICES>([&](auto sc) { wino4x2_load_slice<C, decltype(sc)::value>(in_cb, w_cb, w_step, sbn, ws); });
+    static_for<0, WINO4X2_WORK_SLICES>([&](auto sc) { wino4x2_work_slice<C, decltype(sc)::value>(smem, w_cb, w_step, ws); });
+    __syncthreads();
+#if defined(MVLM_CONV_TIMING)
+    *t_loop = clock64();
+#endif
+    Wino4x2Acc<C> m;
+#pragma unroll
+    for (int ty = 0; ty < 6; ++ty)
+#pragma unroll
+        for (int tx = 0; tx < 4; ++tx) (ty < 4 ? m.a[ty & 3][tx] : m.v[ty & 1][tx]) = f32x16{0.f, 0.f, 0.f, 0.f, 0.f, 0.f, 0.f, 0.f, 0.f, 0.f, 0.f, 0.f, 0.f, 0.f, 0.f, 0.f};
+    wino4x2_settle();
+    int cur = 0;
+    for (int cb = 0; cb < last; cb += C::CK) {
+        in_cb += in_step, w_cb += w_cstep;
+        ws.bn += C::CK;
+        if (cb + C::CK == last) wino4x2_mask_tail<C>(last + wave < a.cin, ws);
+        wino4x2_chunk<C, true>(smem + cur * C::STAGE, smem + (cur ^ 1) * C::STAGE, sbn, in_cb, w_cb, w_step, ws, m);
+        __syncthreads();
+        cur ^= 1;
+    }
+    wino4x2_chunk<C, false>(smem + cur * C::STAGE, nullptr, sbn, nullptr, nullptr, 0, ws, m);
+    wino4x2_settle();
+    __syncthreads();
+    float* const ex = smem + wave * (C::EXCHANGE / 4) + half * (16 * 4 * C::TW);
+#pragma unroll
+    for (int r = 0; r < 16; ++r) {
+        float o[2][6];
+#pragma unroll
+        for (int ty = 0; ty < 6; ++ty) {
+            const f32x16(&t)[4] = ty < 4 ? m.a[ty & 3] : m.v[ty & 1];
+            o[0][ty] = (t[0][r] + t[1][r]) + t[2][r];
+            o[1][ty] = (t[1][r] - t[2][r]) - t[3][r];
+        }
+        float out[4][2];
+#pragma unroll
+        for (int c = 0; c < 2; ++c) {
+            const float m0 = o[c][0], m1 = o[c][1], m2 = o[c][2], m3 = o[c][3], m4 = o[c][4], m5 = o[c][5];
+            const float s = m1 + m2, d = m1 - m2;
+            out[0][c] = (m0 + s) + (m3 + m4);
+            out[1][c] = d + fmaf(-0.5f, m4, 2.f * m3);
+            out[2][c] = s + fmaf(0.25f, m4, 4.f * m3);
+            out[3][c] = (d + fmaf(-0.125f, m4, 8.f * m3)) + m5;
+        }
+#pragma unroll
+        for (int row = 0; row < 4; ++row) *reinterpret_cast<float2*>(ex + (r * 4 + row) * C::TW + 2 * l31) = make_float2(out[row][0], out[row][1]);
+    }
+    __syncthreads();
+#pragma unroll
+    for (int n = 0; n < 8; ++n)
+#pragma unroll
+        for (int r = 0; r < 16; ++r) acc[n][r] = ex[(r * 4 + (n >> 1)) * C::TW + (n & 1) * 32 + l31];
+    (void)t_loop;
+}
+
+template <class C>
+__device__ __forceinline__ void wino4x2_tile(const ConvArgs& a, const int tiles_x, const int tiles_y, const int cout_tiles, const int bid, const int nblk) {
+    extern __shared__ __attribute__((aligned(16))) float smem[];
+    const int tid = threadIdx.x, lane = tid & 63, wave = tid >> 6, half = lane >> 5, l31 = lane & 31;
+    int lid;
+    {
+        const int q = nblk >> 3, r = nblk & 7, xcd = bid & 7;
+        lid = (xcd < r ? xcd * (q + 1) : r * (q + 1) + (xcd - r) * q) + (bid >> 3);
+    }
+    const int ct = lid % cout_tiles, pt = lid / cout_tiles;
+    const int tx = pt % tiles_x, ty = (pt / tiles_x) % tiles_y, tb = pt / (tiles_x * tiles_y);
+    const int x0 = tx * C::TW, y0 = ty * C::TRI, b0 = tb, co0 = ct * C::COUT_T;
+    const int H = a.H, W = a.W;
+    const unsigned HW = unsigned(H) * unsigned(W);
+#if defined(MVLM_CONV_TIMING)
+    const long long t_start = clock64();
+    long long t_loop = t_start;
+    long long* const t_loop_p = &t_loop;
+#else
+    long long* const t_loop_p = nullptr;
+#endif
+    f32x16 acc[C::ENT];
+    wino4x2_main<C>(a, smem, tid, y0, x0, b0, co0, HW, acc, t_loop_p);
+#if defined(MVLM_CONV_TIMING)
+    const long long t_epi = clock64();
+#endif
+    const int eco0 = co0 + 32 * (wave >> 1);
+    const size_t b = size_t(b0);
+    unsigned pix[C::ENT], pix2[C::ENT];
+#pragma unroll
+    for (int n = 0; n < C::ENT; ++n) {
+        const int y = y0 + 4 * (wave & 1) + (n >> 1), x = x0 + 32 * (n & 1) + l31;
+        pix[n] = unsigned(y * W + x);
+        pix2[n] = unsigned(2 * y) * unsigned(2 * W) + unsigned(2 * x);
+    }
+    const bool scat = a.up_out == 1;
+    const unsigned W2 = 2u * unsigned(W);
+#pragma unroll
+    for (int g = 0; g < 4; ++g)
+#pragma unroll
+        for (int j = 0; j < 4; ++j) {
+            const int c = eco0 + 8 * g + 4 * half + j;
+            const bool okc = c < a.cout;
+            const int cs = okc ? c : 0;
+            const float bias = a.bias ? a.bias[c] : 0.f;
+            const float ps = a.post_scale ? a.post_scale[c] : 1.f, pt = a.post_scale ? a.post_shift[c] : 0.f;
+            float v[C::ENT];
+#pragma unroll
+            for (int n = 0; n < C::ENT; ++n) {
+                v[n] = acc[n][4 * g + j];
+                if (a.bias) v[n] += bias;
+                if (a.post_scale) v[n] = fmaxf(fmaf(v[n], ps, pt), 0.f);
+            }
+            if (a.out_raw && okc) {
+                float* const p = a.out_raw + (b * a.raw_ctot + a.raw_coff + c) * HW;
+#pragma unroll
+                for (int n = 0; n < C::ENT; ++n) p[pix[n]] = v[n];
+            }
+            if (a.res1) {
+                const float* const p1 = a.res1 + (b * a.res1_ctot + a.res1_coff + cs) * HW;
+                float r[C::ENT];
+#pragma unroll
+                for (int n = 0; n < C::ENT; ++n) r[n] = p1[pix[n]];
+                if (a.res2) {
+                    const float* const p2 = a.res2 + (b * a.res2_ctot + a.res2_coff + cs) * HW;
+#pragma unroll
+                    for (int n = 0; n < C::ENT; ++n) r[n] += p2[pix[n]];
+                }
+#pragma unroll
+                for (int n = 0; n < C::ENT; ++n) v[n] += r[n];
+            }
+            if (a.out && !scat) {
+                float* const p = a.out + (b * a.out_ctot + a.out_coff + cs) * HW;
+                if (okc) {
+#pragma unroll
+                    for (int n = 0; n < C::ENT; ++n) p[pix[n]] = v[n];
+                }
+            } else if (a.out) {
+                const float* const ps2 = a.skip + (b * a.skip_ctot + a.skip_coff + cs) * HW * 4;
+                float* const p = a.out + (b * a.out_ctot + a.out_coff + cs) * HW * 4;
+                float2 s0[C::ENT], s1[C::ENT];
+#pragma unroll
+                for (int n = 0; n < C::ENT; ++n) {
+                    s0[n] = *reinterpret_cast<const float2*>(ps2 + pix2[n]);
+                    s1[n] = *reinterpret_cast<const float2*>(ps2 + pix2[n] + W2);
+                }
+                if (okc) {
+#pragma unroll
+                    for (int n = 0; n < C::ENT; ++n) {
+                        *reinterpret_cast<float2*>(p + pix2[n]) = make_float2(v[n] + s0[n].x, v[n] + s0[n].y);
+                        *reinterpret_cast<float2*>(p + pix2[n] + W2) = make_float2(v[n] + s1[n].x, v[n] + s1[n].y);
+                    }
+                }
+            }
+        }
+#if defined(MVLM_CONV_TIMING)
+    if (a.timing && tid == 0) {
+        __builtin_amdgcn_s_waitcnt(0);
+        const long long t_end = clock64();
+        atomicAdd(a.timing + 0, (unsigned long long)(t_loop - t_start));
+        atomicAdd(a.timing + 1, (unsigned long long)(t_epi - t_loop));
+        atomicAdd(a.timing + 2, (unsigned long long)(t_end - t_epi));
+        atomicAdd(a.timing + 3, 1ull);
+    }
+#endif
+}
+
+}
+#endif
```

Result: no change. 1377 views/s (median of 3 runs) (-0.0%).
